# Guoxs/DODT

Hardware: AMD Instinct MI355X
Metric: frame-pairs/sec (whole node) KITTI-shape tau=2 (higher is better)
Workload: dtype f32

## Files before the change

dodt_amd/_lib.py:

```python
import ctypes as C
import os

_HERE = os.path.dirname(os.path.abspath(__file__))
LIB_PATH = os.environ.get('DODT_HIP_LIB') or os.path.join(_HERE, 'lib', 'libdodt_hip.so')

OK, ERR_INVALID, ERR_HIP, ERR_UNSUPPORTED = 0, 1, 2, 3
PTS_VELO_XYZI, PTS_CAM_3XN = 0, 1
EXTRACTOR_VGG_PYR = 0
EXTRACTOR_VGG = 1
EXTRACTOR_SHARED_GPU = 0x100
EXTRACTOR_BF16 = 0x200
EXTRACTOR_SPLIT = 0x400
FC_RELU = 1
FC_BF16 = 2
CONFLICT_RAISE, CONFLICT_NEXT_BEST = 0, 1


class DodtError(RuntimeError):
    pass


class BevParams(C.Structure):
    _fields_ = [
        ('point_format', C.c_int32),
# ... 17 lines not shown


class LayerInfo(C.Structure):
    _fields_ = [('name', C.c_char * 32), ('kernel', C.c_char * 48), ('launches', C.c_int32),
                ('items', C.c_int32), ('flops_direct', C.c_double), ('flops_executed', C.c_double),
                ('bytes', C.c_double), ('ms', C.c_float), ('reserved_', C.c_int32)]


_vp = C.c_void_p
_i = C.c_int
_f = C.c_float
_d = C.c_double
_pi32 = C.c_void_p
_pf = C.c_void_p
_hf = C.c_void_p

SIGNATURES = {
    'dodt_version': (_i, []),
    'dodt_last_error': (C.c_char_p, []),
    'dodt_ctx_create': (_i, [_i, C.POINTER(_vp)]),
    'dodt_mark': (_i, [_vp, _i]),
    'dodt_ctx_wait_mark': (_i, [_vp, _vp, _i]),
    'dodt_mark_elapsed': (_i, [_vp, _i, _vp, _i, C.POINTER(_f)]),
    'dodt_ctx_create_high_priority': (_i, [_i, C.POINTER(_vp)]),
    'dodt_ctx_create_on_stream': (_i, [_i, _vp, C.POINTER(_vp)]),
    'dodt_ctx_destroy': (_i, [_vp]),
    'dodt_ctx_sync': (_i, [_vp]),
    'dodt_ctx_wait_for': (_i, [_vp, _vp]),
    'dodt_malloc': (_i, [_vp, C.c_size_t, C.POINTER(_vp)]),
    'dodt_free': (_i, [_vp, _vp]),
    'dodt_memcpy_h2d': (_i, [_vp, _vp, _vp, C.c_size_t]),
    'dodt_memcpy_d2h': (_i, [_vp, _vp, _vp, C.c_size_t]),
    'dodt_memset': (_i, [_vp, _vp, _i, C.c_size_t]),
    'dodt_pinned_alloc': (_i, [_vp, C.c_size_t, C.POINTER(_vp)]),
    'dodt_pinned_free': (_i, [_vp, _vp]),
    'dodt_memcpy_h2d_async': (_i, [_vp, _vp, _vp, C.c_size_t]),
    'dodt_fetch_i32_begin': (_i, [_vp, _pi32, _i, _i]),
    'dodt_fetch_i32_end': (_i, [_vp, _i, C.POINTER(C.c_int32), _i]),
    'dodt_timer_start': (_i, [_vp]),
    'dodt_timer_stop': (_i, [_vp, C.POINTER(_f)]),
    'dodt_bev_slices': (_i, [_vp, _vp, _i, C.POINTER(BevParams), _pf, _vp]),
    'dodt_bev_status': (_i, [_vp, C.POINTER(_i)]),
    'dodt_bev_support_mask': (_i, [C.POINTER(BevParams), _i, _vp, _i, _i]),
    'dodt_anchor_filter': (_i, [_vp, _vp, _i, _i, _pi32, _i, _i, _pi32, _pi32]),
    'dodt_project_anchors_f64': (_i, [_vp, _vp, _pi32, _i, _pi32,
                                      C.POINTER(_d), C.POINTER(_d), _d, _d,
                                      _pf, _pf, _pf]),
    'dodt_project_anchors_f32': (_i, [_vp, _pf, _i, _pi32, C.POINTER(_f),
                                      C.POINTER(_f), _f, _f, _pf, _pf, _pf]),
    'dodt_img_preprocess': (_i, [_vp, _vp, _i, _i, _i, _i, _i,
                                 C.POINTER(_f), _pf]),
    'dodt_conv_mode': (_i, []),
    'dodt_extractor_create': (_i, [_vp, _i, _i, _i, _i, _i, _i,
                                   C.POINTER(_vp)]),
    'dodt_extractor_destroy': (_i, [_vp]),
    'dodt_extractor_set_layer': (_i, [_vp, C.c_char_p, _vp, _i, _i, _i, _i,
                                      _vp, _vp, _vp]),
    'dodt_extractor_input': (_i, [_vp, C.POINTER(_vp), C.POINTER(C.c_longlong)]),
    'dodt_extractor_forward': (_i, [_vp, _pf, _pf, _pf]),
    'dodt_extractor_forward_padded': (_i, [_vp, _pf, _pf, _pf]),
    'dodt_extractor_set_input': (_i, [_vp, _pf]),
    'dodt_extractor_set_input_support': (_i, [_vp, _vp, _i, _i, C.POINTER(C.c_longlong)]),
    'dodt_extractor_set_frame_tables': (_i, [_vp, _i, C.POINTER(_i)]),
    'dodt_extractor_frame_items': (_i, [_vp, C.POINTER(_i), _i]),
    'dodt_extractor_frame_split': (_i, [_vp, C.POINTER(_i), C.POINTER(_i), _i]),
    'dodt_extractor_store_bytes': (C.c_longlong, [_vp]),
    'dodt_frame_tables_host': (_i, [_vp, _i, _i, _i, _i, _i, _i, _vp, _i, _vp, _vp, C.POINTER(_i)]),
    'dodt_frame_restore_host': (_i, [_vp, _i, _i, _i, _i, _i, _i, _i, _i, _i, _vp, _vp, _vp, _vp]),
    'dodt_frame_lists_host': (_i, [_vp, _i, _i, _i, _i, _i, _i, _vp, _i, _vp, _vp, C.POINTER(_i), _vp, C.POINTER(_i)]),
    'dodt_extractor_read_activation': (_i, [_vp, C.c_char_p, _vp,
                                            C.POINTER(_i), C.POINTER(_i),
                                            C.POINTER(_i)]),
    'dodt_extractor_output_shape': (_i, [_vp, C.POINTER(_i), C.POINTER(_i), C.POINTER(_i)]),
    'dodt_extractor_first_layers_folded': (_i, [_vp]),
    'dodt_extractor_flops': (_d, [_vp]),
    'dodt_extractor_mfma_flops': (_d, [_vp]),
    'dodt_extractor_bytes': (_d, [_vp]),
    'dodt_extractor_layer_count': (_i, [_vp]),
    'dodt_extractor_forward_timed': (_i, [_vp, _pf, _pf, _pf, C.POINTER(LayerInfo), _i]),
    'dodt_crop_and_resize': (_i, [_vp, _pf, _i, _i, _i, _pf, _i, _pi32, _i, _i,
                                  _pf]),
    'dodt_crop_and_resize_strided': (_i, [_vp, _pf, _i, _i, _i, _pf, _i, _pi32, _i, _i, _pf,
                                          C.c_longlong]),
    'dodt_correlation': (_i, [_vp, _pf, _pf, _i, _i, _i, _i, _i, _i, _pf]),
    'dodt_mean_fusion': (_i, [_vp, _pf, _pf, _i, _pi32, _i, _pf]),
    'dodt_fc_create': (_i, [_vp, _i, _i, _hf, _hf, _i, C.POINTER(_vp)]),
    'dodt_fc_create_ex': (_i, [_vp, _i, _i, _hf, _hf, _i, C.POINTER(_vp)]),
    'dodt_fc_destroy': (_i, [_vp]),
    'dodt_fc_forward': (_i, [_vp, _vp, _pf, _pf, _i, _i, _pi32, _pf, _i]),
    'dodt_fc_forward_split': (_i, [_vp, _vp, _pf, _i, _i, _pi32, _i, C.POINTER(_i), C.POINTER(_vp)]),
    'dodt_fc_flops': (_d, [_vp, _i]),
    'dodt_fc_bf16_row_elems': (_i, [_vp]),
    'dodt_fc_forward_bf16': (_i, [_vp, _vp, _vp, _i, _i, _pi32, _vp, _i, _i]),
    'dodt_fc_forward_split_bf16': (_i, [_vp, _vp, _vp, _i, _i, _pi32, _i, C.POINTER(_i), C.POINTER(_vp)]),
    'dodt_rows_to_bf16': (_i, [_vp, _pf, _pf, _i, _pi32, _i, _i, _vp, _i]),
    'dodt_nms': (_i, [_vp, _pf, _pf, _i, _pi32, _i, _f, _pi32, _pi32]),
    'dodt_offset_to_anchor': (_i, [_vp, _pf, _pf, _i, _pi32, _pf]),
    'dodt_softmax_fg': (_i, [_vp, _pf, _i, _pi32, _pf]),
    'dodt_rpn_decode': (_i, [_vp, _pf, _pf, _pf, _i, _pi32, C.POINTER(_f), _pf, _pf, _pf]),
    'dodt_gather_project': (_i, [_vp, _pf, _pi32, _i, _pi32, C.POINTER(_f), C.POINTER(_f), _f, _f, _pf, _pf, _pf]),
    'dodt_final_decode': (_i, [_vp, _pf, _pf, _pf, _pf, _i, _pi32, C.POINTER(_f), C.POINTER(_f),
                               _pf, _pf, _pf, _pf, _pf, _pf]),
    'dodt_gather_rows': (_i, [_vp, _pf, _i, _pi32, _i, _pi32, _pf]),
    'dodt_max_fg_logit': (_i, [_vp, _pf, _i, _i, _pi32, _pf]),
    'dodt_pack_detections': (_i, [_vp, _pf, _pf, _pf, _pf, _pi32, _pi32, _i, _f, _pf, _pi32]),
    'dodt_angle_vector_to_orientation': (_i, [_vp, _pf, _i, _pi32, _pf]),
    'dodt_box_4c_decode': (_i, [_vp, _pf, _pf, _i, _pi32, C.POINTER(_f),
                                C.POINTER(_f), _pf, _pf, _pf]),
    'dodt_comm_unique_id': (_i, [_vp]),
    'dodt_comm_create': (_i, [_vp, _i, _i, _vp, C.POINTER(_vp)]),
    'dodt_comm_destroy': (_i, [_vp]),
    'dodt_comm_attach': (_i, [_vp, _vp]),
    'dodt_comm_rank': (_i, [_vp, C.POINTER(_i), C.POINTER(_i)]),
    'dodt_comm_set_late_peer': (_i, [_vp, _d]),
    'dodt_all_gather_records': (_i, [_vp, _vp, _i, _pf, _pi32, _i, _i, _i, _i, _pf, _pi32]),
    'dodt_comm_join': (_i, [_vp, _i, _vp]),
    'dodt_comm_sync': (_i, [_vp]),
    'dodt_comm_barrier': (_i, [_vp]),
    'dodt_comm_max_f64': (_i, [_vp, C.POINTER(_d)]),
    'dodt_three_d_iou_matrix': (_i, [_vp, _vp, _i, _vp, _i, _vp]),
    'dodt_interpolate_pairs': (_i, [_vp, _vp, _i, _pi32, _i, _i, _i, _d, _i, _vp, C.POINTER(_d), _i, _vp,
                                    _pi32, _pi32]),
    'dodt_track_state_bytes': (_i, [_i, C.POINTER(C.c_size_t)]),
    'dodt_track_reset': (_i, [_vp, _vp, _i]),
    'dodt_track_flush': (_i, [_vp, _vp, _d, _i]),
    'dodt_track_encode': (_i, [_vp, _vp, _i, _pi32, _i, _i, C.POINTER(_d), _d, _d, _d, _pf, _pf, _pi32]),
    'dodt_track_pairs': (_i, [_vp, _vp, _vp, _i, _pi32, _i, _i, C.POINTER(_d), _d, _d, _d, _d, _d, _i]),
    'dodt_track_encoded': (_i, [_vp, _vp, _pf, _pf, _pi32, _i, _i, _d, _d, _i]),
}
COMM_ID_BYTES = 128

_lib = None


def load():
    global _lib
    if _lib is not None:
        return _lib
    if not os.path.exists(LIB_PATH):
        raise DodtError(
            'libdodt_hip.so not found at %s -- build it with '
            '`make -C dodt_amd/csrc` (there is no CPU fallback)' % LIB_PATH)
    lib = C.CDLL(LIB_PATH)
    for name, (res, args) in SIGNATURES.items():
        fn = getattr(lib, name)
        fn.restype = res
        fn.argtypes = args
    _lib = lib
    return lib


def check(rc, what=''):
    if rc == OK:
        return
    msg = load().dodt_last_error().decode('utf-8', 'replace')
    if rc == ERR_INVALID:
        raise ValueError(msg or what)
    raise DodtError('%s: %s (status %d)' % (what, msg, rc))
```

dodt_amd/core/avod_fc_layers/fusion_fc_layers.py:

```python
import os

import numpy as np

from dodt_amd import ops


class EarlyFusionFcLayers(object):

    K_ALIGN = 32

    def __init__(self, ctx, params, outputs=('cls_out', 'off_out', 'ang_out'), dtype='f32'):
        names = sorted(k for k in params if k.startswith('fc'))
        w0 = np.asarray(params[names[0]]['w'], np.float32)
        self.in_k = w0.shape[0]
        self.in_ld = -(-self.in_k // self.K_ALIGN) * self.K_ALIGN
        if self.in_ld != self.in_k:
            w0 = np.concatenate([w0, np.zeros((self.in_ld - self.in_k, w0.shape[1]), np.float32)], 0)
        self.hidden = [ops.FullyConnected(ctx, w0 if k == names[0] else params[k]['w'], params[k]['b'],
                                          True, dtype=dtype) for k in names]
        self._packed_first = None
        self._first_params = (params[names[0]]['w'], params[names[0]]['b'], dtype)
        self.outputs = [ops.FullyConnected(ctx, params[k]['w'], params[k]['b'], False, dtype=dtype)
                        for k in outputs]
        self.fused_out = None
        if len(outputs) > 1:
            w = np.concatenate([np.asarray(params[k]['w'], np.float32) for k in outputs], 1)
            b = np.concatenate([np.asarray(params[k]['b'], np.float32) for k in outputs])
            fused = ops.FullyConnected(ctx, w, b, False, dtype=dtype)
            if fused.can_split():
                self.fused_out = fused
            else:
                fused.close()
        self.width = max(l.N for l in self.hidden)
        self.ctx = ctx
        self.bf16_rows = dtype == 'bf16' and os.environ.get('DODT_FC_BF16_ROWS', '1') != '0' and \
            all(l.bf16_row_elems() > 0 for l in self.hidden) and \
            (self.fused_out.bf16_row_elems() > 0 if self.fused_out is not None
             else all(l.bf16_row_elems() > 0 for l in self.outputs))
        self.in_ld16 = self.hidden[0].bf16_row_elems() if self.bf16_rows else 0

    def make_scratch(self, n_max):
        s = [self.ctx.empty((n_max, self.width), np.float32) for _ in range(2)] + \
            [self.ctx.zeros((n_max, self.in_ld), np.float32)]
        if self.bf16_rows:
            s += [self.ctx.zeros((n_max, self.width), np.uint16) for _ in range(2)] + \
                 [self.ctx.zeros((n_max, self.in_ld16), np.uint16)]
        return s

    def forward(self, ctx, d_rois, d_rois2, n, d_n, d_outs, scratch):
        x, x2 = d_rois, d_rois2
        ldx = self._row_floats(d_rois, n, 'd_rois')
        if x2 is not None and self._row_floats(x2, n, 'd_rois2') != ldx:
            raise ValueError('d_rois and d_rois2 must have the same row layout')
        if self.bf16_rows and len(scratch) > 5:
            ops.rows_to_bf16(ctx, x, x2, n, d_n, self.in_k, ldx, scratch[5], self.in_ld16)
            x16, ld16 = scratch[5], self.in_ld16
            for i, l in enumerate(self.hidden):
                y16 = scratch[3 + (i & 1)]
                l.forward_bf16(x16, n, y16, ldx=ld16, ldy=self.width, d_m=d_n, y_bf16=True, ctx=ctx)
                x16, ld16 = y16, self.width
            if self.fused_out is not None:
                self.fused_out.forward_split_bf16(x16, n, d_outs, [l.N for l in self.outputs], ldx=ld16, d_m=d_n, ctx=ctx)
            else:
                for l, d_y in zip(self.outputs, d_outs):
                    l.forward_bf16(x16, n, d_y, ldx=ld16, d_m=d_n, y_bf16=False, ctx=ctx)
            return
        first = self.hidden[0]
        if ldx != self.in_ld:
            if self._packed_first is None:
                w, b, dtype = self._first_params
                self._packed_first = ops.FullyConnected(self.ctx, w, b, True, dtype=dtype)
            first = self._packed_first
        if x2 is not None and len(scratch) > 2 and ldx == self.in_ld == self.in_k and self.in_k % 4 == 0:
            ops.mean_fusion(ctx, x, x2, n, d_n, self.in_ld, scratch[2])
            x, x2 = scratch[2], None
        for i, l in enumerate([first] + self.hidden[1:]):
            y = scratch[i & 1]
            l.forward(x, n, y, ldx=ldx, ldy=self.width, d_x2=x2, d_m=d_n, ctx=ctx)
            x, x2, ldx = y, None, self.width
        if self.fused_out is not None and ldx % 4 == 0:
            self.fused_out.forward_split(x, n, d_outs, [l.N for l in self.outputs], ldx=ldx, d_m=d_n, ctx=ctx)
            return
        for l, d_y in zip(self.outputs, d_outs):
            l.forward(x, n, d_y, ldx=ldx, d_m=d_n, ctx=ctx)

    def _row_floats(self, d, n, name):
        if d.dtype != np.float32:
            raise ValueError('%s must be float32' % name)
        size = int(np.prod(d.shape, dtype=np.int64))
        rows = d.shape[0] if len(d.shape) > 1 else 0
        if rows < n or rows == 0 or size % rows:
            raise ValueError('%s holds %s, fewer than %d rows' % (name, d.shape, n))
        per_row = size // rows
        if per_row not in (self.in_ld, self.in_k):
            raise ValueError('%s rows hold %d floats; the head takes %d (crop + zero tail) or %d (packed)'
                             % (name, per_row, self.in_ld, self.in_k))
        return per_row

    def flops(self, n):
        return sum(l.flops(n) for l in self.hidden + self.outputs) \
            - 2.0 * n * (self.in_ld - self.in_k) * self.hidden[0].N

    def close(self):
        for l in self.hidden + self.outputs + [self.fused_out, self._packed_first]:
            if l is not None:
                l.close()
```

dodt_amd/core/models/anchor_predictor.py:

```python
import numpy as np

from dodt_amd import ops


class AnchorPredictor(object):
    def __init__(self, ctx, params, dtype='f32'):
        def mat(name):
            w = np.asarray(params[name]['w'], np.float32)
            return w.reshape(-1, w.shape[-1]), np.asarray(params[name]['b'], np.float32)
        wc, bc = mat('cls_fc6')
        wr, br = mat('reg_fc6')
        self.width = wc.shape[1]
        if wr.shape != wc.shape:
            raise ValueError('cls_fc6 and reg_fc6 must have the same size')
        self.fc6 = ops.FullyConnected(ctx, np.concatenate([wc, wr], 1),
                                      np.concatenate([bc, br]), True, dtype=dtype)
        self.cls7 = ops.FullyConnected(ctx, *mat('cls_fc7'), relu=True, dtype=dtype)
        self.reg7 = ops.FullyConnected(ctx, *mat('reg_fc7'), relu=True, dtype=dtype)
        self.cls8 = ops.FullyConnected(ctx, *mat('cls_fc8'), relu=False, dtype=dtype)
        self.reg8 = ops.FullyConnected(ctx, *mat('reg_fc8'), relu=False, dtype=dtype)
        self.layers = [self.fc6, self.cls7, self.reg7, self.cls8, self.reg8]
        (w8c, b8c), (w8r, b8r) = mat('cls_fc8'), mat('reg_fc8')
        w8 = np.zeros((w8c.shape[0] + w8r.shape[0], w8c.shape[1] + w8r.shape[1]), np.float32)
        w8[:w8c.shape[0], :w8c.shape[1]] = w8c
        w8[w8c.shape[0]:, w8c.shape[1]:] = w8r
        self.out8 = ops.FullyConnected(ctx, w8, np.concatenate([b8c, b8r]), False, dtype=dtype)
        if not (self.out8.can_split() and w8c.shape[0] == self.width == w8r.shape[0]):
            self.out8.close()
            self.out8 = None
        self.ctx = ctx

    def make_scratch(self, n_max):
        return [self.ctx.empty((n_max, 2 * self.width), np.float32) for _ in range(2)]

    def forward(self, ctx, d_bev_roi, d_img_roi, n, d_objectness, d_offsets, scratch):
        w = self.width
        h6, h7 = scratch
        self.fc6.forward(d_bev_roi, n, h6, d_x2=d_img_roi, ctx=ctx)
        self.cls7.forward(h6, n, h7, ldx=2 * w, ldy=2 * w, ctx=ctx)
        self.reg7.forward(h6.offset(4 * w, (1,)), n, h7.offset(4 * w, (1,)),
                          ldx=2 * w, ldy=2 * w, ctx=ctx)
        if self.out8 is not None:
            self.out8.forward_split(h7, n, [d_objectness, d_offsets], [self.cls8.N, self.reg8.N], ctx=ctx)
            return
        self.cls8.forward(h7, n, d_objectness, ldx=2 * w, ctx=ctx)
        self.reg8.forward(h7.offset(4 * w, (1,)), n, d_offsets, ldx=2 * w, ctx=ctx)

    def flops(self, n):
        return sum(l.flops(n) for l in self.layers)

    def close(self):
        for l in self.layers + ([self.out8] if self.out8 is not None else []):
            l.close()
```

dodt_amd/csrc/crop.hip:

```cpp
#include "common.h"

namespace {

template <int VEC>
__global__ void __launch_bounds__(256)
crop_kernel(const float* __restrict__ img, int H, int W, int C, const float* __restrict__ boxes,
            int n, const int* __restrict__ d_n, int ch, int cw, float* __restrict__ out,
            long long out_stride) {
    const int groups = C / VEC;
    const long long t = (long long)blockIdx.x * blockDim.x + threadIdx.x;
    const int lim = d_n ? min(*d_n, n) : n;
    const long long total = (long long)lim * ch * cw * groups;
    if (t >= total) return;
    const int g = (int)(t % groups);
    long long r = t / groups;
    const int ix = (int)(r % cw); r /= cw;
    const int iy = (int)(r % ch);
    const int b = (int)(r / ch);
    const float4 bx = reinterpret_cast<const float4*>(boxes)[b];
    const float y1 = bx.x, x1 = bx.y, y2 = bx.z, x2 = bx.w;
    const float hm1 = (float)(H - 1), wm1 = (float)(W - 1);
    const float hs = (ch > 1) ? (y2 - y1) * hm1 / (float)(ch - 1) : 0.0f;
    const float ws = (cw > 1) ? (x2 - x1) * wm1 / (float)(cw - 1) : 0.0f;
    const float in_y = (ch > 1) ? y1 * hm1 + (float)iy * hs : 0.5f * (y1 + y2) * hm1;
    const float in_x = (cw > 1) ? x1 * wm1 + (float)ix * ws : 0.5f * (x1 + x2) * wm1;
    float* o = out + (size_t)b * out_stride + (((size_t)iy * cw + ix) * C + (size_t)g * VEC);
    const bool ok = (in_y >= 0.0f) && (in_y <= hm1) && (in_x >= 0.0f) && (in_x <= wm1);
    if (!ok) {
#pragma unroll
        for (int k = 0; k < VEC; ++k) o[k] = 0.0f;
        return;
    }
    const int ty = (int)floorf(in_y), by = (int)ceilf(in_y);
    const int lx_i = (int)floorf(in_x), rx_i = (int)ceilf(in_x);
    const float ly = in_y - (float)ty, lx = in_x - (float)lx_i;
    const float* ptl = img + ((size_t)ty * W + lx_i) * C + (size_t)g * VEC;
    const float* ptr = img + ((size_t)ty * W + rx_i) * C + (size_t)g * VEC;
    const float* pbl = img + ((size_t)by * W + lx_i) * C + (size_t)g * VEC;
    const float* pbr = img + ((size_t)by * W + rx_i) * C + (size_t)g * VEC;
#pragma unroll
    for (int k = 0; k < VEC; ++k) {
        const float tl = ptl[k], tr = ptr[k], bl = pbl[k], br = pbr[k];
        const float top = tl + (tr - tl) * lx;
        const float bot = bl + (br - bl) * lx;
        o[k] = top + (bot - top) * ly;
    }
}

}

extern "C" int dodt_crop_and_resize(dodt_ctx* ctx, const float* d_image, int H, int W, int C,
                                    const float* d_boxes, int n, const int32_t* d_n, int crop_h,
                                    int crop_w, float* d_out) {
    return dodt_crop_and_resize_strided(ctx, d_image, H, W, C, d_boxes, n, d_n, crop_h, crop_w, d_out,
                                        (long long)crop_h * crop_w * C);
}

extern "C" int dodt_crop_and_resize_strided(dodt_ctx* ctx, const float* d_image, int H, int W, int C,
                                            const float* d_boxes, int n, const int32_t* d_n, int crop_h,
                                            int crop_w, float* d_out, long long out_box_stride) {
    DODT_REQUIRE(ctx && d_image && d_out && (n == 0 || d_boxes),
                 "dodt_crop_and_resize: NULL argument");
    DODT_REQUIRE(H > 0 && W > 0 && C > 0 && crop_h > 0 && crop_w > 0 && n >= 0,
                 "dodt_crop_and_resize: bad sizes");
    DODT_REQUIRE(out_box_stride >= (long long)crop_h * crop_w * C,
                 "dodt_crop_and_resize: output stride %lld shorter than a crop", out_box_stride);
    if (n == 0) return DODT_OK;
    const int vec = (C % 4 == 0 && out_box_stride % 4 == 0) ? 4 : 1;
    const long long total = (long long)n * crop_h * crop_w * (C / vec);
    const int blocks = (int)((total + 255) / 256);
    if (vec == 4)
        hipLaunchKernelGGL(crop_kernel<4>, dim3(blocks), dim3(256), 0, ctx->stream, d_image, H, W,
                           C, d_boxes, n, d_n, crop_h, crop_w, d_out, out_box_stride);
    else
        hipLaunchKernelGGL(crop_kernel<1>, dim3(blocks), dim3(256), 0, ctx->stream, d_image, H, W,
                           C, d_boxes, n, d_n, crop_h, crop_w, d_out, out_box_stride);
    DODT_LAUNCH_CHECK();
    return DODT_OK;
}
```

dodt_amd/csrc/gemm.hip:

```cpp
#include <cmath>
#include <cstdlib>
#include <mutex>
#include <set>
#include <type_traits>
#include <vector>

#include <algorithm>

#include "common.h"
#include "lds_dma.h"

namespace {

typedef float f32x16 __attribute__((ext_vector_type(16)));
typedef float f32x4 __attribute__((ext_vector_type(4)));

constexpr int kKAlign = 64;
constexpr int kSmallK = 16;

struct GemmArgs {
    const float* x;
    const float* x2;
    const float* w;
    const float* bias;
    float* y;
    int M, K, Kp, N, ldx, ldy, relu;
    const int* d_m;
    unsigned long long* clock_probe = nullptr;
};

typedef __bf16 bf16x8 __attribute__((ext_vector_type(8)));
typedef __bf16 bf16x2 __attribute__((ext_vector_type(2)));
typedef float f32x2 __attribute__((ext_vector_type(2)));
__device__ __forceinline__ float pack_bf16(float lo, float hi) {
    return __builtin_bit_cast(float, __builtin_convertvector(f32x2{lo, hi}, bf16x2));
}

__device__ __forceinline__ float bf16_value(float packed, int which) {
    const unsigned u = __builtin_bit_cast(unsigned, packed);
    return __builtin_bit_cast(float, which ? (u & 0xffff0000u) : (u << 16));
}

template <int BM, int BN, int WM, int WN, bool XVEC, int WBN, int kBK, bool FUSE, bool BF16>
__global__ void __launch_bounds__(256)
fc_mfma_kernel(const GemmArgs a) {
    constexpr int MT = BM / 32 / WM, NT = BN / 32 / WN;
    constexpr int KB = BF16 ? 8 : 4;
    constexpr int G = kBK * 4 / KB;
    constexpr int kXS = G + 4;
    constexpr int XITEMS = BM * (G / 4);
    constexpr int WITEMS = G * BN / 4;
    constexpr int NX = (XITEMS + 255) / 256, NW = (WITEMS + 255) / 256;
    constexpr int kBuf = BM * kXS + G * BN;
    extern __shared__ __attribute__((aligned(16))) float smem[];

    const int tid = threadIdx.x, lane = tid & 63, wave = tid >> 6;
    const int wm = wave / WN, wn = wave % WN;
    const int li = lane & 31, lh = lane >> 5;
    const int m0 = blockIdx.x * BM, nt0 = blockIdx.y;
    const int M = a.d_m ? min(*a.d_m, a.M) : a.M;
    if (m0 >= M) return;
    const int nstages = a.Kp / kBK;
    static_assert(WBN % BN == 0, "tile must divide the blocked width");
    const f32x4* wblk = reinterpret_cast<const f32x4*>(a.w) +
                        (size_t)(nt0 * BN / WBN) * (a.Kp / (2 * KB)) * 2 * WBN + (nt0 * BN) % WBN;

    constexpr int XV = KB / 4;
    f32x4 prex[NX][XV];
    f32x4 pre[NX + NW];
    constexpr int NSLOT = NX + NW;
    int g_off[NSLOT];
    int l_off[NSLOT];
    int k_q[NX];
#pragma unroll
    for (int j = 0; j < NSLOT; ++j) {
        if (j < NX) {
            const int t = tid + j * 256;
            const int row = min(t / (G / 4), BM - 1), q = t % (G / 4);
            const int m = min(m0 + row, M - 1);
            g_off[j] = m * a.ldx + q * KB;
            k_q[j < NX ? j : 0] = q * KB;
            l_off[j] = row * kXS + q * 4;
        } else {
            const int t = min(tid + (j - NX) * 256, WITEMS - 1);
            g_off[j] = (t / BN) * WBN + t % BN;
            l_off[j] = BM * kXS + t * 4;
        }
    }
    f32x4 pre2[FUSE ? NX : 1][XV];
    auto load_slot = [&](int j, int st) {
        if (j < NX) {
            const int jx = j < NX ? j : 0;
// ... 99 lines not shown
            } else {
#pragma unroll
                for (int s = 0; s < 2; ++s)
#pragma unroll
                    for (int mt = 0; mt < MT; ++mt)
#pragma unroll
                        for (int nt = 0; nt < NT; ++nt)
                            acc[mt * NT + nt] = __builtin_amdgcn_mfma_f32_32x32x2f32(
                                xf[cb][mt][s], wf[cb][nt][s], acc[mt * NT + nt], 0, 0, 0);
            }
#pragma unroll
            for (int j = q * SPQ; j < (q + 1) * SPQ && j < NSLOT; ++j) {
                store_slot(j, buf ^ 1, min(st + 1, last));
                load_slot(j, st2);
            }
            if constexpr (!BF16) {
#pragma unroll
                for (int s = 2; s < 4; ++s)
#pragma unroll
                    for (int mt = 0; mt < MT; ++mt)
#pragma unroll
                        for (int nt = 0; nt < NT; ++nt)
                            acc[mt * NT + nt] = __builtin_amdgcn_mfma_f32_32x32x2f32(
                                xf[cb][mt][s], wf[cb][nt][s], acc[mt * NT + nt], 0, 0, 0);
            }
            __builtin_amdgcn_sched_barrier(0);
        }
        __syncthreads();
    }
#pragma unroll
    for (int nt = 0; nt < NT; ++nt) {
        const int n = nt0 * BN + (wn * NT + nt) * 32 + li;
        const float b = a.bias[n];
#pragma unroll
        for (int mt = 0; mt < MT; ++mt)
#pragma unroll
            for (int r = 0; r < 16; ++r) {
                const int m = m0 + (wm * MT + mt) * 32 + (r & 3) + 8 * (r >> 2) + 4 * lh;
                if (m < M && n < a.N) {
                    float v = acc[mt * NT + nt][r] + b;
                    if (a.relu) v = fmaxf(v, 0.0f);
                    a.y[(size_t)m * a.ldy + n] = v;
                }
            }
    }
}

template <int BM, int BN, int WM, int WN, int WBN = BN, int kBK = 32, bool BF16 = false>
int launch_fc(hipStream_t s, const GemmArgs& a, int Npad) {
    constexpr int G = BF16 ? kBK / 2 : kBK;
    constexpr size_t lds = 2 * (size_t)(BM * (G + 4) + G * BN) * sizeof(float);
    const bool vec = (a.ldx % 4 == 0) && (a.K % (BF16 ? 8 : 4) == 0);
    dim3 grid(dodt::ceil_div(a.M, BM), Npad / BN);
    auto go = [&](auto kernel) -> hipError_t {
        static std::mutex mu;
        static std::set<const void*> prepared;
        {
            std::lock_guard<std::mutex> lock(mu);
            if (!prepared.count(reinterpret_cast<const void*>(kernel))) {
                hipError_t e = hipFuncSetAttribute(reinterpret_cast<const void*>(kernel),
                                                   hipFuncAttributeMaxDynamicSharedMemorySize,
                                                   (int)lds);
                if (e != hipSuccess) return e;
                prepared.insert(reinterpret_cast<const void*>(kernel));
            }
        }
        hipLaunchKernelGGL(kernel, grid, dim3(256), lds, s, a);
        return hipSuccess;
    };
    hipError_t e;
    if (vec && a.x2) e = go(&fc_mfma_kernel<BM, BN, WM, WN, true, WBN, kBK, true, BF16>);
    else if (vec) e = go(&fc_mfma_kernel<BM, BN, WM, WN, true, WBN, kBK, false, BF16>);
    else if (a.x2) e = go(&fc_mfma_kernel<BM, BN, WM, WN, false, WBN, kBK, true, BF16>);
    else e = go(&fc_mfma_kernel<BM, BN, WM, WN, false, WBN, kBK, false, BF16>);
    DODT_HIP_CHECK(e);
    DODT_LAUNCH_CHECK();
    return DODT_OK;
}

constexpr int kDmaBM = 64, kDmaBK = 32, kDmaStages = 3;
constexpr int kDmaXFloats = kDmaBM * kDmaBK;

template <bool FUSE, int NT>
__global__ void __launch_bounds__(256, 2)
fc_dma_kernel(const GemmArgs a, int tiles_m, int tiles_n) {
    constexpr int kDmaBN = 64 * NT, kDmaWFloats = kDmaBK * kDmaBN;
    using dodt::blds16;
    using dodt::i32x4_t;
    using dodt::kOob;
    using dodt::make_rsrc;
    constexpr int kStage = kDmaXFloats * (FUSE ? 2 : 1) + kDmaWFloats;
    extern __shared__ __attribute__((aligned(16))) float smem[];
    const int tid = threadIdx.x, lane = tid & 63;
    const int wave = __builtin_amdgcn_readfirstlane(tid >> 6);
    const int wm = wave >> 1, wn = wave & 1;
    const int li = lane & 31, lh = lane >> 5;
    const int T = tiles_m * tiles_n;
    int tile = blockIdx.x;
    if (T % 8 == 0) tile = (int)(blockIdx.x % 8) * (T / 8) + (int)(blockIdx.x / 8);
    const int mt = tile / tiles_n, nt0 = tile % tiles_n;
    const int m0 = mt * kDmaBM;
    const int M = a.d_m ? min(*a.d_m, a.M) : a.M;
    if (m0 >= M) return;
    const int nstages = a.K / kDmaBK;

    const int rows = min(M - m0, kDmaBM);
    const i32x4_t x_rsrc = make_rsrc(a.x + (size_t)m0 * a.ldx, (unsigned)(((size_t)(rows - 1) * a.ldx + a.K) * 4));
    i32x4_t x2_rsrc = x_rsrc;
    if (FUSE) x2_rsrc = make_rsrc(a.x2 + (size_t)m0 * a.ldx, (unsigned)(((size_t)(rows - 1) * a.ldx + a.K) * 4));
    const int n0 = nt0 * kDmaBN;
    const float* wblk = a.w + ((size_t)(n0 / 128) * (a.Kp / 8) * 2 * 128 + (n0 % 128)) * 4;
    const i32x4_t w_rsrc = make_rsrc(wblk, (unsigned)(((size_t)(a.Kp / 8) * 2 * 128 - (n0 % 128)) * 16));
    int x_off[2], w_off[2 * NT];
#pragma unroll
    for (int k = 0; k < 2; ++k) {
        const int piece = wave + 4 * k;
        const int row = piece * 8 + (lane >> 3), cq = (lane & 7) ^ ((row >> 1) & 7);
        x_off[k] = row < rows ? (row * a.ldx + cq * 4) * 4 : kOob;
    }
#pragma unroll
    for (int k = 0; k < 2 * NT; ++k) {
        const int piece = wave + 4 * k;
        w_off[k] = ((piece / NT) * 128 + (piece % NT) * 64 + lane) * 16;
    }
    const unsigned lds0 = (unsigned)(size_t)(__attribute__((address_space(3))) void*)smem;
    constexpr int kPerStage = (FUSE ? 4 : 2) + 2 * NT;
    auto issue_one = [&](int st, int buf, int n) {
        const unsigned sX = lds0 + (unsigned)(buf * kStage) * 4;
        constexpr int kX = FUSE ? 4 : 2;
        if (n < kX) {
            const int k = FUSE ? n >> 1 : n;
            const unsigned piece = (unsigned)(wave + 4 * k) * 1024;
            if (FUSE && (n & 1)) dodt::blds16s(x2_rsrc, x_off[k], st * (kDmaBK * 4), sX + kDmaXFloats * 4 + piece);
            else dodt::blds16s(x_rsrc, x_off[k], st * (kDmaBK * 4), sX + piece);
        } else {
            const int k = n - kX;
            dodt::blds16s(w_rsrc, w_off[k], st * (8 * 128 * 16),
                          sX + kDmaXFloats * (FUSE ? 8 : 4) + (unsigned)(wave + 4 * k) * 1024);
        }
    };

    f32x16 acc[NT];
#pragma unroll
    for (int nt = 0; nt < NT; ++nt)
#pragma unroll
        for (int r = 0; r < 16; ++r) acc[nt][r] = 0.0f;
    const int xrow = wm * 32 + li;
    const int xsw = (xrow >> 1) & 7;
    const int x_base = xrow * kDmaBK;
    const int w_base = kDmaXFloats * (FUSE ? 2 : 1) + (lh * kDmaBN + wn * 32 * NT + li) * 4;

    int xo[4];
#pragma unroll
    for (int q = 0; q < 4; ++q) xo[q] = x_base + (((2 * q + lh) ^ xsw) * 4);
    auto stage = [&](auto bufc, int st) {
        constexpr int BUF = decltype(bufc)::value;
        if (st + 1 < nstages) __builtin_amdgcn_s_waitcnt(0x0f70 | kPerStage);
        else __builtin_amdgcn_s_waitcnt(0x0f70);
        __builtin_amdgcn_s_barrier();
        const bool more = st + 2 < nstages;
        const float* sS = smem + BUF * kStage;
        f32x4 xf[4], wf[4][NT], x2[FUSE ? 4 : 1];
        auto read_q = [&](int q) {
            xf[q] = *reinterpret_cast<const f32x4*>(sS + xo[q]);
#pragma unroll
            for (int nt = 0; nt < NT; ++nt)
                wf[q][nt] = *reinterpret_cast<const f32x4*>(sS + w_base + q * (2 * kDmaBN * 4) + nt * 128);
            if (FUSE) x2[q] = *reinterpret_cast<const f32x4*>(sS + kDmaXFloats + xo[q]);
        };
        read_q(0);
        read_q(1);
        __builtin_amdgcn_sched_barrier(0);
        constexpr int kPerQ = (kPerStage + 3) / 4;
#pragma unroll
        for (int q = 0; q < 4; ++q) {
            if (q + 2 < 4) read_q(q + 2);
            if (FUSE) {
#pragma unroll
                for (int e = 0; e < 4; ++e) xf[q][e] = (xf[q][e] + x2[q][e]) / 2.0f;
            }
#pragma unroll
            for (int s2 = 0; s2 < 4; ++s2)
#pragma unroll
                for (int nt = 0; nt < NT; ++nt)
                    acc[nt] = __builtin_amdgcn_mfma_f32_32x32x2f32(xf[q][s2], wf[q][nt][s2], acc[nt], 0, 0, 0);
            if (more) {
#pragma unroll
                for (int n = q * kPerQ; n < (q + 1) * kPerQ && n < kPerStage; ++n) issue_one(st + 2, (BUF + 2) % kDmaStages, n);
            }
            __builtin_amdgcn_sched_barrier(0);
        }
    };
    auto issue = [&](int st, int buf) {
#pragma unroll
        for (int n = 0; n < kPerStage; ++n) issue_one(st, buf, n);
    };
    issue(0, 0);
    if (nstages > 1) issue(1, 1);
    const bool probe = a.clock_probe != nullptr && blockIdx.x == 17 && tid == 0;
    unsigned long long c0 = 0, r0 = 0;
    if (probe) { c0 = __builtin_amdgcn_s_memtime(); r0 = __builtin_amdgcn_s_memrealtime(); }
    for (int st = 0; st < nstages; st += 3) {
        stage(std::integral_constant<int, 0>{}, st);
        if (st + 1 < nstages) stage(std::integral_constant<int, 1>{}, st + 1);
        if (st + 2 < nstages) stage(std::integral_constant<int, 2>{}, st + 2);
    }
    if (probe) {
        a.clock_probe[0] = __builtin_amdgcn_s_memtime() - c0;
        a.clock_probe[1] = __builtin_amdgcn_s_memrealtime() - r0;
    }
#pragma unroll
    for (int nt = 0; nt < NT; ++nt) {
        const int n = n0 + wn * 32 * NT + nt * 32 + li;
        const float b = a.bias[n];
#pragma unroll
        for (int r = 0; r < 16; ++r) {
            const int m = m0 + wm * 32 + (r & 3) + 8 * (r >> 2) + 4 * lh;
            if (m < M && n < a.N) {
                float v = acc[nt][r] + b;
                if (a.relu) v = fmaxf(v, 0.0f);
                a.y[(size_t)m * a.ldy + n] = v;
            }
        }
    }
}

int launch_fc_dma(hipStream_t s, const GemmArgs& a_in, int Npad) {
    GemmArgs a = a_in;
    static const bool want_clock = getenv("DODT_FC_CLOCK") != nullptr;
    static unsigned long long* d_probe = nullptr;
    if (want_clock) {
        if (!d_probe) DODT_HIP_CHECK(hipMalloc(&d_probe, 2 * sizeof(unsigned long long)));
        a.clock_probe = d_probe;
    }
    static const int force_nt = getenv("DODT_FC_NT") ? atoi(getenv("DODT_FC_NT")) : 0;
    const int nt = force_nt ? force_nt
                            : (!a.x2 && (long)dodt::ceil_div(a.M, kDmaBM) * (Npad / 128) >= 2 * 256 ? 2 : 1);
    const int tiles_m = dodt::ceil_div(a.M, kDmaBM), tiles_n = Npad / (64 * nt);
    auto go = [&](auto kernel, size_t lds) -> hipError_t {
        static std::mutex mu;
        static std::set<const void*> prepared;
        {
            std::lock_guard<std::mutex> lock(mu);
            if (!prepared.count(reinterpret_cast<const void*>(kernel))) {
                hipError_t e = hipFuncSetAttribute(reinterpret_cast<const void*>(kernel),
                                                   hipFuncAttributeMaxDynamicSharedMemorySize, (int)lds);
                if (e != hipSuccess) return e;
                prepared.insert(reinterpret_cast<const void*>(kernel));
            }
        }
        hipLaunchKernelGGL(kernel, dim3(tiles_m * tiles_n), dim3(256), lds, s, a, tiles_m, tiles_n);
        return hipSuccess;
    };
    hipError_t e;
    if (a.x2) e = go(&fc_dma_kernel<true, 1>, (size_t)kDmaStages * (2 * kDmaXFloats + kDmaBK * 64) * 4);
    else if (nt == 2) e = go(&fc_dma_kernel<false, 2>, (size_t)kDmaStages * (kDmaXFloats + kDmaBK * 128) * 4);
    else e = go(&fc_dma_kernel<false, 1>, (size_t)kDmaStages * (kDmaXFloats + kDmaBK * 64) * 4);
    DODT_HIP_CHECK(e);
    DODT_LAUNCH_CHECK();
    if (want_clock) {
        unsigned long long h[2] = {0, 0};
        (void)hipStreamSynchronize(s);
        (void)hipMemcpy(h, d_probe, sizeof(h), hipMemcpyDeviceToHost);
        if (h[1])
            fprintf(stderr, "[dodt] fc_dma_kernel M %d K %d N %d: K loop of workgroup 17: %llu shader cycles in %.2f us = %.3f GHz\n",
                    a.M, a.K, a.N, h[0], h[1] / 100.0, (double)h[0] / h[1] * 0.1);
    }
    return DODT_OK;
}

constexpr int kBfBM = 64, kBfBN = 128, kBfStages = 3;
__host__ __device__ constexpr int bf_swz(int r, int S) { return (r / (16 / S)) & (S - 1); }

template <bool YBF16, int BK, int R = kBfStages>
__global__ void __launch_bounds__(256, 2)
fc_bf16_dma_kernel(const GemmArgs a, int tiles_m, int tiles_n) {
    static_assert((R - 2) * ((kBfBM + kBfBN) * BK * 2 / 1024 / 4) <= 63, "vmcnt is six bits");
    using dodt::i32x4_t;
    using dodt::kOob;
    using dodt::make_rsrc;
    constexpr int S = BK / 8;
    constexpr int kXBytes = kBfBM * BK * 2, kWBytes = kBfBN * BK * 2, kStage = kXBytes + kWBytes;
    constexpr int kXPieces = kXBytes / 1024 / 4, kWPieces = kWBytes / 1024 / 4;
    constexpr int kPerStage = kXPieces + kWPieces;
    constexpr int kRowsPerPiece = 1024 / (BK * 2);
    constexpr int NQ = BK / 16;
    extern __shared__ __attribute__((aligned(16))) float smem[];
    const int tid = threadIdx.x, lane = tid & 63;
    const int wave = __builtin_amdgcn_readfirstlane(tid >> 6);
    const int wm = wave >> 1, wn = wave & 1;
    const int li = lane & 31, lh = lane >> 5;
    const int T = tiles_m * tiles_n;
    int tile = blockIdx.x;
    if (T % 8 == 0) tile = (int)(blockIdx.x % 8) * (T / 8) + (int)(blockIdx.x / 8);
    const int mt = tile / tiles_n, nt0 = tile % tiles_n;
    const int m0 = mt * kBfBM;
    const int M = a.d_m ? min(*a.d_m, a.M) : a.M;
    if (m0 >= M) return;
    const int nstages = a.Kp / BK;
    const int rows = min(M - m0, kBfBM);
    const unsigned short* x16 = reinterpret_cast<const unsigned short*>(a.x);
    const i32x4_t x_rsrc = make_rsrc(x16 + (size_t)m0 * a.ldx, (unsigned)(((size_t)(rows - 1) * a.ldx + a.Kp) * 2));
    const char* wblk = reinterpret_cast<const char*>(a.w) + (size_t)nt0 * nstages * kWBytes;
    const i32x4_t w_rsrc = make_rsrc(wblk, (unsigned)((size_t)nstages * kWBytes));
    int x_off[kXPieces];
#pragma unroll
    for (int k = 0; k < kXPieces; ++k) {
        const int row = (wave + 4 * k) * kRowsPerPiece + lane / S, slot = (lane % S) ^ bf_swz(row, S);
        x_off[k] = row < rows ? (row * a.ldx + slot * 8) * 2 : kOob;
    }
    const int w_off = lane * 16;
    const unsigned lds0 = (unsigned)(size_t)(__attribute__((address_space(3))) void*)smem;
    auto issue_one = [&](int st, int buf, int n) {
        const unsigned sX = lds0 + (unsigned)(buf * kStage);
        if (n < kXPieces) dodt::blds16s(x_rsrc, x_off[n < kXPieces ? n : 0], st * (BK * 2), sX + (unsigned)(wave + 4 * n) * 1024);
        else dodt::blds16s(w_rsrc, w_off, st * kWBytes + (wave + 4 * (n - kXPieces)) * 1024,
                           sX + kXBytes + (unsigned)(wave + 4 * (n - kXPieces)) * 1024);
    };
    f32x16 acc[2];
#pragma unroll
    for (int nt = 0; nt < 2; ++nt)
#pragma unroll
        for (int r = 0; r < 16; ++r) acc[nt][r] = 0.0f;
    const int sw = bf_swz(li, S);
    int so[NQ];
#pragma unroll
    for (int q = 0; q < NQ; ++q) so[q] = ((2 * q + lh) ^ sw) * 16;
    const int x_base = (wm * 32 + li) * (BK * 2);
    const int w_base = kXBytes + (wn * 64 + li) * (BK * 2);
    auto stage = [&](auto bufc, int st) {
        constexpr int BUF = decltype(bufc)::value;
        if (st + R - 2 < nstages) asm volatile("s_waitcnt vmcnt(%0)" ::"n"((R - 2) * kPerStage) : "memory");
        else __builtin_amdgcn_s_waitcnt(0x0f70);
        __builtin_amdgcn_s_barrier();
        const bool more = st + R - 1 < nstages;
        const char* sS = reinterpret_cast<const char*>(smem) + BUF * kStage;
        f32x4 xf[NQ], wf[NQ][2];
        auto read_q = [&](int q) {
            xf[q] = *reinterpret_cast<const f32x4*>(sS + x_base + so[q]);
#pragma unroll
            for (int nt = 0; nt < 2; ++nt)
                wf[q][nt] = *reinterpret_cast<const f32x4*>(sS + w_base + nt * 32 * (BK * 2) + so[q]);
        };
        read_q(0);
        read_q(1);
        __builtin_amdgcn_sched_barrier(0);
#pragma unroll
        for (int q = 0; q < NQ; ++q) {
            if (q + 2 < NQ) read_q(q + 2);
#pragma unroll
// ... 153 lines not shown
                wa[u] = ok ? w4[(size_t)jj * 128] : z;
                wb[u] = ok ? w4[(size_t)jj * 128 + 16] : z;
            }
#pragma unroll
            for (int u = 0; u < U; ++u)
#pragma unroll
                for (int s = 0; s < 4; ++s) {
                    acc0 = mfma16x4(xv[u][s], wa[u][s], acc0);
                    acc1 = mfma16x4(xv[u][s], wb[u][s], acc1);
                }
        }
    }
    s_part[wave][0][lane] = acc0;
    s_part[wave][1][lane] = acc1;
    __syncthreads();
    if (tid >= 128) return;
    const int nb = tid >> 6;
    f32x4 sum = s_part[0][nb][lane];
#pragma unroll
    for (int w = 1; w < 8; ++w) sum += s_part[w][nb][lane];
    const int n = nb * 16 + i;
    if (n >= a.N) return;
    const float b = a.bias[n];
    const int p = (n >= so.n_end[0]) + (n >= so.n_end[1]);
    float* y = p == 0 ? so.y[0] : (p == 1 ? so.y[1] : so.y[2]);
    const int ld = p == 0 ? so.ld[0] : (p == 1 ? so.ld[1] : so.ld[2]);
    const int nn = n - (p == 0 ? 0 : (p == 1 ? so.n_end[0] : so.n_end[1]));
#pragma unroll
    for (int r = 0; r < 4; ++r) {
        const int m = m0 + 4 * g + r;
        if (m < M) {
            float v = sum[r] + b;
            if (a.relu) v = fmaxf(v, 0.0f);
            y[(size_t)m * ld + nn] = v;
        }
    }
}

template <bool BF16>
__global__ void __launch_bounds__(256)
fc_smallk_kernel(const GemmArgs a, const float* __restrict__ w_plain) {
    const int M = a.d_m ? min(*a.d_m, a.M) : a.M;
    const int n4 = a.N >> 2;
    const long long t = (long long)blockIdx.x * blockDim.x + threadIdx.x;
    const int m = (int)(t / n4), c = (int)(t - (long long)m * n4) * 4;
    if (m >= M) return;
    const float* x = a.x + (size_t)m * a.ldx;
    const float* x2 = a.x2 ? a.x2 + (size_t)m * a.ldx : nullptr;
    f32x4 acc = {0.f, 0.f, 0.f, 0.f};
    for (int k = 0; k < a.K; ++k) {
        float xv = x[k];
        if (x2) xv = (xv + x2[k]) / 2.0f;
        if constexpr (BF16) xv = bf16_value(pack_bf16(xv, 0.0f), 0);
        const f32x4 wv = *reinterpret_cast<const f32x4*>(w_plain + (size_t)k * a.N + c);
        acc += wv * xv;
    }
    const f32x4 b = *reinterpret_cast<const f32x4*>(a.bias + c);
    acc += b;
    if (a.relu) {
#pragma unroll
        for (int i = 0; i < 4; ++i) acc[i] = fmaxf(acc[i], 0.0f);
    }
    float* y = a.y + (size_t)m * a.ldy + c;
    if ((a.ldy & 3) == 0) *reinterpret_cast<f32x4*>(y) = acc;
    else {
#pragma unroll
        for (int i = 0; i < 4; ++i) y[i] = acc[i];
    }
}

bool skinny_ok(int Npad, int K, const GemmArgs& a) {
    static const bool on = !(getenv("DODT_FC_SKINNY") && atoi(getenv("DODT_FC_SKINNY")) == 0);
    return on && Npad == 32 && K % 16 == 0 && a.ldx % 4 == 0 && (size_t)a.x % 16 == 0 && !a.x2;
}

int launch_fc_skinny(hipStream_t s, const GemmArgs& a, const SplitOut& so, bool bf16, bool x_bf16 = false) {
    if (x_bf16) hipLaunchKernelGGL((fc_skinny_kernel<true, true>), dim3(dodt::ceil_div(a.M, 16)), dim3(512), 0, s, a, so);
    else if (bf16) hipLaunchKernelGGL(fc_skinny_kernel<true>, dim3(dodt::ceil_div(a.M, 16)), dim3(512), 0, s, a, so);
    else hipLaunchKernelGGL(fc_skinny_kernel<false>, dim3(dodt::ceil_div(a.M, 16)), dim3(512), 0, s, a, so);
    DODT_LAUNCH_CHECK();
    return DODT_OK;
}

}

namespace {
__global__ void __launch_bounds__(256)
mean_fusion_kernel(const float4* __restrict__ a, const float4* __restrict__ b, int rows, const int* __restrict__ d_n,
                   int row4, float4* __restrict__ out) {
    const int lim = d_n ? min(*d_n, rows) : rows;
    const long long total = (long long)lim * row4;
    for (long long i = (long long)blockIdx.x * blockDim.x + threadIdx.x; i < total;
         i += (long long)gridDim.x * blockDim.x) {
        const float4 x = a[i], y = b[i];
        out[i] = make_float4((x.x + y.x) / 2.0f, (x.y + y.y) / 2.0f, (x.z + y.z) / 2.0f, (x.w + y.w) / 2.0f);
    }
}
}

extern "C" int dodt_mean_fusion(dodt_ctx* ctx, const float* d_a, const float* d_b, int rows, const int32_t* d_n,
                                int row_floats, float* d_out) {
    DODT_REQUIRE(ctx && d_a && d_b && d_out, "dodt_mean_fusion: NULL argument");
    DODT_REQUIRE(rows >= 0 && row_floats >= 4 && row_floats % 4 == 0,
                 "dodt_mean_fusion: rows of a multiple of four floats, got %d", row_floats);
    DODT_REQUIRE(((size_t)d_a | (size_t)d_b | (size_t)d_out) % 16 == 0, "dodt_mean_fusion: 16-byte aligned blocks");
    if (rows == 0) return DODT_OK;
    const long long total = (long long)rows * (row_floats / 4);
    const int blocks = (int)std::min<long long>((total + 255) / 256, 4096);
    hipLaunchKernelGGL(mean_fusion_kernel, dim3(blocks), dim3(256), 0, ctx->stream,
                       reinterpret_cast<const float4*>(d_a), reinterpret_cast<const float4*>(d_b), rows, d_n,
                       row_floats / 4, reinterpret_cast<float4*>(d_out));
    DODT_LAUNCH_CHECK();
    return DODT_OK;
}

namespace {
__global__ void __launch_bounds__(256)
rows_to_bf16_kernel(const float* __restrict__ a, const float* __restrict__ b, int rows, const int* __restrict__ d_n,
                    int row_floats, int in_ld, unsigned short* __restrict__ out, int out_ld) {
    const int lim = d_n ? min(*d_n, rows) : rows;
    const int q4 = out_ld / 4;
    const long long total = (long long)lim * q4;
    for (long long i = (long long)blockIdx.x * blockDim.x + threadIdx.x; i < total;
         i += (long long)gridDim.x * blockDim.x) {
        const int r = (int)(i / q4), c = (int)(i - (long long)r * q4) * 4;
        float v[4];
#pragma unroll
        for (int e = 0; e < 4; ++e) {
            float t = 0.0f;
            if (c + e < row_floats) {
                t = a[(size_t)r * in_ld + c + e];
                if (b) t = (t + b[(size_t)r * in_ld + c + e]) / 2.0f;
            }
            v[e] = t;
        }
        f32x2 o = {pack_bf16(v[0], v[1]), pack_bf16(v[2], v[3])};
        *reinterpret_cast<f32x2*>(out + (size_t)r * out_ld + c) = o;
    }
}
}

extern "C" int dodt_rows_to_bf16(dodt_ctx* ctx, const float* d_a, const float* d_b, int rows, const int32_t* d_n,
                                 int row_floats, int in_ld, void* d_out_bf16, int out_ld) {
    DODT_REQUIRE(ctx && d_a && d_out_bf16, "dodt_rows_to_bf16: NULL argument");
    DODT_REQUIRE(rows >= 0 && row_floats >= 1 && in_ld >= row_floats && out_ld >= row_floats && out_ld % 4 == 0,
                 "dodt_rows_to_bf16: rows of %d floats, %d apart, into rows of %d bf16 (a multiple of 4)", row_floats,
                 in_ld, out_ld);
    DODT_REQUIRE((size_t)d_out_bf16 % 8 == 0, "dodt_rows_to_bf16: 8-byte aligned output");
    if (rows == 0) return DODT_OK;
    const long long total = (long long)rows * (out_ld / 4);
    const int blocks = (int)std::min<long long>((total + 255) / 256, 4096);
    hipLaunchKernelGGL(rows_to_bf16_kernel, dim3(blocks), dim3(256), 0, ctx->stream, d_a, d_b, rows, d_n, row_floats,
                       in_ld, reinterpret_cast<unsigned short*>(d_out_bf16), out_ld);
    DODT_LAUNCH_CHECK();
    return DODT_OK;
}

struct dodt_fc {
    dodt_ctx* ctx = nullptr;
    int K = 0, Kp = 0, N = 0, Npad = 0, BN = 0, relu = 0;
    bool bf16 = false;
    float* d_w = nullptr;
    float* d_b = nullptr;
    float* d_w_plain = nullptr;
    void* d_w_dma = nullptr;
    int Kd = 0;
// ... 48 lines not shown
    if (bf16 && N % kBfBN == 0 && K >= 128) {
        const int BK = bf16_dma_bk(), S = BK / 8;
        f->Kd = (int)dodt::align_up((size_t)K, (size_t)64);
        f->dma_bk = BK;
        const int ns = f->Kd / BK;
        std::vector<uint16_t> img((size_t)(N / kBfBN) * ns * kBfBN * BK, 0);
        for (int k = 0; k < K; ++k)
            for (int n = 0; n < N; ++n) {
                const int t = n / kBfBN, c = n % kBfBN, st = k / BK, kk = k % BK;
                const int slot = (kk / 8) ^ bf_swz(c, S);
                img[((((size_t)t * ns + st) * kBfBN + c) * S + slot) * 8 + kk % 8] = dodt::float_to_bf16(w[(size_t)k * N + n]);
            }
        if (hipMalloc(&f->d_w_dma, img.size() * sizeof(uint16_t)) != hipSuccess) {
            dodt::set_error("dodt_fc_create: hipMalloc failed");
            dodt_fc_destroy(f);
            return DODT_ERR_HIP;
        }
        DODT_HIP_CHECK(hipMemcpy(f->d_w_dma, img.data(), img.size() * sizeof(uint16_t), hipMemcpyHostToDevice));
    }
    std::vector<float> plain;
    if (K <= kSmallK && N % 4 == 0) {
        plain.assign(w, w + (size_t)K * N);
        if (bf16)
            for (float& v : plain) v = dodt::bf16_to_float(dodt::float_to_bf16(v));
        if (hipMalloc(&f->d_w_plain, plain.size() * sizeof(float)) != hipSuccess) {
            dodt::set_error("dodt_fc_create: hipMalloc failed");
            dodt_fc_destroy(f);
            return DODT_ERR_HIP;
        }
        DODT_HIP_CHECK(hipMemcpyAsync(f->d_w_plain, plain.data(), plain.size() * sizeof(float),
                                      hipMemcpyHostToDevice, ctx->stream));
    }
    DODT_HIP_CHECK(hipStreamSynchronize(ctx->stream));
    *out = f;
    return DODT_OK;
}

int dodt_fc_destroy(dodt_fc* f) {
    if (!f) return DODT_OK;
    if (f->d_w) (void)hipFree(f->d_w);
    if (f->d_b) (void)hipFree(f->d_b);
    if (f->d_w_plain) (void)hipFree(f->d_w_plain);
    if (f->d_w_dma) (void)hipFree(f->d_w_dma);
    delete f;
    return DODT_OK;
}

int dodt_fc_forward(dodt_fc* f, dodt_ctx* ctx, const float* d_x, const float* d_x2, int ldx,
                    int M, const int32_t* d_m, float* d_y, int ldy) {
    DODT_REQUIRE(f && d_x && d_y, "dodt_fc_forward: NULL argument");
    DODT_REQUIRE(M >= 0 && ldx >= f->K && ldy >= f->N, "dodt_fc_forward: bad strides");
    if (M == 0) return DODT_OK;
    GemmArgs a;
    a.x = d_x; a.x2 = d_x2; a.w = f->d_w; a.bias = f->d_b; a.y = d_y;
    a.M = M; a.K = f->K; a.Kp = f->Kp; a.N = f->N; a.ldx = ldx; a.ldy = ldy; a.relu = f->relu;
    a.d_m = d_m;
    hipStream_t s = (ctx ? ctx : f->ctx)->stream;
    static const bool smallk = !(getenv("DODT_FC_SMALLK") && atoi(getenv("DODT_FC_SMALLK")) == 0);
    if (smallk && f->d_w_plain && f->N >= 64 && (size_t)d_y % 16 == 0) {
        const long long threads = (long long)M * (f->N / 4);
        if (f->bf16)
            hipLaunchKernelGGL(fc_smallk_kernel<true>, dim3((unsigned)((threads + 255) / 256)), dim3(256), 0, s, a,
                               f->d_w_plain);
        else
            hipLaunchKernelGGL(fc_smallk_kernel<false>, dim3((unsigned)((threads + 255) / 256)), dim3(256), 0, s, a,
                               f->d_w_plain);
        DODT_LAUNCH_CHECK();
        return DODT_OK;
    }
    if (skinny_ok(f->Npad, f->K, a)) {
        SplitOut so = {{d_y, d_y, d_y}, {f->N, f->N, f->N}, {ldy, ldy, ldy}};
        return launch_fc_skinny(s, a, so, f->bf16);
    }
    if (f->bf16) {
        if (f->BN == 128) {
            static const int bk = getenv("DODT_FC_BF16_BK") ? atoi(getenv("DODT_FC_BF16_BK")) : 32;
            if (bk == 64) return launch_fc<64, 128, 2, 2, 128, 64, true>(s, a, f->Npad);
            if (bk == 32) return launch_fc<64, 128, 2, 2, 128, 32, true>(s, a, f->Npad);
            return launch_fc<64, 128, 2, 2, 128, 128, true>(s, a, f->Npad);
        }
        return launch_fc<128, 32, 4, 1, 32, 64, true>(s, a, f->Npad);
    }
    if (f->BN == 128) {
        static const bool dma = !(getenv("DODT_FC_DMA") && atoi(getenv("DODT_FC_DMA")) == 0);
        if (dma && f->K % kDmaBK == 0 && ldx % 4 == 0 && f->K >= 2 * kDmaBK &&
            ((size_t)d_x % 16 == 0) && (!d_x2 || (size_t)d_x2 % 16 == 0))
            return launch_fc_dma(s, a, f->Npad);
        static const int tile = getenv("DODT_FC_TILE") ? atoi(getenv("DODT_FC_TILE")) : 0;
        if (tile == 256) return launch_fc<128, 128, 2, 2, 128, 32>(s, a, f->Npad);
        if (tile == 64) return launch_fc<64, 64, 2, 2, 128>(s, a, f->Npad);
        if (tile == 32) return launch_fc<64, 128, 2, 2, 128, 32>(s, a, f->Npad);
        return launch_fc<64, 128, 2, 2, 128, 64>(s, a, f->Npad);
    }
    return launch_fc<128, 32, 4, 1>(s, a, f->Npad);
}

int dodt_fc_forward_split(dodt_fc* f, dodt_ctx* ctx, const float* d_x, int ldx, int M, const int32_t* d_m,
                          int parts, const int* widths, float* const* d_ys) {
    DODT_REQUIRE(f && d_x && widths && d_ys, "dodt_fc_forward_split: NULL argument");
    DODT_REQUIRE(parts >= 1 && parts <= 3, "dodt_fc_forward_split: %d parts (1..3)", parts);
    DODT_REQUIRE(M >= 0 && ldx >= f->K, "dodt_fc_forward_split: bad strides");
    GemmArgs a;
    a.x = d_x; a.x2 = nullptr; a.w = f->d_w; a.bias = f->d_b; a.y = nullptr;
    a.M = M; a.K = f->K; a.Kp = f->Kp; a.N = f->N; a.ldx = ldx; a.ldy = 0; a.relu = f->relu;
    a.d_m = d_m;
    SplitOut so;
    int end = 0;
    for (int p = 0; p < 3; ++p) {
        const int q = p < parts ? p : parts - 1;
        DODT_REQUIRE(widths[q] >= 1 && d_ys[q], "dodt_fc_forward_split: part %d is empty", q);
        if (p < parts) end += widths[p];
        so.y[p] = d_ys[q];
        so.n_end[p] = p < parts ? end : f->N + 1;
        so.ld[p] = widths[q];
    }
    DODT_REQUIRE(end == f->N, "dodt_fc_forward_split: the parts have %d columns, the layer %d", end, f->N);
    if (!skinny_ok(f->Npad, f->K, a)) {
        dodt::set_error("dodt_fc_forward_split: layers with N <= 32, K %% 16 == 0 and 16-byte aligned rows only");
        return DODT_ERR_UNSUPPORTED;
    }
    if (M == 0) return DODT_OK;
    return launch_fc_skinny((ctx ? ctx : f->ctx)->stream, a, so, f->bf16);
}

int dodt_fc_bf16_row_elems(const dodt_fc* f) {
    if (!f || !f->bf16) return 0;
    if (f->d_w_dma) return f->Kd;
    return (f->Npad == 32 && f->K % 16 == 0) ? f->K : 0;
}

int dodt_fc_forward_bf16(dodt_fc* f, dodt_ctx* ctx, const void* d_x_bf16, int ldx, int M, const int32_t* d_m,
                         void* d_y, int ldy, int y_bf16) {
    DODT_REQUIRE(f && d_x_bf16 && d_y, "dodt_fc_forward_bf16: NULL argument");
    DODT_REQUIRE(f->bf16, "dodt_fc_forward_bf16: the layer was not created with DODT_FC_BF16");
    DODT_REQUIRE(M >= 0 && ldy >= f->N, "dodt_fc_forward_bf16: bad strides");
    if (M == 0) return DODT_OK;
    GemmArgs a;
    a.x = reinterpret_cast<const float*>(d_x_bf16); a.x2 = nullptr; a.bias = f->d_b; a.y = reinterpret_cast<float*>(d_y);
    a.M = M; a.K = f->K; a.N = f->N; a.ldx = ldx; a.ldy = ldy; a.relu = f->relu; a.d_m = d_m;
    hipStream_t s = (ctx ? ctx : f->ctx)->stream;
    if (f->d_w_dma) {
        DODT_REQUIRE(ldx >= f->Kd && ldx % 8 == 0 && (size_t)d_x_bf16 % 16 == 0,
                     "dodt_fc_forward_bf16: rows of >= %d bf16 (zeros beyond K = %d), 16-byte aligned", f->Kd, f->K);
        DODT_REQUIRE((size_t)M * ldx * 2 < (1ull << 31), "dodt_fc_forward_bf16: x block beyond 2 GB");
        a.w = reinterpret_cast<const float*>(f->d_w_dma);
        a.Kp = f->Kd;
        return launch_fc_bf16_dma(s, a, f->Npad, y_bf16 != 0, f->dma_bk);
    }
    if (f->Npad == 32 && f->K % 16 == 0 && ldx % 4 == 0 && (size_t)d_x_bf16 % 8 == 0 && !y_bf16) {
        DODT_REQUIRE(ldx >= f->K, "dodt_fc_forward_bf16: bad strides");
        a.w = f->d_w; a.Kp = f->Kp;
        float* y = reinterpret_cast<float*>(d_y);
        SplitOut so = {{y, y, y}, {f->N, f->N, f->N}, {ldy, ldy, ldy}};
        return launch_fc_skinny(s, a, so, true, true);
    }
    dodt::set_error("dodt_fc_forward_bf16: layers with N %% 128 == 0 and K >= 128, or N <= 32 and K %% 16 == 0 with "
                    "float32 output, only (K = %d, N = %d)", f->K, f->N);
    return DODT_ERR_UNSUPPORTED;
}

int dodt_fc_forward_split_bf16(dodt_fc* f, dodt_ctx* ctx, const void* d_x_bf16, int ldx, int M, const int32_t* d_m,
                               int parts, const int* widths, float* const* d_ys) {
    DODT_REQUIRE(f && d_x_bf16 && widths && d_ys, "dodt_fc_forward_split_bf16: NULL argument");
    DODT_REQUIRE(f->bf16, "dodt_fc_forward_split_bf16: the layer was not created with DODT_FC_BF16");
    DODT_REQUIRE(parts >= 1 && parts <= 3, "dodt_fc_forward_split_bf16: %d parts (1..3)", parts);
    DODT_REQUIRE(M >= 0 && ldx >= f->K, "dodt_fc_forward_split_bf16: bad strides");
    GemmArgs a;
    a.x = reinterpret_cast<const float*>(d_x_bf16); a.x2 = nullptr; a.w = f->d_w; a.bias = f->d_b; a.y = nullptr;
    a.M = M; a.K = f->K; a.Kp = f->Kp; a.N = f->N; a.ldx = ldx; a.ldy = 0; a.relu = f->relu;
    a.d_m = d_m;
    SplitOut so;
    int end = 0;
    for (int p = 0; p < 3; ++p) {
        const int q = p < parts ? p : parts - 1;
        DODT_REQUIRE(widths[q] >= 1 && d_ys[q], "dodt_fc_forward_split_bf16: part %d is empty", q);
        if (p < parts) end += widths[p];
        so.y[p] = d_ys[q];
// ... 18 lines not shown
```

dodt_amd/csrc/nms.hip:

```cpp
#include "common.h"

namespace {

constexpr int kTile = 8192;
constexpr int kSortThreads = 1024;
constexpr int kChunkRows = 2048;
constexpr int kColGroup = 1;
constexpr int kRankMax = 32768;
constexpr int kRankSeg = 512;

struct NmsState {
    int count;
    int done;
    int n_eff;
    int pad;
};

__device__ __forceinline__ uint32_t ordered_bits(float f) {
    const uint32_t b = __float_as_uint(f);
    return (b & 0x80000000u) ? ~b : (b | 0x80000000u);
}

__global__ void __launch_bounds__(256)
nms_keys_kernel(const float* __restrict__ scores, int n, const int* __restrict__ d_n, int n_pad,
                unsigned long long* __restrict__ keys, NmsState* __restrict__ st,
                unsigned long long* __restrict__ removed, int nb, int* __restrict__ rank) {
    const int i = blockIdx.x * blockDim.x + threadIdx.x;
    const int n_eff = d_n ? min(*d_n, n) : n;
    if (i == 0) { st->count = 0; st->done = (n_eff <= 0); st->n_eff = n_eff; }
    if (i < nb) removed[i] = 0ull;
    if (i >= n_pad) return;
    if (rank) rank[i] = 0;
    unsigned long long k = ~0ull;
    if (i < n_eff) k = ((unsigned long long)(~ordered_bits(scores[i])) << 32) | (uint32_t)i;
    keys[i] = k;
}

__device__ __forceinline__ void cmp_swap(unsigned long long& a, unsigned long long& b, bool up) {
    if ((a > b) == up) { const unsigned long long t = a; a = b; b = t; }
}

__global__ void __launch_bounds__(kSortThreads)
nms_sort_local(unsigned long long* __restrict__ keys, int n_pad) {
    extern __shared__ __attribute__((aligned(16))) unsigned long long s_keys[];
    const int tile = min(kTile, n_pad);
    const size_t base = (size_t)blockIdx.x * tile;
    for (int t = threadIdx.x; t < tile; t += kSortThreads) s_keys[t] = keys[base + t];
    __syncthreads();
    for (int k = 2; k <= tile; k <<= 1) {
        for (int j = k >> 1; j > 0; j >>= 1) {
            for (int t = threadIdx.x; t < tile / 2; t += kSortThreads) {
                const int lo = ((t & ~(j - 1)) << 1) | (t & (j - 1));
                const int hi = lo + j;
                const bool up = (((base + lo) & (size_t)k) == 0);
                unsigned long long a = s_keys[lo], b = s_keys[hi];
                cmp_swap(a, b, up);
                s_keys[lo] = a;
                s_keys[hi] = b;
            }
            __syncthreads();
        }
    }
    for (int t = threadIdx.x; t < tile; t += kSortThreads) keys[base + t] = s_keys[t];
}

__global__ void __launch_bounds__(256)
nms_sort_global_step(unsigned long long* __restrict__ keys, int n_pad, int k, int j) {
    const int t = blockIdx.x * blockDim.x + threadIdx.x;
    if (t >= n_pad / 2) return;
    const int lo = ((t & ~(j - 1)) << 1) | (t & (j - 1));
    const int hi = lo + j;
    unsigned long long a = keys[lo], b = keys[hi];
    const bool up = ((lo & k) == 0);
    if ((a > b) == up) { keys[lo] = b; keys[hi] = a; }
}

__global__ void __launch_bounds__(kSortThreads)
nms_sort_local_merge(unsigned long long* __restrict__ keys, int n_pad, int k) {
    extern __shared__ __attribute__((aligned(16))) unsigned long long s_keys[];
    const size_t base = (size_t)blockIdx.x * kTile;
    for (int t = threadIdx.x; t < kTile; t += kSortThreads) s_keys[t] = keys[base + t];
    __syncthreads();
    for (int j = kTile >> 1; j > 0; j >>= 1) {
        for (int t = threadIdx.x; t < kTile / 2; t += kSortThreads) {
            const int lo = ((t & ~(j - 1)) << 1) | (t & (j - 1));
            const int hi = lo + j;
            const bool up = (((base + lo) & (size_t)k) == 0);
            unsigned long long a = s_keys[lo], b = s_keys[hi];
            cmp_swap(a, b, up);
            s_keys[lo] = a;
            s_keys[hi] = b;
        }
        __syncthreads();
    }
    for (int t = threadIdx.x; t < kTile; t += kSortThreads) keys[base + t] = s_keys[t];
}

__global__ void __launch_bounds__(256)
nms_rank_kernel(const unsigned long long* __restrict__ keys, const NmsState* __restrict__ st, int n_pad,
                int* __restrict__ rank) {
    __shared__ __attribute__((aligned(16))) unsigned long long s_seg[kRankSeg];
    const int n_eff = st->n_eff;
    const int i0 = blockIdx.x * 256, j0 = blockIdx.y * kRankSeg;
    if (i0 >= n_eff || j0 >= n_eff) return;
    for (int t = threadIdx.x; t < kRankSeg; t += 256) s_seg[t] = (j0 + t < n_pad) ? keys[j0 + t] : ~0ull;
    __syncthreads();
    const int i = i0 + threadIdx.x;
    if (i >= n_eff) return;
    const unsigned long long mine = keys[i];
    int cnt = 0;
#pragma unroll 16
    for (int j = 0; j < kRankSeg; ++j) cnt += (s_seg[j] < mine) ? 1 : 0;
    if (cnt) atomicAdd(&rank[i], cnt);
}

__global__ void __launch_bounds__(256)
nms_scatter_kernel(const float* __restrict__ boxes, const int* __restrict__ rank,
                   const NmsState* __restrict__ st, int n_rows, float* __restrict__ sb,
                   int* __restrict__ sorted_idx) {
    const int i = blockIdx.x * blockDim.x + threadIdx.x;
    if (i >= n_rows) return;
    float ymin = 0, xmin = 0, ymax = 0, xmax = 0, area = -1.0f;
    int idx = -1, row = i;
    if (i < st->n_eff) {
        idx = i;
        row = rank[i];
        const float4 b = reinterpret_cast<const float4*>(boxes)[i];
        ymin = fminf(b.x, b.z); ymax = fmaxf(b.x, b.z);
        xmin = fminf(b.y, b.w); xmax = fmaxf(b.y, b.w);
        area = (ymax - ymin) * (xmax - xmin);
    }
    float* o = sb + (size_t)row * 5;
    o[0] = ymin; o[1] = xmin; o[2] = ymax; o[3] = xmax; o[4] = area;
    sorted_idx[row] = idx;
}

struct SBox { float ymin, xmin, ymax, xmax, area; };

__global__ void __launch_bounds__(256)
nms_gather_kernel(const float* __restrict__ boxes, const unsigned long long* __restrict__ keys,
                  const NmsState* __restrict__ st, int n_rows, float* __restrict__ sb,
                  int* __restrict__ sorted_idx) {
    const int i = blockIdx.x * blockDim.x + threadIdx.x;
    if (i >= n_rows) return;
    float ymin = 0, xmin = 0, ymax = 0, xmax = 0, area = -1.0f;
    int idx = -1;
    if (i < st->n_eff) {
        idx = (int)(keys[i] & 0xFFFFFFFFull);
        const float4 b = reinterpret_cast<const float4*>(boxes)[idx];
        ymin = fminf(b.x, b.z); ymax = fmaxf(b.x, b.z);
        xmin = fminf(b.y, b.w); xmax = fmaxf(b.y, b.w);
        area = (ymax - ymin) * (xmax - xmin);
    }
    float* o = sb + (size_t)i * 5;
    o[0] = ymin; o[1] = xmin; o[2] = ymax; o[3] = xmax; o[4] = area;
    sorted_idx[i] = idx;
}

__device__ __forceinline__ bool iou_gt(float ymin_i, float xmin_i, float ymax_i, float xmax_i,
                                       float area_i, float ymin_j, float xmin_j, float ymax_j,
                                       float xmax_j, float area_j, float thr) {
    if (area_i <= 0.0f || area_j <= 0.0f) return false;
    const float iy = fmaxf(fminf(ymax_i, ymax_j) - fmaxf(ymin_i, ymin_j), 0.0f);
    const float ix = fmaxf(fminf(xmax_i, xmax_j) - fmaxf(xmin_i, xmin_j), 0.0f);
    const float inter = iy * ix;
    const float iou = inter / ((area_i + area_j) - inter);
    return iou > thr;
}

__global__ void __launch_bounds__(256)
nms_mask_kernel(const float* __restrict__ sb, const NmsState* __restrict__ st, int row0, int rows,
                int nb, float thr, unsigned long long* __restrict__ mask,
                unsigned long long* __restrict__ diag_cols) {
    if (st->done) return;
    __shared__ float s_rows[4][64][5];
    const int wave = threadIdx.x >> 6, lane = threadIdx.x & 63;
    const int rb = (row0 >> 6) + blockIdx.y * 4 + wave;
    const int n_eff = st->n_eff;
    const int row = rb * 64 + lane;
    {
        const float* p = sb + (size_t)row * 5;
        const bool ok = row < n_eff;
#pragma unroll
        for (int k = 0; k < 5; ++k) s_rows[wave][lane][k] = ok ? p[k] : (k == 4 ? -1.0f : 0.0f);
    }
    __syncthreads();
    if (rb * 64 >= n_eff || rb * 64 >= row0 + rows) return;
    const int cb0 = blockIdx.x * kColGroup;
    unsigned long long words[kColGroup];
#pragma unroll
    for (int g = 0; g < kColGroup; ++g) {
        const int cb = cb0 + g;
        unsigned long long mine = 0ull;
        if (cb >= rb && cb < nb) {
            const int col = cb * 64 + lane;
            float cy0 = 0, cx0 = 0, cy1 = 0, cx1 = 0, ca = -1.0f;
            if (col < n_eff) {
                const float* p = sb + (size_t)col * 5;
                cy0 = p[0]; cx0 = p[1]; cy1 = p[2]; cx1 = p[3]; ca = p[4];
            }
            unsigned long long hits = 0ull;
            for (int r = 0; r < 64; ++r) {
                const float* q = s_rows[wave][r];
                const bool hit = (col > rb * 64 + r) &&
                                 iou_gt(q[0], q[1], q[2], q[3], q[4], cy0, cx0, cy1, cx1, ca, thr);
                const unsigned long long w = __ballot(hit);
                if (lane == r) mine = w;
                hits |= hit ? (1ull << r) : 0ull;
            }
// ... 50 lines not shown
    auto block = [&](auto stage, int b) -> bool {
        constexpr int S = decltype(stage)::value;
        load_block(b + kScanDepth - 1, v[(S + kScanDepth - 1) % kScanDepth]);
        if (tid < 64) {
            const int row = b * 64 + lane;
            const unsigned long long cols = s_cols[(b - b0) * 64 + lane];
            const int valid = min(64, n_eff - b * 64);
            unsigned long long init = ~s_removed[b];
            if (valid < 64) init &= (1ull << valid) - 1ull;
            const bool mine = (init >> lane) & 1ull;
            unsigned long long alive = __ballot(mine);
            for (;;) {
                const unsigned long long na = __ballot(mine && (cols & alive) == 0ull);
                if (na == alive) break;
                alive = na;
            }
            const int cnt0 = __builtin_amdgcn_readfirstlane(s_count);
            const int room = max_out - cnt0;
            const unsigned long long below = (1ull << lane) - 1ull;
            unsigned long long sel = alive;
            if (__popcll(sel) > room)
                sel = __ballot(((sel >> lane) & 1ull) && __popcll(sel & below) < room);
            const int cnt = cnt0 + __popcll(sel);
            if ((sel >> lane) & 1ull) sel_out[cnt0 + __popcll(sel & below)] = sorted_idx[row];
            if (lane == 0) {
                s_sel = sel;
                s_kept[b - b0] = sel;
                s_count = cnt;
                if (cnt >= max_out) s_done = 1;
            }
        }
        __syncthreads();
        const unsigned long long sel = s_sel;
        const bool done = s_done != 0;
        if (!done && sel != 0ull) {
            unsigned long long acc = 0ull;
#pragma unroll
            for (int k = 0; k < 4; ++k)
                if ((sel >> (wave + 16 * k)) & 1ull) acc |= v[S][k];
            if (acc) atomicOr(&s_removed[b + 1 + lane], acc);
        }
        __syncthreads();
        return done;
    };
    bool stop = false;
    for (int b = b0; b < b1 && !stop; b += kScanDepth) {
        stop = block(std::integral_constant<int, 0>{}, b);
        if (!stop && b + 1 < b1) stop = block(std::integral_constant<int, 1>{}, b + 1);
        if (!stop && b + 2 < b1) stop = block(std::integral_constant<int, 2>{}, b + 2);
        if (!stop && b + 3 < b1) stop = block(std::integral_constant<int, 3>{}, b + 3);
    }
    static_assert(kScanDepth == 4, "the loop above is unrolled by hand");

    if (!stop && row0 + rows < n_eff) {
        const int nrows = (b1 - b0) * 64;
        for (int ct = b1; ct < nb; ct += 64) {
            const int c = ct + lane;
            if (c >= nb) continue;
            const unsigned long long* base = mask + (size_t)(b0 * 64 - row0) * nb + c;
            unsigned long long acc = 0ull;
            for (int r0 = wave; r0 < nrows; r0 += 16 * 8) {
                unsigned long long w[8];
#pragma unroll
                for (int k = 0; k < 8; ++k) w[k] = base[(size_t)min(r0 + 16 * k, nrows - 1) * nb];
#pragma unroll
                for (int k = 0; k < 8; ++k) {
                    const int r = r0 + 16 * k;
                    if (r < nrows && ((s_kept[r >> 6] >> (r & 63)) & 1ull)) acc |= w[k];
                }
            }
            if (acc) atomicOr(&s_removed[c], acc);
        }
        __syncthreads();
    }
    for (int c = tid; c < nb; c += 1024) g_removed[c] = s_removed[c];
    if (tid == 0) {
        st->count = s_count;
        const int exhausted = (row0 + rows >= n_eff);
        if (s_done || exhausted) st->done = 1;
        if (last_chunk || s_done || exhausted) *count_out = s_count;
    }
}

int next_pow2(int v) {
    int p = 1;
    while (p < v) p <<= 1;
    return p;
}

}

extern "C" int dodt_nms(dodt_ctx* ctx, const float* d_boxes, const float* d_scores, int n,
                        const int32_t* d_n, int max_out, float iou_threshold, int32_t* d_sel_out,
                        int32_t* d_count_out) {
    DODT_REQUIRE(ctx && d_sel_out && d_count_out && (n == 0 || (d_boxes && d_scores)),
                 "dodt_nms: NULL argument");
    DODT_REQUIRE(n >= 0 && max_out >= 0, "dodt_nms: negative size");
    DODT_REQUIRE(n <= 400000, "dodt_nms: n = %d exceeds 400000", n);
    if (n == 0 || max_out == 0) {
        DODT_HIP_CHECK(hipMemsetAsync(d_count_out, 0, sizeof(int32_t), ctx->stream));
        return DODT_OK;
    }
    const int n_pad = next_pow2(n < 2 ? 2 : n);
    const int nb = dodt::ceil_div(n, 64);
    const int n_rows = nb * 64;
    const bool ranked = n <= kRankMax;
    const int later_rows = nb <= 1024 ? 2 * kChunkRows : kChunkRows;
    int first_rows = (int)dodt::align_up((size_t)max_out + (size_t)max_out / 8, 64) + 64;
    if (first_rows > later_rows) first_rows = later_rows;
    if (first_rows > n_rows || n_rows <= kChunkRows) first_rows = n_rows;
    if (n_rows - first_rows > later_rows && n_rows - later_rows <= later_rows) first_rows = n_rows - later_rows;
    const int chunk_rows = n_rows < later_rows ? n_rows : later_rows;
    size_t off = 0;
    const size_t o_state = off; off += 256;
    const size_t o_keys = off; off += dodt::align_up((size_t)n_pad * 8, 256);
    const size_t o_rank = off; off += dodt::align_up((size_t)n_pad * 4, 256);
    const size_t o_sb = off; off += dodt::align_up((size_t)n_rows * 5 * 4, 256);
    const size_t o_idx = off; off += dodt::align_up((size_t)n_rows * 4, 256);
    const size_t o_removed = off; off += dodt::align_up((size_t)nb * 8, 256);
    const size_t o_diag = off; off += dodt::align_up((size_t)n_rows * 8, 256);
    const size_t o_mask = off; off += (size_t)chunk_rows * nb * 8;
    int rc = ctx->nms_ws.reserve(off);
    if (rc) return rc;
    char* ws = reinterpret_cast<char*>(ctx->nms_ws.ptr);
    NmsState* st = reinterpret_cast<NmsState*>(ws + o_state);
    unsigned long long* keys = reinterpret_cast<unsigned long long*>(ws + o_keys);
    int* rank = reinterpret_cast<int*>(ws + o_rank);
    float* sb = reinterpret_cast<float*>(ws + o_sb);
    int* sorted_idx = reinterpret_cast<int*>(ws + o_idx);
    unsigned long long* removed = reinterpret_cast<unsigned long long*>(ws + o_removed);
    unsigned long long* diag_cols = reinterpret_cast<unsigned long long*>(ws + o_diag);
    unsigned long long* mask = reinterpret_cast<unsigned long long*>(ws + o_mask);
    hipStream_t s = ctx->stream;

    const int init_n = n_pad > nb ? n_pad : nb;
    hipLaunchKernelGGL(nms_keys_kernel, dim3(dodt::ceil_div(init_n, 256)), dim3(256), 0, s,
                       d_scores, n, d_n, n_pad, keys, st, removed, nb, ranked ? rank : (int*)nullptr);
    DODT_LAUNCH_CHECK();
    if (ranked) {
        hipLaunchKernelGGL(nms_rank_kernel, dim3(dodt::ceil_div(n, 256), dodt::ceil_div(n, kRankSeg)),
                           dim3(256), 0, s, keys, st, n_pad, rank);
        DODT_LAUNCH_CHECK();
        hipLaunchKernelGGL(nms_scatter_kernel, dim3(dodt::ceil_div(n_rows, 256)), dim3(256), 0, s,
                           d_boxes, rank, st, n_rows, sb, sorted_idx);
        DODT_LAUNCH_CHECK();
    } else {
        const int tile = n_pad < kTile ? n_pad : kTile;
        hipLaunchKernelGGL(nms_sort_local, dim3(n_pad / tile), dim3(kSortThreads), (size_t)tile * 8, s,
                           keys, n_pad);
        DODT_LAUNCH_CHECK();
        for (int k = 2 * kTile; k <= n_pad; k <<= 1) {
            for (int j = k >> 1; j >= kTile; j >>= 1) {
                hipLaunchKernelGGL(nms_sort_global_step, dim3(dodt::ceil_div(n_pad / 2, 256)),
                                   dim3(256), 0, s, keys, n_pad, k, j);
                DODT_LAUNCH_CHECK();
            }
            hipLaunchKernelGGL(nms_sort_local_merge, dim3(n_pad / kTile), dim3(kSortThreads),
                               (size_t)kTile * 8, s, keys, n_pad, k);
            DODT_LAUNCH_CHECK();
        }
        hipLaunchKernelGGL(nms_gather_kernel, dim3(dodt::ceil_div(n_rows, 256)), dim3(256), 0, s,
                           d_boxes, keys, st, n_rows, sb, sorted_idx);
        DODT_LAUNCH_CHECK();
    }
    const int col_groups = dodt::ceil_div(nb, kColGroup);
    const size_t scan_lds = ((size_t)nb + chunk_rows + chunk_rows / 64) * 8;
    static const hipError_t lds_attr = hipFuncSetAttribute(
        reinterpret_cast<const void*>(nms_scan_kernel), hipFuncAttributeMaxDynamicSharedMemorySize, 128 * 1024);
    DODT_HIP_CHECK(lds_attr);
    for (int row0 = 0; row0 < n_rows;) {
        const int want = row0 == 0 ? first_rows : later_rows;
        const int rows = (n_rows - row0) < want ? (n_rows - row0) : want;
        hipLaunchKernelGGL(nms_mask_kernel, dim3(col_groups, dodt::ceil_div(rows / 64, 4)),
                           dim3(256), 0, s, sb, st, row0, rows, nb, iou_threshold, mask, diag_cols);
        DODT_LAUNCH_CHECK();
        const int last = (row0 + rows >= n_rows);
        hipLaunchKernelGGL(nms_scan_kernel, dim3(1), dim3(1024), scan_lds, s, mask, diag_cols,
                           sorted_idx, st, removed, row0, rows, nb, max_out, d_sel_out,
                           d_count_out, last);
        DODT_LAUNCH_CHECK();
        row0 += rows;
    }
    return DODT_OK;
}
```

dodt_amd/csrc/voxelizer.hip:

```cpp
#include "common.h"

#include <cmath>
#include <vector>

namespace {

constexpr int kMaxSlices = 8;
constexpr int kIdxBits = 25;

struct VoxParams {
    int format, n, S, X, Z;
    int cx_min, cy_min, cz_min;
    int occ_words_per_row;
    int origin_off;
    int has_pre;
    double pre_t[3], pre_r[9];
    double m[12];
    double p2[12];
    double im_w, im_h;
    double a, b, c, d, nrm;
    double ext[6];
    double vs;
    double d_hi[kMaxSlices], d_lo[kMaxSlices];
    double lo[kMaxSlices];
    double per_div;
    double dens_d_hi, dens_d_lo, occ_d_hi, occ_d_lo;
    float quirk[kMaxSlices];
    float dens_table[16];
};

constexpr int kCntList = 0, kCntErr = 1, kCntSlice = 2;

__device__ __forceinline__ bool load_point(const void* pts, const VoxParams& P, int i,
                                           double& x, double& y, double& z, bool warp = true) {
    if (P.format == DODT_PTS_VELO_XYZI) {
        const float4 v = reinterpret_cast<const float4*>(pts)[i];
        double vx = v.x, vy = v.y, vz = v.z;
        if (warp && P.has_pre) {
            const double ax = vx + P.pre_t[0], ay = vy + P.pre_t[1], az = vz + P.pre_t[2];
            vx = (double)(float)fma(az, P.pre_r[6], fma(ay, P.pre_r[3], ax * P.pre_r[0]));
            vy = (double)(float)fma(az, P.pre_r[7], fma(ay, P.pre_r[4], ax * P.pre_r[1]));
            vz = (double)(float)fma(az, P.pre_r[8], fma(ay, P.pre_r[5], ax * P.pre_r[2]));
        }
        x = fma(P.m[2], vz, fma(P.m[1], vy, P.m[0] * vx)) + P.m[3];
        y = fma(P.m[6], vz, fma(P.m[5], vy, P.m[4] * vx)) + P.m[7];
        z = fma(P.m[10], vz, fma(P.m[9], vy, P.m[8] * vx)) + P.m[11];
        if (!(z > 0.0)) return false;
        const double un = fma(P.p2[2], z, fma(P.p2[1], y, P.p2[0] * x)) + P.p2[3];
        const double vn = fma(P.p2[6], z, fma(P.p2[5], y, P.p2[4] * x)) + P.p2[7];
        const double w = fma(P.p2[10], z, fma(P.p2[9], y, P.p2[8] * x)) + P.p2[11];
        const double u = un / w, vv = vn / w;
        return (u > 0.0) && (u < P.im_w) && (vv > 0.0) && (vv < P.im_h);
    } else {
        const double* p = reinterpret_cast<const double*>(pts);
        x = p[i];
        y = p[(size_t)P.n + i];
        z = p[2 * (size_t)P.n + i];
        return true;
    }
}

__device__ __forceinline__ bool in_extents(const VoxParams& P, double x, double y, double z) {
    return x > P.ext[0] && x < P.ext[1] && y > P.ext[2] && y < P.ext[3] && z > P.ext[4] &&
           z < P.ext[5];
}

__global__ void __launch_bounds__(256)
vox_scatter(const void* __restrict__ pts, const VoxParams P, uint32_t* __restrict__ out,
            uint32_t* __restrict__ occ, uint32_t* __restrict__ list,
            uint32_t* __restrict__ counters, uint32_t list_cap) {
    __shared__ uint32_t s_cnt[kMaxSlices];
    __shared__ uint32_t s_n;
    __shared__ uint32_t s_base;
    __shared__ uint32_t s_items[256 * (kMaxSlices + 1)];
    const int tid = threadIdx.x;
    if (tid < kMaxSlices) s_cnt[tid] = 0;
    if (tid == 0) s_n = 0;
    __syncthreads();

    const int i = blockIdx.x * blockDim.x + tid;
    double x, y, z;
    bool ok = i < P.n && load_point(pts, P, i, x, y, z);
    ok = ok && in_extents(P, x, y, z);
    bool occ_ok = ok;
    double occ_dotp = 0.0;
    int occ_xi = 0, occ_zi = 0;
    if (ok) {
        const double dotp = fma(P.c, z, fma(P.b, y, P.a * x));
        const int xi = (int)floor(x / P.vs) - P.cx_min;
        const int yb = (int)floor(y / P.vs) - P.cy_min;
        const int zi = (int)floor(z / P.vs) - P.cz_min;
        if (xi < 0 || xi >= P.X || zi < 0 || zi >= P.Z || yb < 0 || yb > 126) {
            atomicOr(&counters[kCntErr], 1u);
            occ_ok = false;
        } else {
            const int C = P.S + 1;
            const uint32_t base = (uint32_t)(((P.Z - 1 - zi) * P.X + xi) * C);
            const uint32_t key = ~(((uint32_t)yb << kIdxBits) | (uint32_t)i);
            for (int s = 0; s < P.S; ++s) {
                const bool member = ((dotp + P.d_hi[s]) < 0.0) != ((dotp + P.d_lo[s]) < 0.0);
                if (member) {
                    const uint32_t old = atomicMax(&out[base + s], key);
                    if (old == 0u) s_items[atomicAdd(&s_n, 1u)] = base + s;
                    atomicAdd(&s_cnt[s], 1u);
                }
            }
            if (((dotp + P.dens_d_hi) < 0.0) != ((dotp + P.dens_d_lo) < 0.0)) {
                const uint32_t old = atomicAdd(&out[base + P.S], 1u);
                if (old == 0u) s_items[atomicAdd(&s_n, 1u)] = base + P.S;
            }
            occ_dotp = dotp;
            occ_xi = xi;
            occ_zi = zi;
        }
    }
    if (occ != nullptr) {
        if (P.has_pre && P.format == DODT_PTS_VELO_XYZI) {
            double ux, uy, uz;
            occ_ok = i < P.n && load_point(pts, P, i, ux, uy, uz, false) && in_extents(P, ux, uy, uz);
            if (occ_ok) {
                occ_dotp = fma(P.c, uz, fma(P.b, uy, P.a * ux));
                occ_xi = (int)floor(ux / P.vs) - P.cx_min;
                occ_zi = (int)floor(uz / P.vs) - P.cz_min;
                const int yb = (int)floor(uy / P.vs) - P.cy_min;
                if (occ_xi < 0 || occ_xi >= P.X || occ_zi < 0 || occ_zi >= P.Z || yb < 0 || yb > 126) {
                    atomicOr(&counters[kCntErr], 1u);
                    occ_ok = false;
                }
            }
        }
        if (occ_ok && (((occ_dotp + P.occ_d_hi) < 0.0) != ((occ_dotp + P.occ_d_lo) < 0.0)))
            atomicOr(&occ[occ_zi * P.occ_words_per_row + (occ_xi >> 5)], 1u << (occ_xi & 31));
    }
    __syncthreads();
    if (tid < P.S && s_cnt[tid]) atomicAdd(&counters[kCntSlice + tid], s_cnt[tid]);
    if (tid == 0) s_base = s_n ? atomicAdd(&counters[kCntList], s_n) : 0u;
    __syncthreads();
    const uint32_t n = s_n, gbase = s_base;
    for (uint32_t k = tid; k < n; k += 256) {
        if (gbase + k < list_cap) list[gbase + k] = s_items[k];
        else atomicOr(&counters[kCntErr], 2u);
    }
}

__global__ void __launch_bounds__(256)
vox_finalize(const void* __restrict__ pts, const VoxParams P, uint32_t* __restrict__ out,
             const uint32_t* __restrict__ list, const uint32_t* __restrict__ counters,
// ... 30 lines not shown
    outf[off] = (float)(__dsub_rn(h, P.lo[ch]) / P.per_div);
}

}

extern "C" int dodt_bev_slices(dodt_ctx* ctx, const void* d_points, int n_points,
                               const dodt_bev_params* bp, float* d_bev_out,
                               uint32_t* d_occ_bits_out) {
    DODT_REQUIRE(ctx && bp && d_bev_out, "dodt_bev_slices: NULL argument");
    DODT_REQUIRE(n_points >= 0 && (n_points == 0 || d_points),
                 "dodt_bev_slices: bad point buffer");
    DODT_REQUIRE(bp->point_format == DODT_PTS_VELO_XYZI || bp->point_format == DODT_PTS_CAM_3XN,
                 "dodt_bev_slices: unknown point_format %d", bp->point_format);
    DODT_REQUIRE(bp->num_slices >= 1 && bp->num_slices <= kMaxSlices,
                 "dodt_bev_slices: num_slices %d not in [1,%d]", bp->num_slices, kMaxSlices);
    DODT_REQUIRE(n_points < (1 << kIdxBits), "dodt_bev_slices: n_points %d >= 2^25", n_points);
    DODT_REQUIRE(bp->voxel_size > 0, "dodt_bev_slices: voxel_size must be positive");

    VoxParams P;
    P.format = bp->point_format;
    P.n = n_points;
    P.S = bp->num_slices;
    const double vs = bp->voxel_size;
    const double minx = std::floor(bp->extents[0] / vs), maxx = std::ceil(bp->extents[1] / vs - 1);
    const double miny = std::floor(bp->extents[2] / vs), maxy = std::ceil(bp->extents[3] / vs - 1);
    const double minz = std::floor(bp->extents[4] / vs), maxz = std::ceil(bp->extents[5] / vs - 1);
    P.X = (int)(maxx - minx + 1);
    P.Z = (int)(maxz - minz + 1);
    DODT_REQUIRE(P.X > 0 && P.Z > 0, "Extents are the wrong shape");
    DODT_REQUIRE(maxy - miny + 1 <= 127, "dodt_bev_slices: more than 127 y-bins (%g)",
                 maxy - miny + 1);
    DODT_REQUIRE((double)P.X * P.Z * (P.S + 1) < 4.0e9, "dodt_bev_slices: grid too large");
    P.cx_min = (int)minx;
    P.cy_min = (int)miny;
    P.cz_min = (int)minz;
    P.occ_words_per_row = dodt::ceil_div(P.X, 32);
    for (int k = 0; k < 12; ++k) { P.m[k] = bp->velo_to_cam[k]; P.p2[k] = bp->p2[k]; }
    P.has_pre = bp->has_pre_transform != 0;
    DODT_REQUIRE(!P.has_pre || bp->point_format == DODT_PTS_VELO_XYZI,
                 "dodt_bev_slices: the ego-motion pre-transform applies to velodyne points");
    for (int k = 0; k < 3; ++k) P.pre_t[k] = bp->pre_translate[k];
    for (int k = 0; k < 9; ++k) P.pre_r[k] = bp->pre_rotate[k];
    P.im_w = bp->im_w;
    P.im_h = bp->im_h;
    P.a = bp->plane[0]; P.b = bp->plane[1]; P.c = bp->plane[2]; P.d = bp->plane[3];
    P.nrm = std::sqrt(P.a * P.a + P.b * P.b + P.c * P.c);
    DODT_REQUIRE(P.nrm > 0, "dodt_bev_slices: degenerate ground plane");
    for (int k = 0; k < 6; ++k) P.ext[k] = bp->extents[k];
    P.vs = vs;
    const double per_div = (bp->height_hi - bp->height_lo) / P.S;
    P.per_div = per_div;
    const double h0 = P.d / P.nrm;
    for (int s = 0; s < P.S; ++s) {
        const double lo = bp->height_lo + s * per_div;
        const double hi = lo + per_div;
        P.lo[s] = lo;
        P.d_lo[s] = P.d + (-lo);
        P.d_hi[s] = P.d + (-hi);
        P.quirk[s] = (float)((h0 - lo) / per_div);
    }
    P.dens_d_lo = P.d + (-bp->height_lo);
    P.dens_d_hi = P.d + (-bp->height_hi);
    P.occ_d_lo = P.d + (-bp->occ_lo);
    P.occ_d_hi = P.d + (-bp->occ_hi);
    for (int n = 0; n < 16; ++n)
        P.dens_table[n] = (float)std::fmin(1.0, std::log((double)n + 1.0) / std::log(16.0));
    {
        const int ox = 0 - P.cx_min, oz = 0 - P.cz_min;
        P.origin_off = (ox >= 0 && ox < P.X && oz >= 0 && oz < P.Z)
                           ? ((P.Z - 1 - oz) * P.X + ox) * (P.S + 1)
                           : -1;
    }

    const size_t cells = (size_t)P.X * P.Z * (P.S + 1);
    size_t cap = (size_t)3 * n_points;
    if (cap > cells) cap = cells;
    const size_t counters_bytes = 256;
    int rc = ctx->vox_ws.reserve(counters_bytes + (cap + 16) * sizeof(uint32_t));
    if (rc) return rc;
    uint32_t* counters = reinterpret_cast<uint32_t*>(ctx->vox_ws.ptr);
    uint32_t* list = counters + counters_bytes / sizeof(uint32_t);
    uint32_t* out = reinterpret_cast<uint32_t*>(d_bev_out);

    DODT_HIP_CHECK(hipMemsetAsync(out, 0, cells * sizeof(uint32_t), ctx->stream));
    DODT_HIP_CHECK(hipMemsetAsync(counters, 0, counters_bytes, ctx->stream));
    if (d_occ_bits_out)
        DODT_HIP_CHECK(hipMemsetAsync(d_occ_bits_out, 0,
                                      (size_t)P.Z * P.occ_words_per_row * sizeof(uint32_t),
                                      ctx->stream));
    if (n_points > 0) {
        hipLaunchKernelGGL(vox_scatter, dim3(dodt::ceil_div(n_points, 256)), dim3(256), 0,
                           ctx->stream, d_points, P, out, d_occ_bits_out, list, counters,
                           (uint32_t)cap);
        DODT_LAUNCH_CHECK();
    }
    const int fin = (int)cap + P.S;
    hipLaunchKernelGGL(vox_finalize, dim3(dodt::ceil_div(fin, 256)), dim3(256), 0, ctx->stream,
                       d_points, P, out, list, counters, (uint32_t)cap);
    DODT_LAUNCH_CHECK();
    return DODT_OK;
}

extern "C" int dodt_bev_support_mask(const dodt_bev_params* bp, int pad_top, uint8_t* mask, int rows, int cols) {
    DODT_REQUIRE(bp && mask, "dodt_bev_support_mask: NULL argument");
    DODT_REQUIRE(bp->point_format == DODT_PTS_VELO_XYZI,
                 "dodt_bev_support_mask: only velodyne points pass the frustum filter");
    DODT_REQUIRE(bp->voxel_size > 0 && pad_top >= 0, "dodt_bev_support_mask: bad voxel size or padding");
    const double vs = bp->voxel_size;
    const double minx = std::floor(bp->extents[0] / vs), maxx = std::ceil(bp->extents[1] / vs - 1);
    const double minz = std::floor(bp->extents[4] / vs), maxz = std::ceil(bp->extents[5] / vs - 1);
    const int X = (int)(maxx - minx + 1), Z = (int)(maxz - minz + 1);
    DODT_REQUIRE(X > 0 && Z > 0 && rows == pad_top + Z && cols == X,
                 "dodt_bev_support_mask: map is %dx%d, expected %dx%d", rows, cols, pad_top + Z, X);
    const double* p = bp->p2;
    const double ys[2] = {bp->extents[2], bp->extents[3]};
    std::vector<uint8_t> cell((size_t)rows * cols, 0);
    for (int zi = 0; zi < Z; ++zi) {
        const double zs[2] = {(zi + minz) * vs, (zi + minz + 1) * vs};
        for (int xi = 0; xi < X; ++xi) {
            const double xs[2] = {(xi + minx) * vs, (xi + minx + 1) * vs};
            bool maybe = false;
            double umin = INFINITY, umax = -INFINITY;
            for (int k = 0; k < 8; ++k) {
                const double x = xs[k & 1], y = ys[(k >> 1) & 1], z = zs[k >> 2];
                const double w = p[8] * x + p[9] * y + p[10] * z + p[11];
                if (!(w > 0.0)) { maybe = true; break; }
                const double u = (p[0] * x + p[1] * y + p[2] * z + p[3]) / w;
                umin = std::fmin(umin, u);
                umax = std::fmax(umax, u);
            }
            if (maybe || (umax > 0.0 && umin < bp->im_w)) cell[(size_t)(pad_top + Z - 1 - zi) * cols + xi] = 1;
        }
    }
    const int ox = 0 - (int)minx, oz = 0 - (int)minz;
    if (ox >= 0 && ox < X && oz >= 0 && oz < Z) cell[(size_t)(pad_top + Z - 1 - oz) * cols + ox] = 1;
    for (int r = 0; r < rows; ++r)
        for (int c = 0; c < cols; ++c) {
            uint8_t m = 0;
            for (int dr = -1; dr <= 1 && !m && r >= pad_top; ++dr)
                for (int dc = -1; dc <= 1 && !m; ++dc) {
                    const int rr = r + dr, cc = c + dc;
                    m = rr >= 0 && rr < rows && cc >= 0 && cc < cols && cell[(size_t)rr * cols + cc];
                }
            mask[(size_t)r * cols + c] = m;
        }
    return DODT_OK;
}

extern "C" int dodt_bev_status(dodt_ctx* ctx, int* flags) {
    DODT_REQUIRE(ctx && flags, "dodt_bev_status: NULL argument");
    *flags = 0;
    if (!ctx->vox_ws.ptr) return DODT_OK;
    uint32_t host[2] = {0, 0};
    DODT_HIP_CHECK(hipMemcpyAsync(host, ctx->vox_ws.ptr, sizeof(host), hipMemcpyDeviceToHost,
                                  ctx->stream));
    DODT_HIP_CHECK(hipStreamSynchronize(ctx->stream));
    *flags = (int)(host[kCntErr] & 3u);
    return DODT_OK;
}
```

dodt_amd/ops.py:

```python
import ctypes as C
import os

import numpy as np

from dodt_amd import _lib


def _arr(ctype, values):
    values = [float(v) for v in np.asarray(values, dtype=np.float64).reshape(-1)]
    return (ctype * len(values))(*values)


def _p(a):
    return None if a is None else C.c_void_p(a.ptr)


def make_bev_params(cfg, velo_to_cam=None, p2=None, im_wh=None,
                    point_format=_lib.PTS_VELO_XYZI, ground_plane=None,
                    area_extents=None, voxel_size=None):
    bp = _lib.BevParams()
    bp.point_format = point_format
    bp.num_slices = int(cfg['num_slices'])
    m = np.zeros(12) if velo_to_cam is None else \
        np.asarray(velo_to_cam, dtype=np.float64).reshape(-1)[:12]
# ... 53 lines not shown
                                          int(th), int(tw), items.ctypes.data, len(items),
                                          None if prev is None else prev.ctypes.data, run.ctypes.data, C.byref(n)),
               'dodt_frame_tables_host')
    return run[:n.value].copy()


def frame_lists_host(masks, layer, th, tw, items, prev=None, lib=None):
    lib = lib or _lib.load()
    masks = np.ascontiguousarray(masks, dtype=np.uint8)
    items = np.ascontiguousarray(items, dtype=np.int32).reshape(-1, 4)
    prev = None if prev is None else np.ascontiguousarray(prev, dtype=np.uint8)
    run = np.zeros((max(len(items), 1), 4), np.int32)
    restore = np.zeros((max(len(items), 1), 4), np.int32)
    n, nr = C.c_int(), C.c_int()
    _lib.check(lib.dodt_frame_lists_host(masks.ctypes.data, masks.shape[0], masks.shape[1], masks.shape[2], int(layer),
                                         int(th), int(tw), items.ctypes.data, len(items),
                                         None if prev is None else prev.ctypes.data, run.ctypes.data, C.byref(n),
                                         restore.ctypes.data, C.byref(nr)),
               'dodt_frame_lists_host')
    return run[:n.value].copy(), restore[:nr.value].copy()


def frame_restore_host(item, f, th, tw, bn, ch0, dst, src, dst2=None, src2=None, pad_top=-1, lib=None):
    lib = lib or _lib.load()
    for a in (dst, src, dst2, src2):
        assert a is None or (a.dtype == np.float32 and a.flags.c_contiguous)
    item = np.ascontiguousarray(item, dtype=np.int32)
    if pad_top < 0:
        rows, cols, channels = dst.shape[2], dst.shape[3], dst.shape[1] * 8
    else:
        rows, cols, channels = dst.shape[1] + pad_top, dst.shape[2], dst.shape[3]
    _lib.check(lib.dodt_frame_restore_host(item.ctypes.data, int(f), int(th), int(tw), int(bn), int(ch0), rows, cols,
                                           channels, int(pad_top), dst.ctypes.data, src.ctypes.data,
                                           None if dst2 is None else dst2.ctypes.data,
                                           None if src2 is None else src2.ctypes.data), 'dodt_frame_restore_host')


def bev_status(ctx):
    f = C.c_int()
    _lib.check(ctx.lib.dodt_bev_status(ctx.handle, C.byref(f)), 'dodt_bev_status')
    return f.value


def anchor_filter(ctx, d_occ_bits, nx, nz, d_cells, n_anchors, d_keep_idx, d_count,
                  density_threshold=1):
    _lib.check(ctx.lib.dodt_anchor_filter(
        ctx.handle, _p(d_occ_bits), int(nx), int(nz), _p(d_cells), int(n_anchors),
        int(density_threshold), _p(d_keep_idx), _p(d_count)), 'dodt_anchor_filter')


def project_anchors_f64(ctx, d_anchors, d_idx, n, d_n, bev_extents, p2, im_wh,
                        d_bev_norm=None, d_img_norm=None, d_anchors_f32=None):
    _lib.check(ctx.lib.dodt_project_anchors_f64(
        ctx.handle, _p(d_anchors), _p(d_idx), int(n), _p(d_n),
        _arr(C.c_double, bev_extents), _arr(C.c_double, p2),
        float(im_wh[0]), float(im_wh[1]), _p(d_bev_norm), _p(d_img_norm),
        _p(d_anchors_f32)), 'dodt_project_anchors_f64')


def project_anchors_f32(ctx, d_anchors, n, d_n, bev_extents, p2, im_wh,
                        d_bev=None, d_bev_norm_tf=None, d_img_norm_tf=None):
    _lib.check(ctx.lib.dodt_project_anchors_f32(
        ctx.handle, _p(d_anchors), int(n), _p(d_n), _arr(C.c_float, bev_extents),
        _arr(C.c_float, p2), float(im_wh[0]), float(im_wh[1]), _p(d_bev),
        _p(d_bev_norm_tf), _p(d_img_norm_tf)), 'dodt_project_anchors_f32')


def img_preprocess(ctx, d_img_u8, in_hw, out_hw, out_c, mean_rgb, d_out):
    _lib.check(ctx.lib.dodt_img_preprocess(
        ctx.handle, _p(d_img_u8), int(in_hw[0]), int(in_hw[1]), int(out_hw[0]),
        int(out_hw[1]), int(out_c), _arr(C.c_float, mean_rgb), _p(d_out)),
        'dodt_img_preprocess')


def crop_and_resize(ctx, d_image, hwc, d_boxes, n, d_n, crop_hw, d_out, out_box_stride=None):
    if out_box_stride is None:
        out_box_stride = int(crop_hw[0]) * int(crop_hw[1]) * int(hwc[2])
    _lib.check(ctx.lib.dodt_crop_and_resize_strided(
        ctx.handle, _p(d_image), int(hwc[0]), int(hwc[1]), int(hwc[2]), _p(d_boxes),
        int(n), _p(d_n), int(crop_hw[0]), int(crop_hw[1]), _p(d_out), int(out_box_stride)),
        'dodt_crop_and_resize')


def nms(ctx, d_boxes, d_scores, n, d_n, max_out, iou_threshold, d_sel, d_count):
    _lib.check(ctx.lib.dodt_nms(
        ctx.handle, _p(d_boxes), _p(d_scores), int(n), _p(d_n), int(max_out),
        float(iou_threshold), _p(d_sel), _p(d_count)), 'dodt_nms')


def offset_to_anchor(ctx, d_anchors, d_offsets, n, d_n, d_out):
    _lib.check(ctx.lib.dodt_offset_to_anchor(
        ctx.handle, _p(d_anchors), _p(d_offsets), int(n), _p(d_n), _p(d_out)),
        'dodt_offset_to_anchor')


def softmax_fg(ctx, d_logits, n, d_n, d_scores):
    _lib.check(ctx.lib.dodt_softmax_fg(
        ctx.handle, _p(d_logits), int(n), _p(d_n), _p(d_scores)), 'dodt_softmax_fg')


def rpn_decode(ctx, d_anchors, d_offsets, d_logits, n, d_n, bev_extents, d_regressed, d_bev_norm_tf, d_scores):
    _lib.check(ctx.lib.dodt_rpn_decode(
        ctx.handle, _p(d_anchors), _p(d_offsets), _p(d_logits), int(n), _p(d_n), _arr(C.c_float, bev_extents),
        _p(d_regressed), _p(d_bev_norm_tf), _p(d_scores)), 'dodt_rpn_decode')


def gather_project(ctx, d_src, d_idx, n, d_n, bev_extents, p2, im_wh, d_rows, d_bev_norm_tf, d_img_norm_tf):
    _lib.check(ctx.lib.dodt_gather_project(
        ctx.handle, _p(d_src), _p(d_idx), int(n), _p(d_n), _arr(C.c_float, bev_extents), _arr(C.c_float, p2),
        float(im_wh[0]), float(im_wh[1]), _p(d_rows), _p(d_bev_norm_tf), _p(d_img_norm_tf)), 'dodt_gather_project')


def final_decode(ctx, d_top_anchors, d_offsets, d_cls_logits, d_angle_vectors, n, d_n, plane, bev_extents,
                 d_boxes_3d, d_pred_anchors, d_bev_tf, d_nms_scores, d_det_scores, d_orientations):
    _lib.check(ctx.lib.dodt_final_decode(
        ctx.handle, _p(d_top_anchors), _p(d_offsets), _p(d_cls_logits), _p(d_angle_vectors), int(n), _p(d_n),
        _arr(C.c_float, plane), _arr(C.c_float, bev_extents), _p(d_boxes_3d), _p(d_pred_anchors), _p(d_bev_tf),
        _p(d_nms_scores), _p(d_det_scores), _p(d_orientations)), 'dodt_final_decode')


def gather_rows(ctx, d_src, width, d_idx, n, d_n, d_out):
    _lib.check(ctx.lib.dodt_gather_rows(
        ctx.handle, _p(d_src), int(width), _p(d_idx), int(n), _p(d_n), _p(d_out)),
        'dodt_gather_rows')


def box_4c_decode(ctx, d_top_anchors, d_offsets, n, d_n, plane, bev_extents,
                  d_boxes_3d=None, d_pred_anchors=None, d_bev_tf=None):
    _lib.check(ctx.lib.dodt_box_4c_decode(
        ctx.handle, _p(d_top_anchors), _p(d_offsets), int(n), _p(d_n),
        _arr(C.c_float, plane), _arr(C.c_float, bev_extents), _p(d_boxes_3d),
        _p(d_pred_anchors), _p(d_bev_tf)), 'dodt_box_4c_decode')


def max_fg_logit(ctx, d_logits, n_cls, n, d_n, d_scores):
    _lib.check(ctx.lib.dodt_max_fg_logit(
        ctx.handle, _p(d_logits), int(n_cls), int(n), _p(d_n), _p(d_scores)),
        'dodt_max_fg_logit')


def angle_vector_to_orientation(ctx, d_angle_vectors, n, d_n, d_orientations):
    _lib.check(ctx.lib.dodt_angle_vector_to_orientation(
        ctx.handle, _p(d_angle_vectors), int(n), _p(d_n), _p(d_orientations)),
        'dodt_angle_vector_to_orientation')


def pack_detections(ctx, d_boxes_3d, d_scores, d_sel, d_count, max_det, frame_mark,
                    d_rec, d_count_out, d_corr_offsets=None, d_orientations=None):
    _lib.check(ctx.lib.dodt_pack_detections(
        ctx.handle, _p(d_boxes_3d), _p(d_scores), _p(d_orientations), _p(d_corr_offsets),
        _p(d_sel), _p(d_count), int(max_det), float(frame_mark), _p(d_rec), _p(d_count_out)),
        'dodt_pack_detections')


def fetch_i32_begin(ctx, d_src, n, slot):
    _lib.check(ctx.lib.dodt_fetch_i32_begin(ctx.handle, _p(d_src), int(n), int(slot)),
               'dodt_fetch_i32_begin')


def fetch_i32_end(ctx, slot, n):
    buf = (C.c_int32 * n)()
    _lib.check(ctx.lib.dodt_fetch_i32_end(ctx.handle, int(slot), buf, int(n)),
               'dodt_fetch_i32_end')
    return list(buf)


def correlation(ctx, d_a, d_b, hwc, max_displacement, stride_2, pad, d_out):
    _lib.check(ctx.lib.dodt_correlation(
        ctx.handle, _p(d_a), _p(d_b), int(hwc[0]), int(hwc[1]), int(hwc[2]),
        int(max_displacement), int(stride_2), int(pad), _p(d_out)), 'dodt_correlation')


def mean_fusion(ctx, d_a, d_b, rows, d_n, row_floats, d_out):
    _lib.check(ctx.lib.dodt_mean_fusion(ctx.handle, _p(d_a), _p(d_b), int(rows), _p(d_n),
                                        int(row_floats), _p(d_out)), 'dodt_mean_fusion')


def rows_to_bf16(ctx, d_a, d_b, rows, d_n, row_floats, in_ld, d_out, out_ld):
    _lib.check(ctx.lib.dodt_rows_to_bf16(ctx.handle, _p(d_a), _p(d_b), int(rows), _p(d_n), int(row_floats),
                                         int(in_ld), _p(d_out), int(out_ld)), 'dodt_rows_to_bf16')


def bf16_to_float(a):
    return (np.asarray(a, np.uint16).astype(np.uint32) << 16).view(np.float32)


class FullyConnected(object):

    def __init__(self, ctx, w, b, relu, dtype='f32'):
        if dtype not in ('f32', 'bf16'):
            raise ValueError("dtype must be 'f32' or 'bf16'")
        w = np.ascontiguousarray(w, dtype=np.float32)
        b = np.ascontiguousarray(b, dtype=np.float32)
        if w.ndim != 2 or b.shape != (w.shape[1],):
            raise ValueError('weights must be (K,N) and bias (N,)')
        self.ctx, self.K, self.N, self.dtype = ctx, int(w.shape[0]), int(w.shape[1]), dtype
        h = C.c_void_p()
        flags = (_lib.FC_RELU if relu else 0) | (_lib.FC_BF16 if dtype == 'bf16' else 0)
        _lib.check(ctx.lib.dodt_fc_create_ex(ctx.handle, self.K, self.N,
                                             w.ctypes.data_as(C.c_void_p),
                                             b.ctypes.data_as(C.c_void_p), flags, C.byref(h)),
                   'dodt_fc_create_ex')
        self.handle = h

    def forward(self, d_x, M, d_y, ldx=None, ldy=None, d_x2=None, d_m=None, ctx=None):
        c = ctx or self.ctx
        _lib.check(c.lib.dodt_fc_forward(
            self.handle, c.handle, _p(d_x), _p(d_x2), int(self.K if ldx is None else ldx),
            int(M), _p(d_m), _p(d_y), int(self.N if ldy is None else ldy)), 'dodt_fc_forward')

    def can_split(self, ldx=None):
        return self.N <= 32 and self.K % 16 == 0 and \
            (self.K if ldx is None else ldx) % 4 == 0 and os.environ.get('DODT_FC_SKINNY') != '0'

    def forward_split(self, d_x, M, d_ys, widths, ldx=None, d_m=None, ctx=None):
        c = ctx or self.ctx
        w = (C.c_int * len(widths))(*[int(v) for v in widths])
        ys = (C.c_void_p * len(d_ys))(*[_p(y) for y in d_ys])
        _lib.check(c.lib.dodt_fc_forward_split(
            self.handle, c.handle, _p(d_x), int(self.K if ldx is None else ldx), int(M), _p(d_m),
            len(widths), w, ys), 'dodt_fc_forward_split')

    def bf16_row_elems(self):
        return int(self.ctx.lib.dodt_fc_bf16_row_elems(self.handle)) if self.dtype == 'bf16' else 0

    def forward_bf16(self, d_x, M, d_y, ldx, ldy=None, d_m=None, y_bf16=True, ctx=None):
        c = ctx or self.ctx
        _lib.check(c.lib.dodt_fc_forward_bf16(self.handle, c.handle, _p(d_x), int(ldx), int(M), _p(d_m), _p(d_y),
                                              int(self.N if ldy is None else ldy), 1 if y_bf16 else 0),
                   'dodt_fc_forward_bf16')

    def forward_split_bf16(self, d_x, M, d_ys, widths, ldx, d_m=None, ctx=None):
        c = ctx or self.ctx
        w = (C.c_int * len(widths))(*[int(v) for v in widths])
        ys = (C.c_void_p * len(d_ys))(*[_p(y) for y in d_ys])
        _lib.check(c.lib.dodt_fc_forward_split_bf16(
            self.handle, c.handle, _p(d_x), int(ldx), int(M), _p(d_m), len(widths), w, ys), 'dodt_fc_forward_split_bf16')

    def flops(self, M):
        return 2.0 * M * self.K * self.N

    def close(self):
        if self.handle is not None:
            self.ctx.lib.dodt_fc_destroy(self.handle)
            self.handle = None


def three_d_iou_matrix(ctx, d_a, na, d_b, nb, d_iou_out):
    _lib.check(ctx.lib.dodt_three_d_iou_matrix(ctx.handle, _p(d_a), int(na), _p(d_b), int(nb), _p(d_iou_out)),
               'dodt_three_d_iou_matrix')


def temporal_calib(r0_rect, tr_velo_to_cam):
    r0 = np.asarray(r0_rect, np.float64).reshape(3, 3)
    tr = np.asarray(tr_velo_to_cam, np.float64).reshape(3, 4)
    inv = np.zeros_like(tr)
    inv[0:3, 0:3] = np.transpose(tr[0:3, 0:3])
    inv[0:3, 3] = np.dot(-np.transpose(tr[0:3, 0:3]), tr[0:3, 3])
    return np.concatenate([np.linalg.inv(r0).reshape(-1), inv.reshape(-1), tr.reshape(-1), r0.reshape(-1)])


def temporal_ego(ego, n_frames):
    if len(ego) != n_frames - 1:
        raise ValueError('recovery needs one (trans, matrix, delta) per frame 1..n_frames-1')
    out = np.zeros((n_frames, 13))
    for i, (trans, matrix, delta) in enumerate(ego):
        out[i + 1, 0:3] = np.asarray(trans, np.float64).reshape(3)
        out[i + 1, 3:12] = np.linalg.inv(np.asarray(matrix, np.float64).reshape(3, 3)).reshape(-1)
        out[i + 1, 12] = float(delta)
    return out


def interpolate_pairs(ctx, d_records, d_counts, n_pairs, max_det, n_frames, threshold, on_conflict, d_out,
                      d_out_counts, d_status, d_recover=None, calib=None, max_out=None):
    if on_conflict not in ('raise', 'next_best'):
        raise ValueError("on_conflict must be 'raise' or 'next_best'")
    if d_records.dtype not in (np.float32, np.float64):
        raise ValueError('records must be float32 or float64')
    cal = None if calib is None else _arr(C.c_double, calib)
    _lib.check(ctx.lib.dodt_interpolate_pairs(
        ctx.handle, _p(d_records), int(d_records.dtype == np.float64), _p(d_counts), int(n_pairs), int(max_det),
        int(n_frames), float(threshold), _lib.CONFLICT_NEXT_BEST if on_conflict == 'next_best' else _lib.CONFLICT_RAISE,
        _p(d_recover), cal, int(2 * max_det if max_out is None else max_out), _p(d_out), _p(d_out_counts),
        _p(d_status)), 'dodt_interpolate_pairs')


def track_state_bytes(log_capacity):
    n = C.c_size_t()
    _lib.check(_lib.load().dodt_track_state_bytes(int(log_capacity), C.byref(n)), 'dodt_track_state_bytes')
    return int(n.value)


def track_reset(ctx, d_state, log_capacity):
# ... 32 lines not shown
```

dodt_amd/pipeline.py:

```python
import os

import numpy as np

from dodt_amd import config as _config
from dodt_amd import _lib, device, ops, tracking
from dodt_amd.core.anchor_generators import grid_anchor_3d_generator as gen
from dodt_amd.core.avod_fc_layers.fusion_fc_layers import EarlyFusionFcLayers
from dodt_amd.core.feature_extractors.vgg import BevVgg, ImgVgg
from dodt_amd.core.feature_extractors.vgg_pyramid import BevVggPyr, ImgVggPyr
from dodt_amd.core.models.anchor_predictor import AnchorPredictor
from dodt_amd.temporal import unpack_frames

EXTRACTORS = {'vgg_pyr': (BevVggPyr, ImgVggPyr), 'vgg': (BevVgg, ImgVgg)}

MAX_DET = 100
REC_COLS = 17
ROI = 7
CORR_MAX_DISP, CORR_STRIDE2, CORR_PAD = 5, 2, 5
CORR_CH = (2 * (CORR_MAX_DISP // CORR_STRIDE2) + 1) ** 2


class FramePairPipeline(object):

    def __init__(self, ctx, cfg, bev_params, img_params, p2=_config.KITTI_P2,
# ... 411 lines not shown

    def _frame_ids(self, frame_ids):
        if frame_ids is not None:
            ids = [tuple(f) for f in frame_ids]
            return lambda pair, kf: ids[pair][kf]
        tau = self.temporal['n_frames'] - 1 if self.temporal is not None else 1
        return lambda pair, kf: pair * tau + kf * tau

    def tracks_so_far(self, frame_ids=None):
        if self.tracker is None:
            raise ValueError('tracks_so_far: the pipeline has no tracker')
        self.ctx.wait_for(self.img_ctx)
        return tracking.tracks_from_log(self.track_state.read(), self._frame_ids(frame_ids), self.tracker['classes'])

    def end_sequence(self, frame_ids=None):
        if self.tracker is None:
            raise ValueError('end_sequence: the pipeline has no tracker')
        if self.pending is not None:
            raise ValueError('end_sequence: call finish() first (the last step is not tracked yet)')
        self.track_state.flush(ctx=self.img_ctx)
        tracks = self.tracks_so_far(frame_ids)
        self.track_state.reset(ctx=self.img_ctx)
        self.last_sequence_tracks = tracks
        return tracks

    def kitti_tracking_rows(self, tracks=None):
        from dodt_amd.core.dt_evaluator_utils import convert_trajectory_to_kitti_format
        if tracks is None:
            if self.tracker is None or self.last_sequence_tracks is None:
                raise ValueError('kitti_tracking_rows: no sequence has ended')
            tracks = self.last_sequence_tracks
        return convert_trajectory_to_kitti_format(tracks)

    def frames(self):
        if self.temporal is None:
            raise ValueError('frames: the pipeline has no temporal module')
        self.ctx.wait_for(self.img_ctx)
        return unpack_frames(self.d_frames.download(), self.d_frame_counts.download(),
                             self.d_frame_status.download(), self.temporal['on_conflict'])

    CONV_DONE_MARK = 250
    CORR_MAP_MARK = 248

    def _corr_on_img(self):
        return (self.rpn_head is not None and self.fps == 2 and len(self.sides) >= 2
                and not os.environ.get('DODT_PIPE_NO_CORR') and os.environ.get('DODT_PIPE_CORR_ON_F1', '1') != '0'
                and os.environ.get('DODT_PIPE_CORR_MAP', 'img') == 'img')

    def _wait_convs(self, st):
        if self.early_prep:
            for s in self._streams(st['cur'])[0]:
                s.wait_mark(self.ctx, self.CONV_DONE_MARK + st['cur'])
                s.wait_mark(self.img_ctx, self.CONV_DONE_MARK + st['cur'])

    def _tail(self, st):
        cfg, nf = self.cfg, self.nf
        cur = st['cur']
        sides, preps = self._streams(cur)
        ns = len(sides)
        head_scratch = self.head_scratch_sets[cur % len(self.stream_sets)] if self.rpn_head is not None else None
        fr, feat = self.fr2[cur], self.feat[cur]
        heads = st['heads']
        k3 = st['step'] % 3
        counts = [ops.fetch_i32_end(preps[f % ns], 3 * f + k3, 1)[0]
                  for f in range(nf)]
        self.last_anchor_counts = counts
        fr = [dict(b, **p) for b, p in zip(fr, self.prep3[k3])]
        self.fr = fr
        self.d_records, self.d_rec_counts = self.rec2[st['rslot']], self.cnt2[st['rslot']]
        self.d_bev_in = self._views(self.in_bev[cur], (self.bev_h, self.bev_w, self.cfg['bev_depth']), self.bev_pad)
        bev_px = self.bev_fh * self.bev_fw
        img_px = self.img_fh * self.img_fw
        FC = self.feat_c
        bev_hw, img_hw = (self.bev_fh, self.bev_fw), (self.img_fh, self.img_fw)
        plane = cfg['ground_plane']
        if os.environ.get('DODT_PIPE_NO_TAIL'):
            return
        if self.on_records_reuse is not None:
            self.on_records_reuse(st['rslot'], sides)
        computed = heads is None
        split_t = computed and self.fps == 2 and ns >= 2 and not os.environ.get('DODT_PIPE_NO_CORR') \
            and os.environ.get('DODT_PIPE_CORR_ON_F1', '1') != '0'
        corr_img = split_t and self._corr_on_img()
        fused_tail = os.environ.get('DODT_PIPE_FUSED_TAIL', '1') != '0'

        def t_branch_crops(cc, f0, scratch):
            fb0 = feat['bev_feat'].offset(4 * bev_px * FC * f0, bev_hw + (FC,))
            fb1 = feat['bev_feat'].offset(4 * bev_px * FC * (f0 + 1), bev_hw + (FC,))
            ops.correlation(cc, fb0, fb1, bev_hw + (FC,), CORR_MAX_DISP, CORR_STRIDE2, CORR_PAD,
                            scratch['corr_map'])
            ops.crop_and_resize(cc, scratch['corr_map'], bev_hw + (CORR_CH,), fr[f0]['top_bev'], self.P,
                                fr[f0]['top_count'], (ROI, ROI), fr[f0]['corr_rois'],
                                out_box_stride=self.corr_head.in_ld)

        def frame(f):
            c, b, A = sides[f % ns], fr[f], counts[f]
            h = b if computed else heads[f]
            scratch = head_scratch[f % ns] if computed else None
            self._mark(c, st['step'], 'tail%d_start' % f)
            bneck_b = feat['bev_bneck'].offset(4 * bev_px * f, bev_hw + (1,))
            bneck_i = feat['img_bneck'].offset(4 * img_px * f, img_hw + (1,))
            feat_b = feat['bev_feat'].offset(4 * bev_px * FC * f, bev_hw + (FC,))
            feat_i = feat['img_feat'].offset(4 * img_px * FC * f, img_hw + (FC,))
            ops.crop_and_resize(c, bneck_b, bev_hw + (1,), b['bev_norm'], A, None,
                                (3, 3), b['rpn_bev_roi'])
            ops.crop_and_resize(c, bneck_i, img_hw + (1,), b['img_norm'], A, None,
                                (3, 3), b['rpn_img_roi'])
            self._mark(c, st['step'], 'tail%d_crops' % f)
            if computed and not os.environ.get('DODT_PIPE_NO_RPN'):
                self.rpn_head.forward(c, b['rpn_bev_roi'], b['rpn_img_roi'], A, b['rpn_logits'],
                                      b['rpn_offsets'], scratch['rpn'])
            self._mark(c, st['step'], 'tail%d_rpn' % f)
            if fused_tail:
                ops.rpn_decode(c, b['anchors'], h['rpn_offsets'], h['rpn_logits'], A, None, self.bev_extents_flat,
                               b['regressed'], b['prop_bev'], b['scores'])
            else:
                ops.offset_to_anchor(c, b['anchors'], h['rpn_offsets'], A, None, b['regressed'])
                ops.project_anchors_f32(c, b['regressed'], A, None, self.bev_extents_flat, self.p2,
                                        self.image_wh, d_bev_norm_tf=b['prop_bev'])
                ops.softmax_fg(c, h['rpn_logits'], A, None, b['scores'])
            ops.nms(c, b['prop_bev'], b['scores'], A, None, self.P,
                    cfg['rpn_nms_iou_thresh'], b['top_idx'], b['top_count'])
            if fused_tail:
                ops.gather_project(c, b['regressed'], b['top_idx'], self.P, b['top_count'], self.bev_extents_flat,
                                   self.p2, self.image_wh, b['top_anchors'], b['top_bev'], b['top_img'])
                self._mark(c, st['step'], 'tail%d_nms1' % f)
            else:
                ops.gather_rows(c, b['regressed'], 6, b['top_idx'], self.P, b['top_count'],
                                b['top_anchors'])
                self._mark(c, st['step'], 'tail%d_nms1' % f)
                ops.project_anchors_f32(c, b['top_anchors'], self.P, b['top_count'],
                                        self.bev_extents_flat, self.p2, self.image_wh,
                                        d_bev_norm_tf=b['top_bev'], d_img_norm_tf=b['top_img'])
            ops.crop_and_resize(c, feat_b, bev_hw + (FC,), b['top_bev'], self.P,
                                b['top_count'], (ROI, ROI), b['bev_rois'])
            ops.crop_and_resize(c, feat_i, img_hw + (FC,), b['top_img'], self.P,
                                b['top_count'], (ROI, ROI), b['img_rois'])
            yield 'crops'
            pair = self.fps == 2
            corr_offsets = h.get('corr_offsets') if pair and f % 2 == 0 else None
            self._mark(c, st['step'], 'tail%d_crops2' % f)
            if computed:
                self.avod_head.forward(c, b['bev_rois'], b['img_rois'], self.P, b['top_count'],
                                       [b['cls_logits'], b['offsets_4c']]
                                       + ([b['angle_vectors']] if self.box_4ca else []),
                                       scratch['fc'])
                self._mark(c, st['step'], 'tail%d_fc2' % f)
                yield 'head'
                if pair and f % 2 == 0 and not os.environ.get('DODT_PIPE_NO_CORR'):
                    if corr_img:
                        pass
                    else:
                        if split_t:
                            c.wait_mark(sides[(f + 1) % ns], self.CORR_ROIS_MARK)
                        else:
                            t_branch_crops(c, f, scratch)
                        self._mark(c, st['step'], 'tail%d_corrmap' % f)
                        self.corr_head.forward(c, b['corr_rois'], None, self.P, b['top_count'],
                                               [b['corr_offsets']], scratch['fc'])
            self._mark(c, st['step'], 'tail%d_heads' % f)
            if fused_tail:
                ops.final_decode(c, b['top_anchors'], h['offsets_4c'], h['cls_logits'],
                                 h['angle_vectors'] if self.box_4ca else None, self.P, b['top_count'], plane,
                                 self.bev_extents_flat, b['boxes_3d'], b['pred_anchors'], b['nms2_boxes'],
                                 b['nms2_scores'], b['det_scores'], b['orientations'] if self.box_4ca else None)
                ops.nms(c, b['nms2_boxes'], b['nms2_scores'], self.P, b['top_count'], MAX_DET,
                        cfg['avod_nms_iou_thresh'], b['det_idx'], b['det_count'])
            else:
                ops.box_4c_decode(c, b['top_anchors'], h['offsets_4c'], self.P, b['top_count'],
                                  plane, self.bev_extents_flat, b['boxes_3d'], b['pred_anchors'],
                                  b['nms2_boxes'])
                ops.max_fg_logit(c, h['cls_logits'], 2, self.P, b['top_count'], b['nms2_scores'])
                ops.nms(c, b['nms2_boxes'], b['nms2_scores'], self.P, b['top_count'], MAX_DET,
                        cfg['avod_nms_iou_thresh'], b['det_idx'], b['det_count'])
                ops.softmax_fg(c, h['cls_logits'], self.P, b['top_count'], b['det_scores'])
                if self.box_4ca:
                    ops.angle_vector_to_orientation(c, h['angle_vectors'], self.P, b['top_count'],
                                                    b['orientations'])
            yield 'pack'
            ops.pack_detections(
                c, b['boxes_3d'], b['det_scores'], b['det_idx'], b['det_count'], MAX_DET,
                float(f % self.fps),
                self.d_records.offset(4 * MAX_DET * REC_COLS * f, (MAX_DET, REC_COLS)),
                self.d_rec_counts.offset(4 * f, (1,), np.int32), d_corr_offsets=corr_offsets,
                d_orientations=b['orientations'] if self.box_4ca else None)
            self._mark(c, st['step'], 'tail%d_end' % f)

        def drain(g):
            for _ in g:
                pass

        if not split_t:
            for f in range(nf):
                drain(frame(f))
            return
        for f0 in range(0, nf, 2):
            c0, c1 = sides[f0 % ns], sides[(f0 + 1) % ns]
            g0, g1 = frame(f0), frame(f0 + 1)
            while next(g0) != 'crops':
                pass
            c0.mark(self.PROPOSALS_MARK)
            if corr_img:
                while next(g0) != 'pack':
                    pass
                while next(g1) != 'crops':
                    pass
                c1.wait_mark(c0, self.PROPOSALS_MARK)
                c1.wait_mark(self.img_ctx, self.CORR_MAP_MARK + cur)
                ops.crop_and_resize(c1, self.corr_maps[cur][f0 // 2], bev_hw + (CORR_CH,), fr[f0]['top_bev'], self.P,
                                    fr[f0]['top_count'], (ROI, ROI), fr[f0]['corr_rois'],
                                    out_box_stride=self.corr_head.in_ld)
                self.corr_head.forward(c1, fr[f0]['corr_rois'], None, self.P, fr[f0]['top_count'],
                                       [fr[f0]['corr_offsets']], head_scratch[(f0 + 1) % ns]['fc'])
                c1.mark(self.CORR_ROIS_MARK)
                c0.wait_mark(c1, self.CORR_ROIS_MARK)
                drain(g0)
                drain(g1)
                continue
            while next(g0) != 'head':
                pass
            while next(g1) != 'crops':
                pass
            c1.wait_mark(c0, self.PROPOSALS_MARK)
            t_branch_crops(c1, f0, head_scratch[(f0 + 1) % ns])
            c1.mark(self.CORR_ROIS_MARK)
            drain(g1)
            drain(g0)

    PROPOSALS_MARK, CORR_ROIS_MARK = 252, 253
# ... 32 lines not shown
```

include/dodt_hip.h:

```cpp
#ifndef DODT_HIP_H
#define DODT_HIP_H

#include <stddef.h>
#include <stdint.h>

#ifdef __cplusplus
extern "C" {
#endif

#define DODT_OK 0
#define DODT_ERR_INVALID 1
#define DODT_ERR_HIP 2
#define DODT_ERR_UNSUPPORTED 3

typedef struct dodt_ctx dodt_ctx;

int dodt_version(void);
const char* dodt_last_error(void);
int dodt_ctx_create(int device_id, dodt_ctx** out);
int dodt_ctx_create_high_priority(int device_id, dodt_ctx** out);
int dodt_ctx_create_on_stream(int device_id, void* hip_stream, dodt_ctx** out);
int dodt_ctx_destroy(dodt_ctx* ctx);
int dodt_ctx_sync(dodt_ctx* ctx);
int dodt_mark(dodt_ctx* ctx, int slot);
// ... 43 lines not shown

int dodt_anchor_filter(dodt_ctx* ctx, const uint32_t* d_occ_bits, int nx, int nz,
                       const int32_t* d_anchor_cells, int n_anchors,
                       int density_threshold, int32_t* d_keep_idx_out,
                       int32_t* d_count_out);

int dodt_project_anchors_f64(dodt_ctx* ctx, const double* d_anchors,
                             const int32_t* d_idx, int n, const int32_t* d_n,
                             const double bev_extents[4], const double p2[12],
                             double im_w, double im_h, float* d_bev_norm_out,
                             float* d_img_norm_out, float* d_anchors_f32_out);

int dodt_project_anchors_f32(dodt_ctx* ctx, const float* d_anchors, int n,
                             const int32_t* d_n, const float bev_extents[4],
                             const float p2[12], float im_w, float im_h,
                             float* d_bev_out, float* d_bev_norm_tf_out,
                             float* d_img_norm_tf_out);

int dodt_img_preprocess(dodt_ctx* ctx, const uint8_t* d_img_u8, int in_h, int in_w,
                        int out_h, int out_w, int out_c, const float mean_rgb[3],
                        float* d_out);

typedef struct dodt_extractor dodt_extractor;
#define DODT_EXTRACTOR_VGG_PYR 0
#define DODT_EXTRACTOR_VGG 1
#define DODT_EXTRACTOR_SHARED_GPU 0x100
#define DODT_EXTRACTOR_BF16 0x200
#define DODT_EXTRACTOR_SPLIT 0x400
#define DODT_CONV_MODE_DEFAULT 2
int dodt_conv_mode(void);
int dodt_extractor_create(dodt_ctx* ctx, int kind, int in_h, int in_w, int in_c,
                          int pad_top, int batch, dodt_extractor** out);
int dodt_extractor_destroy(dodt_extractor* ex);
int dodt_extractor_set_layer(dodt_extractor* ex, const char* name, const float* w,
                             int kh, int kw, int c_a, int c_b, const float* beta,
                             const float* mean, const float* var);
int dodt_extractor_input(dodt_extractor* ex, float** d_ptr, long long* frame_stride_floats);
int dodt_extractor_forward(dodt_extractor* ex, const float* d_in, float* d_feat_out,
                           float* d_bottleneck_out);
int dodt_extractor_forward_padded(dodt_extractor* ex, const float* d_x0, float* d_feat_out,
                                  float* d_bottleneck_out);
int dodt_extractor_set_input(dodt_extractor* ex, const float* d_x0);
int dodt_extractor_set_input_support(dodt_extractor* ex, const uint8_t* mask, int rows, int cols,
                                     long long* skipped_items);
int dodt_extractor_set_frame_tables(dodt_extractor* ex, int on, int* enabled);
int dodt_extractor_frame_items(dodt_extractor* ex, int* items, int n);
int dodt_extractor_frame_split(dodt_extractor* ex, int* computed, int* restored, int n);
long long dodt_extractor_store_bytes(const dodt_extractor* ex);
int dodt_frame_tables_host(const uint8_t* masks, int frames, int rows, int cols, int layer, int th, int tw,
                           const int* items, int n_items, const uint8_t* prev, int* run, int* n_run);
int dodt_frame_lists_host(const uint8_t* masks, int frames, int rows, int cols, int layer, int th, int tw,
                          const int* items, int n_items, const uint8_t* prev, int* run, int* n_run, int* restore,
                          int* n_restore);
int dodt_frame_restore_host(const int* item, int f, int th, int tw, int bn, int ch0, int rows, int cols, int channels,
                            int pad_top, float* dst, const float* src, float* dst2, const float* src2);
int dodt_extractor_output_shape(const dodt_extractor* ex, int* h, int* w, int* c);
int dodt_extractor_first_layers_folded(const dodt_extractor* ex);
int dodt_extractor_read_activation(dodt_extractor* ex, const char* name, float* dst,
                                   int* h, int* w, int* c);
double dodt_extractor_flops(const dodt_extractor* ex);
double dodt_extractor_mfma_flops(const dodt_extractor* ex);
double dodt_extractor_bytes(const dodt_extractor* ex);
typedef struct dodt_layer_info {
    char name[32];
    char kernel[48];
    int32_t launches;
    int32_t items;
    double flops_direct;
    double flops_executed;
    double bytes;
    float ms;
    int32_t reserved_;
} dodt_layer_info;
int dodt_extractor_layer_count(const dodt_extractor* ex);
int dodt_extractor_forward_timed(dodt_extractor* ex, const float* d_in, float* d_feat_out,
                                 float* d_bottleneck_out, dodt_layer_info* info, int n_info);

int dodt_crop_and_resize(dodt_ctx* ctx, const float* d_image, int H, int W, int C,
                         const float* d_boxes, int n, const int32_t* d_n, int crop_h,
                         int crop_w, float* d_out);
int dodt_crop_and_resize_strided(dodt_ctx* ctx, const float* d_image, int H, int W, int C,
                                 const float* d_boxes, int n, const int32_t* d_n, int crop_h,
                                 int crop_w, float* d_out, long long out_box_stride);

int dodt_correlation(dodt_ctx* ctx, const float* d_a, const float* d_b, int H, int W, int C,
                     int max_displacement, int stride_2, int pad, float* d_out);

int dodt_mean_fusion(dodt_ctx* ctx, const float* d_a, const float* d_b, int rows, const int32_t* d_n,
                     int row_floats, float* d_out);
typedef struct dodt_fc dodt_fc;
int dodt_fc_create(dodt_ctx* ctx, int K, int N, const float* w, const float* bias, int relu,
                   dodt_fc** out);
#define DODT_FC_RELU 1
#define DODT_FC_BF16 2
int dodt_fc_create_ex(dodt_ctx* ctx, int K, int N, const float* w, const float* bias, int flags,
                      dodt_fc** out);
int dodt_fc_destroy(dodt_fc* fc);
int dodt_fc_forward(dodt_fc* fc, dodt_ctx* ctx, const float* d_x, const float* d_x2, int ldx,
                    int M, const int32_t* d_m, float* d_y, int ldy);
int dodt_fc_forward_split(dodt_fc* fc, dodt_ctx* ctx, const float* d_x, int ldx, int M, const int32_t* d_m,
                          int parts, const int* widths, float* const* d_ys);
int dodt_fc_bf16_row_elems(const dodt_fc* fc);
int dodt_fc_forward_bf16(dodt_fc* fc, dodt_ctx* ctx, const void* d_x_bf16, int ldx, int M, const int32_t* d_m,
                         void* d_y, int ldy, int y_bf16);
int dodt_fc_forward_split_bf16(dodt_fc* fc, dodt_ctx* ctx, const void* d_x_bf16, int ldx, int M, const int32_t* d_m,
                               int parts, const int* widths, float* const* d_ys);
int dodt_rows_to_bf16(dodt_ctx* ctx, const float* d_a, const float* d_b, int rows, const int32_t* d_n,
                      int row_floats, int in_ld, void* d_out_bf16, int out_ld);
double dodt_fc_flops(const dodt_fc* fc, int M);

int dodt_nms(dodt_ctx* ctx, const float* d_boxes, const float* d_scores, int n,
             const int32_t* d_n, int max_out, float iou_threshold, int32_t* d_sel_out,
             int32_t* d_count_out);

int dodt_offset_to_anchor(dodt_ctx* ctx, const float* d_anchors, const float* d_offsets,
                          int n, const int32_t* d_n, float* d_out);
int dodt_softmax_fg(dodt_ctx* ctx, const float* d_logits2, int n, const int32_t* d_n,
                    float* d_scores_out);
int dodt_rpn_decode(dodt_ctx* ctx, const float* d_anchors, const float* d_offsets, const float* d_logits2, int n,
                    const int32_t* d_n, const float bev_extents[4], float* d_regressed_out,
                    float* d_bev_norm_tf_out, float* d_scores_out);
int dodt_gather_project(dodt_ctx* ctx, const float* d_src, const int32_t* d_idx, int n, const int32_t* d_n,
                        const float bev_extents[4], const float p2[12], float im_w, float im_h,
                        float* d_rows_out, float* d_bev_norm_tf_out, float* d_img_norm_tf_out);
int dodt_final_decode(dodt_ctx* ctx, const float* d_top_anchors, const float* d_offsets, const float* d_cls_logits2,
                      const float* d_angle_vectors, int n, const int32_t* d_n, const float plane[4],
                      const float bev_extents[4], float* d_boxes_3d_out, float* d_pred_anchors_out,
                      float* d_bev_tf_out, float* d_nms_scores_out, float* d_det_scores_out,
                      float* d_orientations_out);
int dodt_gather_rows(dodt_ctx* ctx, const float* d_src, int width, const int32_t* d_idx,
                     int n, const int32_t* d_n, float* d_out);
int dodt_max_fg_logit(dodt_ctx* ctx, const float* d_logits, int n_cls, int n,
                      const int32_t* d_n, float* d_scores_out);
int dodt_angle_vector_to_orientation(dodt_ctx* ctx, const float* d_angle_vectors, int n,
                                     const int32_t* d_n, float* d_orientations_out);
int dodt_pack_detections(dodt_ctx* ctx, const float* d_boxes_3d, const float* d_scores,
                         const float* d_orientations, const float* d_corr_offsets,
                         const int32_t* d_sel, const int32_t* d_count, int max_det,
                         float frame_mark, float* d_rec_out, int32_t* d_count_out);
int dodt_box_4c_decode(dodt_ctx* ctx, const float* d_top_anchors, const float* d_offsets,
                       int n, const int32_t* d_n, const float plane[4],
                       const float bev_extents[4], float* d_boxes_3d_out,
                       float* d_pred_anchors_out, float* d_bev_tf_out);

int dodt_three_d_iou_matrix(dodt_ctx* ctx, const double* d_a, int na, const double* d_b, int nb,
                            double* d_iou_out);
#define DODT_CONFLICT_RAISE 0
#define DODT_CONFLICT_NEXT_BEST 1
int dodt_interpolate_pairs(dodt_ctx* ctx, const void* d_records, int records_f64, const int32_t* d_counts,
                           int n_pairs, int max_det, int n_frames, double threshold, int on_conflict,
                           const double* d_recover, const double* calib, int max_out, double* d_out,
                           int32_t* d_out_counts, int32_t* d_status);

int dodt_track_state_bytes(int log_capacity, size_t* bytes);
int dodt_track_reset(dodt_ctx* ctx, void* d_state, int log_capacity);
int dodt_track_flush(dodt_ctx* ctx, void* d_state, double high_threshold, int t_min);
int dodt_track_encode(dodt_ctx* ctx, const void* d_records, int records_f64, const int32_t* d_counts,
                      int n_pairs, int max_det, const double* p2, double image_w, double image_h,
                      double score_threshold, float* d_track_out, float* d_ious_out, int32_t* d_counts_out);
int dodt_track_pairs(dodt_ctx* ctx, void* d_state, const void* d_records, int records_f64,
                     const int32_t* d_counts, int n_pairs, int max_det, const double* p2, double image_w,
                     double image_h, double score_threshold, double high_threshold, double iou_threshold,
                     int t_min);
int dodt_track_encoded(dodt_ctx* ctx, void* d_state, const float* d_track, const float* d_ious,
                       const int32_t* d_counts, int n_pairs, int max_rows, double high_threshold,
                       double iou_threshold, int t_min);

typedef struct dodt_comm dodt_comm;
#define DODT_COMM_ID_BYTES 128
int dodt_comm_unique_id(uint8_t* id_out);
int dodt_comm_create(dodt_ctx* ctx, int rank, int world, const uint8_t* id, dodt_comm** out);
int dodt_comm_destroy(dodt_comm* comm);
int dodt_comm_attach(dodt_comm* comm, dodt_ctx* ctx);
int dodt_comm_rank(const dodt_comm* comm, int* rank, int* world);
int dodt_comm_set_late_peer(dodt_comm* comm, double microseconds);
int dodt_all_gather_records(dodt_comm* comm, dodt_ctx* producer, int slot, const float* d_records,
                            const int32_t* d_counts, int pairs, int frames, int max_det, int cols,
                            float* d_all_records, int32_t* d_all_counts);
int dodt_comm_join(dodt_comm* comm, int slot, dodt_ctx* consumer);
int dodt_comm_sync(dodt_comm* comm);
int dodt_comm_barrier(dodt_comm* comm);
int dodt_comm_max_f64(dodt_comm* comm, double* value);
// ... 6 lines not shown
```

Measured before the change: 388.1.

## Fuse RPN crop+fc6, pair cls7/reg7 GEMMs, and fuse ROI crop pair with mean

Adds three fused paths for the per-frame tail. The two 3x3 RPN bottleneck crops, their mean and the K=9 fc6 layer now run in one rpn_front kernel. The cls7 and reg7 layers, which share a shape, run as one paired DMA GEMM launch. The BEV and image ROI crops are done in one kernel that also writes the mean-fused rows, so the FC head skips its separate mean_fusion launch. The aim is fewer kernel launches and less intermediate traffic, in exchange for more code paths and a new default tail mode (2) that enables them.

```diff
diff --git a/dodt_amd/_lib.py b/dodt_amd/_lib.py
--- a/dodt_amd/_lib.py
+++ b/dodt_amd/_lib.py
@@ -123,6 +123,8 @@
                                   _pf]),
     'dodt_crop_and_resize_strided': (_i, [_vp, _pf, _i, _i, _i, _pf, _i, _pi32, _i, _i, _pf,
                                           C.c_longlong]),
+    'dodt_crop_pair': (_i, [_vp, _pf, _i, _i, _pf, _i, _i, _i, _pf, _pf, _i, _pi32, _i, _i, _pf, _pf, C.c_longlong, _pf,
+                            C.c_longlong]),
     'dodt_correlation': (_i, [_vp, _pf, _pf, _i, _i, _i, _i, _i, _i, _pf]),
     'dodt_mean_fusion': (_i, [_vp, _pf, _pf, _i, _pi32, _i, _pf]),
     'dodt_fc_create': (_i, [_vp, _i, _i, _hf, _hf, _i, C.POINTER(_vp)]),
@@ -130,6 +132,8 @@
     'dodt_fc_destroy': (_i, [_vp]),
     'dodt_fc_forward': (_i, [_vp, _vp, _pf, _pf, _i, _i, _pi32, _pf, _i]),
     'dodt_fc_forward_split': (_i, [_vp, _vp, _pf, _i, _i, _pi32, _i, C.POINTER(_i), C.POINTER(_vp)]),
+    'dodt_fc_forward_pair': (_i, [_vp, _vp, _vp, _pf, _pf, _i, _i, _pi32, _pf, _pf, _i]),
+    'dodt_rpn_front': (_i, [_vp, _vp, _pf, _i, _i, _pf, _i, _i, _pf, _pf, _i, _pi32, _pf, _pf, _pf, _i]),
     'dodt_fc_flops': (_d, [_vp, _i]),
     'dodt_fc_bf16_row_elems': (_i, [_vp]),
     'dodt_fc_forward_bf16': (_i, [_vp, _vp, _vp, _i, _i, _pi32, _vp, _i, _i]),
diff --git a/dodt_amd/core/avod_fc_layers/fusion_fc_layers.py b/dodt_amd/core/avod_fc_layers/fusion_fc_layers.py
--- a/dodt_amd/core/avod_fc_layers/fusion_fc_layers.py
+++ b/dodt_amd/core/avod_fc_layers/fusion_fc_layers.py
@@ -47,8 +47,15 @@
                  [self.ctx.zeros((n_max, self.in_ld16), np.uint16)]
         return s
 
-    def forward(self, ctx, d_rois, d_rois2, n, d_n, d_outs, scratch):
+    def mean_rows(self, scratch):
+        if self.bf16_rows and len(scratch) > 5:
+            return None
+        return scratch[2] if len(scratch) > 2 and self.in_ld == self.in_k and self.in_k % 4 == 0 else None
+
+    def forward(self, ctx, d_rois, d_rois2, n, d_n, d_outs, scratch, mean_done=False):
         x, x2 = d_rois, d_rois2
+        if mean_done and (x2 is None or self.mean_rows(scratch) is None):
+            raise ValueError('mean_done: this head takes no precomputed mean rows (mean_rows() is None)')
         ldx = self._row_floats(d_rois, n, 'd_rois')
         if x2 is not None and self._row_floats(x2, n, 'd_rois2') != ldx:
             raise ValueError('d_rois and d_rois2 must have the same row layout')
@@ -72,7 +79,8 @@
                 self._packed_first = ops.FullyConnected(self.ctx, w, b, True, dtype=dtype)
             first = self._packed_first
         if x2 is not None and len(scratch) > 2 and ldx == self.in_ld == self.in_k and self.in_k % 4 == 0:
-            ops.mean_fusion(ctx, x, x2, n, d_n, self.in_ld, scratch[2])
+            if not mean_done:
+                ops.mean_fusion(ctx, x, x2, n, d_n, self.in_ld, scratch[2])
             x, x2 = scratch[2], None
         for i, l in enumerate([first] + self.hidden[1:]):
             y = scratch[i & 1]
diff --git a/dodt_amd/core/models/anchor_predictor.py b/dodt_amd/core/models/anchor_predictor.py
--- a/dodt_amd/core/models/anchor_predictor.py
+++ b/dodt_amd/core/models/anchor_predictor.py
@@ -33,18 +33,29 @@
     def make_scratch(self, n_max):
         return [self.ctx.empty((n_max, 2 * self.width), np.float32) for _ in range(2)]
 
-    def forward(self, ctx, d_bev_roi, d_img_roi, n, d_objectness, d_offsets, scratch):
+    def forward(self, ctx, d_bev_roi, d_img_roi, n, d_objectness, d_offsets, scratch, maps=None, fused=True):
         w = self.width
         h6, h7 = scratch
-        self.fc6.forward(d_bev_roi, n, h6, d_x2=d_img_roi, ctx=ctx)
-        self.cls7.forward(h6, n, h7, ldx=2 * w, ldy=2 * w, ctx=ctx)
-        self.reg7.forward(h6.offset(4 * w, (1,)), n, h7.offset(4 * w, (1,)),
-                          ldx=2 * w, ldy=2 * w, ctx=ctx)
+        if maps is not None:
+            map_b, hw_b, map_i, hw_i, boxes_b, boxes_i = maps
+            self.fc6.rpn_front(map_b, hw_b, map_i, hw_i, boxes_b, boxes_i, n, d_bev_roi, d_img_roi, h6, ctx=ctx)
+        else:
+            self.fc6.forward(d_bev_roi, n, h6, d_x2=d_img_roi, ctx=ctx)
+        if fused and self.cls7.can_pair(self.reg7, ldx=2 * w):
+            self.cls7.forward_pair(self.reg7, h6, h6.offset(4 * w, (1,)), n, h7, h7.offset(4 * w, (1,)),
+                                   ldx=2 * w, ldy=2 * w, ctx=ctx)
+        else:
+            self.cls7.forward(h6, n, h7, ldx=2 * w, ldy=2 * w, ctx=ctx)
+            self.reg7.forward(h6.offset(4 * w, (1,)), n, h7.offset(4 * w, (1,)),
+                              ldx=2 * w, ldy=2 * w, ctx=ctx)
         if self.out8 is not None:
             self.out8.forward_split(h7, n, [d_objectness, d_offsets], [self.cls8.N, self.reg8.N], ctx=ctx)
             return
         self.cls8.forward(h7, n, d_objectness, ldx=2 * w, ctx=ctx)
         self.reg8.forward(h7.offset(4 * w, (1,)), n, d_offsets, ldx=2 * w, ctx=ctx)
+
+    def can_front(self):
+        return self.fc6.can_front()
 
     def flops(self, n):
         return sum(l.flops(n) for l in self.layers)
diff --git a/dodt_amd/csrc/crop.hip b/dodt_amd/csrc/crop.hip
--- a/dodt_amd/csrc/crop.hip
+++ b/dodt_amd/csrc/crop.hip
@@ -1,4 +1,5 @@
 #include "common.h"
+#include "crop_sample.h"
 
 namespace {
 
@@ -47,6 +48,37 @@
     }
 }
 
+template <int VEC>
+__global__ void __launch_bounds__(256)
+crop_pair_kernel(const float* __restrict__ img_a, int Ha, int Wa, const float* __restrict__ img_b, int Hb, int Wb,
+                 int C, const float* __restrict__ boxes_a, const float* __restrict__ boxes_b, int n,
+                 const int* __restrict__ d_n, int ch, int cw, float* __restrict__ out_a, float* __restrict__ out_b,
+                 long long out_stride, float* __restrict__ mean, long long mean_stride) {
+    const int groups = C / VEC;
+    const long long t = (long long)blockIdx.x * blockDim.x + threadIdx.x;
+    const int lim = d_n ? min(*d_n, n) : n;
+    const long long total = (long long)lim * ch * cw * groups;
+    if (t >= total) return;
+    const int g = (int)(t % groups);
+    long long r = t / groups;
+    const int ix = (int)(r % cw); r /= cw;
+    const int iy = (int)(r % ch);
+    const int b = (int)(r / ch);
+    float va[VEC], vb[VEC];
+    dodt::crop_sample<VEC>(img_a, Ha, Wa, C, reinterpret_cast<const float4*>(boxes_a)[b], iy, ix, g, ch, cw, va);
+    dodt::crop_sample<VEC>(img_b, Hb, Wb, C, reinterpret_cast<const float4*>(boxes_b)[b], iy, ix, g, ch, cw, vb);
+    const size_t in_box = ((size_t)iy * cw + ix) * C + (size_t)g * VEC;
+    float* oa = out_a + (size_t)b * out_stride + in_box;
+    float* ob = out_b + (size_t)b * out_stride + in_box;
+#pragma unroll
+    for (int k = 0; k < VEC; ++k) { oa[k] = va[k]; ob[k] = vb[k]; }
+    if (mean) {
+        float* om = mean + (size_t)b * mean_stride + in_box;
+#pragma unroll
+        for (int k = 0; k < VEC; ++k) om[k] = (va[k] + vb[k]) / 2.0f;
+    }
+}
+
 }
 
 extern "C" int dodt_crop_and_resize(dodt_ctx* ctx, const float* d_image, int H, int W, int C,
@@ -78,3 +110,30 @@
     DODT_LAUNCH_CHECK();
     return DODT_OK;
 }
+
+extern "C" int dodt_crop_pair(dodt_ctx* ctx, const float* d_image_a, int Ha, int Wa, const float* d_image_b, int Hb,
+                              int Wb, int C, const float* d_boxes_a, const float* d_boxes_b, int n,
+                              const int32_t* d_n, int crop_h, int crop_w, float* d_out_a, float* d_out_b,
+                              long long out_box_stride, float* d_mean, long long mean_stride) {
+    DODT_REQUIRE(ctx && d_image_a && d_image_b && d_out_a && d_out_b && (n == 0 || (d_boxes_a && d_boxes_b)),
+                 "dodt_crop_pair: NULL argument");
+    DODT_REQUIRE(Ha > 0 && Wa > 0 && Hb > 0 && Wb > 0 && C > 0 && crop_h > 0 && crop_w > 0 && n >= 0,
+                 "dodt_crop_pair: bad sizes");
+    const long long crop = (long long)crop_h * crop_w * C;
+    DODT_REQUIRE(out_box_stride >= crop, "dodt_crop_pair: output stride %lld shorter than a crop", out_box_stride);
+    DODT_REQUIRE(!d_mean || mean_stride >= crop, "dodt_crop_pair: mean stride %lld shorter than a crop", mean_stride);
+    if (n == 0) return DODT_OK;
+    const int vec = (C % 4 == 0 && out_box_stride % 4 == 0 && (!d_mean || mean_stride % 4 == 0)) ? 4 : 1;
+    const long long total = (long long)n * crop_h * crop_w * (C / vec);
+    const int blocks = (int)((total + 255) / 256);
+    if (vec == 4)
+        hipLaunchKernelGGL(crop_pair_kernel<4>, dim3(blocks), dim3(256), 0, ctx->stream, d_image_a, Ha, Wa, d_image_b,
+                           Hb, Wb, C, d_boxes_a, d_boxes_b, n, d_n, crop_h, crop_w, d_out_a, d_out_b, out_box_stride,
+                           d_mean, mean_stride);
+    else
+        hipLaunchKernelGGL(crop_pair_kernel<1>, dim3(blocks), dim3(256), 0, ctx->stream, d_image_a, Ha, Wa, d_image_b,
+                           Hb, Wb, C, d_boxes_a, d_boxes_b, n, d_n, crop_h, crop_w, d_out_a, d_out_b, out_box_stride,
+                           d_mean, mean_stride);
+    DODT_LAUNCH_CHECK();
+    return DODT_OK;
+}
diff --git a/dodt_amd/csrc/crop_sample.h b/dodt_amd/csrc/crop_sample.h
--- /dev/null
+++ b/dodt_amd/csrc/crop_sample.h
@@ -0,0 +1,37 @@
+#pragma once
+#include "common.h"
+
+namespace dodt {
+
+template <int VEC>
+__device__ __forceinline__ void crop_sample(const float* __restrict__ img, int H, int W, int C, const float4 bx,
+                                            int iy, int ix, int g, int ch, int cw, float (&v)[VEC]) {
+    const float y1 = bx.x, x1 = bx.y, y2 = bx.z, x2 = bx.w;
+    const float hm1 = (float)(H - 1), wm1 = (float)(W - 1);
+    const float hs = (ch > 1) ? (y2 - y1) * hm1 / (float)(ch - 1) : 0.0f;
+    const float ws = (cw > 1) ? (x2 - x1) * wm1 / (float)(cw - 1) : 0.0f;
+    const float in_y = (ch > 1) ? y1 * hm1 + (float)iy * hs : 0.5f * (y1 + y2) * hm1;
+    const float in_x = (cw > 1) ? x1 * wm1 + (float)ix * ws : 0.5f * (x1 + x2) * wm1;
+    const bool ok = (in_y >= 0.0f) && (in_y <= hm1) && (in_x >= 0.0f) && (in_x <= wm1);
+    if (!ok) {
+#pragma unroll
+        for (int k = 0; k < VEC; ++k) v[k] = 0.0f;
+        return;
+    }
+    const int ty = (int)floorf(in_y), by = (int)ceilf(in_y);
+    const int lx_i = (int)floorf(in_x), rx_i = (int)ceilf(in_x);
+    const float ly = in_y - (float)ty, lx = in_x - (float)lx_i;
+    const float* ptl = img + ((size_t)ty * W + lx_i) * C + (size_t)g * VEC;
+    const float* ptr = img + ((size_t)ty * W + rx_i) * C + (size_t)g * VEC;
+    const float* pbl = img + ((size_t)by * W + lx_i) * C + (size_t)g * VEC;
+    const float* pbr = img + ((size_t)by * W + rx_i) * C + (size_t)g * VEC;
+#pragma unroll
+    for (int k = 0; k < VEC; ++k) {
+        const float tl = ptl[k], tr = ptr[k], bl = pbl[k], br = pbr[k];
+        const float top = tl + (tr - tl) * lx;
+        const float bot = bl + (br - bl) * lx;
+        v[k] = top + (bot - top) * ly;
+    }
+}
+
+}
diff --git a/dodt_amd/csrc/gemm.hip b/dodt_amd/csrc/gemm.hip
--- a/dodt_amd/csrc/gemm.hip
+++ b/dodt_amd/csrc/gemm.hip
@@ -8,6 +8,7 @@
 #include <algorithm>
 
 #include "common.h"
+#include "crop_sample.h"
 #include "lds_dma.h"
 
 namespace {
@@ -273,8 +274,7 @@
 constexpr int kDmaXFloats = kDmaBM * kDmaBK;
 
 template <bool FUSE, int NT>
-__global__ void __launch_bounds__(256, 2)
-fc_dma_kernel(const GemmArgs a, int tiles_m, int tiles_n) {
+__device__ __forceinline__ void fc_dma_body(const GemmArgs& a, int tiles_m, int tiles_n, const int bid) {
     constexpr int kDmaBN = 64 * NT, kDmaWFloats = kDmaBK * kDmaBN;
     using dodt::blds16;
     using dodt::i32x4_t;
@@ -287,8 +287,8 @@
     const int wm = wave >> 1, wn = wave & 1;
     const int li = lane & 31, lh = lane >> 5;
     const int T = tiles_m * tiles_n;
-    int tile = blockIdx.x;
-    if (T % 8 == 0) tile = (int)(blockIdx.x % 8) * (T / 8) + (int)(blockIdx.x / 8);
+    int tile = bid;
+    if (T % 8 == 0) tile = (int)(bid % 8) * (T / 8) + (int)(bid / 8);
     const int mt = tile / tiles_n, nt0 = tile % tiles_n;
     const int m0 = mt * kDmaBM;
     const int M = a.d_m ? min(*a.d_m, a.M) : a.M;
@@ -388,7 +388,7 @@
     };
     issue(0, 0);
     if (nstages > 1) issue(1, 1);
-    const bool probe = a.clock_probe != nullptr && blockIdx.x == 17 && tid == 0;
+    const bool probe = a.clock_probe != nullptr && bid == 17 && tid == 0;
     unsigned long long c0 = 0, r0 = 0;
     if (probe) { c0 = __builtin_amdgcn_s_memtime(); r0 = __builtin_amdgcn_s_memrealtime(); }
     for (int st = 0; st < nstages; st += 3) {
@@ -414,6 +414,20 @@
             }
         }
     }
+}
+
+template <bool FUSE, int NT>
+__global__ void __launch_bounds__(256, 2)
+fc_dma_kernel(const GemmArgs a, int tiles_m, int tiles_n) {
+    fc_dma_body<FUSE, NT>(a, tiles_m, tiles_n, (int)blockIdx.x);
+}
+
+template <int NT>
+__global__ void __launch_bounds__(256, 2)
+fc_dma_pair_kernel(const GemmArgs a, const GemmArgs b, int tiles_m, int tiles_n) {
+    const int T = tiles_m * tiles_n;
+    const bool second = (int)blockIdx.x >= T;
+    fc_dma_body<false, NT>(second ? b : a, tiles_m, tiles_n, (int)blockIdx.x - (second ? T : 0));
 }
 
 int launch_fc_dma(hipStream_t s, const GemmArgs& a_in, int Npad) {
@@ -457,6 +471,33 @@
             fprintf(stderr, "[dodt] fc_dma_kernel M %d K %d N %d: K loop of workgroup 17: %llu shader cycles in %.2f us = %.3f GHz\n",
                     a.M, a.K, a.N, h[0], h[1] / 100.0, (double)h[0] / h[1] * 0.1);
     }
+    return DODT_OK;
+}
+
+bool fc_dma_ok(int BN, int K, const GemmArgs& a) {
+    static const bool dma = !(getenv("DODT_FC_DMA") && atoi(getenv("DODT_FC_DMA")) == 0);
+    return BN == 128 && dma && K % kDmaBK == 0 && a.ldx % 4 == 0 && K >= 2 * kDmaBK && ((size_t)a.x % 16 == 0) &&
+           (!a.x2 || (size_t)a.x2 % 16 == 0);
+}
+
+int launch_fc_dma_pair(hipStream_t s, const GemmArgs& a, const GemmArgs& b, int Npad) {
+    static const int force_nt = getenv("DODT_FC_NT") ? atoi(getenv("DODT_FC_NT")) : 0;
+    const int nt = force_nt ? force_nt : ((long)dodt::ceil_div(a.M, kDmaBM) * (Npad / 128) >= 2 * 256 ? 2 : 1);
+    const int tiles_m = dodt::ceil_div(a.M, kDmaBM), tiles_n = Npad / (64 * nt);
+    const size_t lds = (size_t)kDmaStages * (kDmaXFloats + kDmaBK * 64 * nt) * 4;
+    static const hipError_t attr1 = hipFuncSetAttribute(reinterpret_cast<const void*>(&fc_dma_pair_kernel<1>),
+                                                        hipFuncAttributeMaxDynamicSharedMemorySize,
+                                                        kDmaStages * (kDmaXFloats + kDmaBK * 64) * 4);
+    static const hipError_t attr2 = hipFuncSetAttribute(reinterpret_cast<const void*>(&fc_dma_pair_kernel<2>),
+                                                        hipFuncAttributeMaxDynamicSharedMemorySize,
+                                                        kDmaStages * (kDmaXFloats + kDmaBK * 128) * 4);
+    DODT_HIP_CHECK(attr1);
+    DODT_HIP_CHECK(attr2);
+    if (nt == 2)
+        hipLaunchKernelGGL(fc_dma_pair_kernel<2>, dim3(2 * tiles_m * tiles_n), dim3(256), lds, s, a, b, tiles_m, tiles_n);
+    else
+        hipLaunchKernelGGL(fc_dma_pair_kernel<1>, dim3(2 * tiles_m * tiles_n), dim3(256), lds, s, a, b, tiles_m, tiles_n);
+    DODT_LAUNCH_CHECK();
     return DODT_OK;
 }
 
@@ -776,6 +817,52 @@
     return DODT_OK;
 }
 
+constexpr int kFrontAnchors = 16, kFrontK = 9;
+
+__global__ void __launch_bounds__(256)
+rpn_front_kernel(const float* __restrict__ map_a, int Ha, int Wa, const float* __restrict__ map_b, int Hb, int Wb,
+                 const float* __restrict__ boxes_a, const float* __restrict__ boxes_b, int n, const int* __restrict__ d_n,
+                 float* __restrict__ roi_a, float* __restrict__ roi_b, const float* __restrict__ w_plain,
+                 const float* __restrict__ bias, int N, int relu, float* __restrict__ y, int ldy) {
+    __shared__ float s_x[kFrontAnchors * kFrontK];
+    const int M = d_n ? min(*d_n, n) : n;
+    const int m0 = blockIdx.x * kFrontAnchors;
+    if (m0 >= M) return;
+    const int tid = threadIdx.x;
+    if (tid < kFrontAnchors * kFrontK) {
+        const int g = tid / kFrontK, k = tid - g * kFrontK, m = m0 + g;
+        if (m < M) {
+            const int iy = k / 3, ix = k - iy * 3;
+            float va[1], vb[1];
+            dodt::crop_sample<1>(map_a, Ha, Wa, 1, reinterpret_cast<const float4*>(boxes_a)[m], iy, ix, 0, 3, 3, va);
+            dodt::crop_sample<1>(map_b, Hb, Wb, 1, reinterpret_cast<const float4*>(boxes_b)[m], iy, ix, 0, 3, 3, vb);
+            roi_a[(size_t)m * kFrontK + k] = va[0];
+            roi_b[(size_t)m * kFrontK + k] = vb[0];
+            s_x[tid] = (va[0] + vb[0]) / 2.0f;
+        }
+    }
+    __syncthreads();
+    const int n4 = N >> 2;
+    const int rows = min(kFrontAnchors, M - m0);
+    for (int it = tid; it < rows * n4; it += 256) {
+        const int g = it / n4, c = (it - g * n4) * 4;
+        f32x4 acc = {0.f, 0.f, 0.f, 0.f};
+#pragma unroll
+        for (int k = 0; k < kFrontK; ++k) {
+            const float xv = s_x[g * kFrontK + k];
+            const f32x4 wv = *reinterpret_cast<const f32x4*>(w_plain + (size_t)k * N + c);
+            acc += wv * xv;
+        }
+        const f32x4 b = *reinterpret_cast<const f32x4*>(bias + c);
+        acc += b;
+        if (relu) {
+#pragma unroll
+            for (int i = 0; i < 4; ++i) acc[i] = fmaxf(acc[i], 0.0f);
+        }
+        *reinterpret_cast<f32x4*>(y + (size_t)(m0 + g) * ldy + c) = acc;
+    }
+}
+
 }
 
 namespace {
@@ -990,10 +1077,7 @@
         return launch_fc<128, 32, 4, 1, 32, 64, true>(s, a, f->Npad);
     }
     if (f->BN == 128) {
-        static const bool dma = !(getenv("DODT_FC_DMA") && atoi(getenv("DODT_FC_DMA")) == 0);
-        if (dma && f->K % kDmaBK == 0 && ldx % 4 == 0 && f->K >= 2 * kDmaBK &&
-            ((size_t)d_x % 16 == 0) && (!d_x2 || (size_t)d_x2 % 16 == 0))
-            return launch_fc_dma(s, a, f->Npad);
+        if (fc_dma_ok(f->BN, f->K, a)) return launch_fc_dma(s, a, f->Npad);
         static const int tile = getenv("DODT_FC_TILE") ? atoi(getenv("DODT_FC_TILE")) : 0;
         if (tile == 256) return launch_fc<128, 128, 2, 2, 128, 32>(s, a, f->Npad);
         if (tile == 64) return launch_fc<64, 64, 2, 2, 128>(s, a, f->Npad);
@@ -1001,6 +1085,44 @@
         return launch_fc<64, 128, 2, 2, 128, 64>(s, a, f->Npad);
     }
     return launch_fc<128, 32, 4, 1>(s, a, f->Npad);
+}
+
+int dodt_rpn_front(dodt_fc* f, dodt_ctx* ctx, const float* d_map_a, int Ha, int Wa, const float* d_map_b, int Hb, int Wb,
+                   const float* d_boxes_a, const float* d_boxes_b, int n, const int32_t* d_n, float* d_roi_a,
+                   float* d_roi_b, float* d_y, int ldy) {
+    DODT_REQUIRE(f && d_map_a && d_map_b && d_roi_a && d_roi_b && d_y && (n == 0 || (d_boxes_a && d_boxes_b)),
+                 "dodt_rpn_front: NULL argument");
+    DODT_REQUIRE(Ha > 0 && Wa > 0 && Hb > 0 && Wb > 0 && n >= 0 && ldy >= f->N, "dodt_rpn_front: bad sizes");
+    if (f->K != kFrontK || f->bf16 || !f->d_w_plain || f->N % 4 != 0 || ldy % 4 != 0 || (size_t)d_y % 16 != 0) {
+        dodt::set_error("dodt_rpn_front: an fp32 layer with K = 9 (3x3x1 crops) and N %% 4 == 0 into 16-byte aligned rows only");
+        return DODT_ERR_UNSUPPORTED;
+    }
+    if (n == 0) return DODT_OK;
+    hipLaunchKernelGGL(rpn_front_kernel, dim3(dodt::ceil_div(n, kFrontAnchors)), dim3(256), 0,
+                       (ctx ? ctx : f->ctx)->stream, d_map_a, Ha, Wa, d_map_b, Hb, Wb, d_boxes_a, d_boxes_b, n, d_n,
+                       d_roi_a, d_roi_b, f->d_w_plain, f->d_b, f->N, f->relu, d_y, ldy);
+    DODT_LAUNCH_CHECK();
+    return DODT_OK;
+}
+
+int dodt_fc_forward_pair(dodt_fc* fa, dodt_fc* fb, dodt_ctx* ctx, const float* d_xa, const float* d_xb, int ldx, int M,
+                         const int32_t* d_m, float* d_ya, float* d_yb, int ldy) {
+    DODT_REQUIRE(fa && fb && d_xa && d_xb && d_ya && d_yb, "dodt_fc_forward_pair: NULL argument");
+    DODT_REQUIRE(M >= 0 && ldx >= fa->K && ldy >= fa->N, "dodt_fc_forward_pair: bad strides");
+    GemmArgs a, b;
+    a.x = d_xa; a.x2 = nullptr; a.w = fa->d_w; a.bias = fa->d_b; a.y = d_ya;
+    a.M = M; a.K = fa->K; a.Kp = fa->Kp; a.N = fa->N; a.ldx = ldx; a.ldy = ldy; a.relu = fa->relu;
+    a.d_m = d_m;
+    b = a;
+    b.x = d_xb; b.w = fb->d_w; b.bias = fb->d_b; b.y = d_yb; b.relu = fb->relu;
+    if (fa->K != fb->K || fa->N != fb->N || fa->bf16 || fb->bf16 || !fc_dma_ok(fa->BN, fa->K, a) ||
+        !fc_dma_ok(fb->BN, fb->K, b)) {
+        dodt::set_error("dodt_fc_forward_pair: two fp32 layers of one size that dodt_fc_forward runs on the LDS-DMA "
+                        "kernel only (N >= 128, K %% 32 == 0, K >= 64, 16-byte aligned rows)");
+        return DODT_ERR_UNSUPPORTED;
+    }
+    if (M == 0) return DODT_OK;
+    return launch_fc_dma_pair((ctx ? ctx : fa->ctx)->stream, a, b, fa->Npad);
 }
 
 int dodt_fc_forward_split(dodt_fc* f, dodt_ctx* ctx, const float* d_x, int ldx, int M, const int32_t* d_m,
diff --git a/dodt_amd/csrc/nms.hip b/dodt_amd/csrc/nms.hip
--- a/dodt_amd/csrc/nms.hip
+++ b/dodt_amd/csrc/nms.hip
@@ -1,4 +1,6 @@
 #include "common.h"
+
+#include <cstdlib>
 
 namespace {
 
@@ -125,6 +127,46 @@
     if (i < st->n_eff) {
         idx = i;
         row = rank[i];
+        const float4 b = reinterpret_cast<const float4*>(boxes)[i];
+        ymin = fminf(b.x, b.z); ymax = fmaxf(b.x, b.z);
+        xmin = fminf(b.y, b.w); xmax = fmaxf(b.y, b.w);
+        area = (ymax - ymin) * (xmax - xmin);
+    }
+    float* o = sb + (size_t)row * 5;
+    o[0] = ymin; o[1] = xmin; o[2] = ymax; o[3] = xmax; o[4] = area;
+    sorted_idx[row] = idx;
+}
+
+__device__ __forceinline__ unsigned long long nms_key(const float* __restrict__ scores, int i, int n_eff) {
+    return i < n_eff ? ((unsigned long long)(~ordered_bits(scores[i])) << 32) | (uint32_t)i : ~0ull;
+}
+
+__global__ void __launch_bounds__(256)
+nms_order_kernel(const float* __restrict__ boxes, const float* __restrict__ scores, int n,
+                 const int* __restrict__ d_n, int n_rows, int nb, NmsState* __restrict__ st,
+                 unsigned long long* __restrict__ removed, float* __restrict__ sb, int* __restrict__ sorted_idx) {
+    __shared__ __attribute__((aligned(16))) unsigned long long s_seg[kRankSeg];
+    const int i = blockIdx.x * 256 + threadIdx.x;
+    const int n_eff = d_n ? min(*d_n, n) : n;
+    if (i == 0) { st->count = 0; st->done = (n_eff <= 0); st->n_eff = n_eff; }
+    if (i < nb) removed[i] = 0ull;
+    int cnt = 0;
+    if (blockIdx.x * 256 < n_eff) {
+        const unsigned long long mine = nms_key(scores, i, n_eff);
+        for (int j0 = 0; j0 < n_eff; j0 += kRankSeg) {
+            __syncthreads();
+            for (int t = threadIdx.x; t < kRankSeg; t += 256) s_seg[t] = nms_key(scores, j0 + t, n_eff);
+            __syncthreads();
+#pragma unroll 16
+            for (int j = 0; j < kRankSeg; ++j) cnt += (s_seg[j] < mine) ? 1 : 0;
+        }
+    }
+    if (i >= n_rows) return;
+    float ymin = 0, xmin = 0, ymax = 0, xmax = 0, area = -1.0f;
+    int idx = -1, row = i;
+    if (i < n_eff) {
+        idx = i;
+        row = cnt;
         const float4 b = reinterpret_cast<const float4*>(boxes)[i];
         ymin = fminf(b.x, b.z); ymax = fmaxf(b.x, b.z);
         xmin = fminf(b.y, b.w); xmax = fmaxf(b.y, b.w);
@@ -341,6 +383,134 @@
     }
 }
 
+constexpr int kOneMax = 2048;
+
+__global__ void __launch_bounds__(1024)
+nms_one_kernel(const float* __restrict__ boxes, const float* __restrict__ scores, int n,
+               const int* __restrict__ d_n, float thr, int max_out, int* __restrict__ sel_out,
+               int* __restrict__ count_out) {
+    __shared__ __attribute__((aligned(16))) float s_raw[kOneMax * 6];
+    __shared__ unsigned long long s_removed[kOneMax / 64], s_cols[64], s_sel;
+    __shared__ int s_count, s_done;
+    const int tid = threadIdx.x, lane = tid & 63, wave = tid >> 6;
+    const int n_eff = d_n ? min(*d_n, n) : n;
+    if (n_eff <= 0) {
+        if (tid == 0) *count_out = 0;
+        return;
+    }
+    int np = 2;
+    while (np < n_eff) np <<= 1;
+    unsigned long long* const s_keys = reinterpret_cast<unsigned long long*>(s_raw);
+    for (int t = tid; t < np; t += 1024) s_keys[t] = nms_key(scores, t, n_eff);
+    __syncthreads();
+    for (int k = 2; k <= np; k <<= 1) {
+        for (int j = k >> 1; j > 0; j >>= 1) {
+            for (int t = tid; t < np / 2; t += 1024) {
+                const int lo = ((t & ~(j - 1)) << 1) | (t & (j - 1));
+                const int hi = lo + j;
+                unsigned long long a = s_keys[lo], b = s_keys[hi];
+                cmp_swap(a, b, (lo & k) == 0);
+                s_keys[lo] = a;
+                s_keys[hi] = b;
+            }
+            __syncthreads();
+        }
+    }
+    const int nbk = (n_eff + 63) >> 6;
+    unsigned long long kk[kOneMax / 1024];
+#pragma unroll
+    for (int q = 0; q < kOneMax / 1024; ++q) kk[q] = (tid + 1024 * q < np) ? s_keys[tid + 1024 * q] : ~0ull;
+    __syncthreads();
+    float* const s_y0 = s_raw;
+    float* const s_x0 = s_raw + kOneMax;
+    float* const s_y1 = s_raw + 2 * kOneMax;
+    float* const s_x1 = s_raw + 3 * kOneMax;
+    float* const s_ar = s_raw + 4 * kOneMax;
+    int* const s_idx = reinterpret_cast<int*>(s_raw + 5 * kOneMax);
+#pragma unroll
+    for (int q = 0; q < kOneMax / 1024; ++q) {
+        const int r = tid + 1024 * q;
+        if (r >= nbk * 64) continue;
+        float ymin = 0, xmin = 0, ymax = 0, xmax = 0, area = -1.0f;
+        int idx = -1;
+        if (r < n_eff) {
+            idx = (int)(kk[q] & 0xFFFFFFFFull);
+            const float4 b = reinterpret_cast<const float4*>(boxes)[idx];
+            ymin = fminf(b.x, b.z); ymax = fmaxf(b.x, b.z);
+            xmin = fminf(b.y, b.w); xmax = fmaxf(b.y, b.w);
+            area = (ymax - ymin) * (xmax - xmin);
+        }
+        s_y0[r] = ymin; s_x0[r] = xmin; s_y1[r] = ymax; s_x1[r] = xmax; s_ar[r] = area;
+        s_idx[r] = idx;
+    }
+    if (tid < kOneMax / 64) s_removed[tid] = 0ull;
+    if (tid == 0) { s_count = 0; s_done = 0; }
+    __syncthreads();
+
+    for (int b = 0; b < nbk; ++b) {
+        if (tid < 64) s_cols[tid] = 0ull;
+        __syncthreads();
+        {
+            const int col = b * 64 + lane;
+            const float cy0 = s_y0[col], cx0 = s_x0[col], cy1 = s_y1[col], cx1 = s_x1[col], ca = s_ar[col];
+            unsigned long long bits = 0ull;
+#pragma unroll
+            for (int q = 0; q < 4; ++q) {
+                const int r = wave * 4 + q, row = b * 64 + r;
+                const bool hit = (col > row) && iou_gt(s_y0[row], s_x0[row], s_y1[row], s_x1[row], s_ar[row],
+                                                       cy0, cx0, cy1, cx1, ca, thr);
+                bits |= hit ? (1ull << r) : 0ull;
+            }
+            if (bits) atomicOr(&s_cols[lane], bits);
+        }
+        __syncthreads();
+        if (tid < 64) {
+            const int row = b * 64 + lane;
+            const unsigned long long cols = s_cols[lane];
+            const int valid = min(64, n_eff - b * 64);
+            unsigned long long init = ~s_removed[b];
+            if (valid < 64) init &= (1ull << valid) - 1ull;
+            const bool mine = (init >> lane) & 1ull;
+            unsigned long long alive = __ballot(mine);
+            for (;;) {
+                const unsigned long long na = __ballot(mine && (cols & alive) == 0ull);
+                if (na == alive) break;
+                alive = na;
+            }
+            const int cnt0 = __builtin_amdgcn_readfirstlane(s_count);
+            const int room = max_out - cnt0;
+            const unsigned long long below = (1ull << lane) - 1ull;
+            unsigned long long sel = alive;
+            if (__popcll(sel) > room)
+                sel = __ballot(((sel >> lane) & 1ull) && __popcll(sel & below) < room);
+            const int cnt = cnt0 + __popcll(sel);
+            if ((sel >> lane) & 1ull) sel_out[cnt0 + __popcll(sel & below)] = s_idx[row];
+            if (lane == 0) {
+                s_sel = sel;
+                s_count = cnt;
+                if (cnt >= max_out) s_done = 1;
+            }
+        }
+        __syncthreads();
+        const unsigned long long sel = s_sel;
+        if (s_done) break;
+        if (sel != 0ull) {
+            for (int c = b + 1 + wave; c < nbk; c += 16) {
+                const int col = c * 64 + lane;
+                const float cy0 = s_y0[col], cx0 = s_x0[col], cy1 = s_y1[col], cx1 = s_x1[col], ca = s_ar[col];
+                bool hit = false;
+                for (unsigned long long m = sel; m != 0ull; m &= m - 1ull) {
+                    const int row = b * 64 + __builtin_ctzll(m);
+                    hit = hit || iou_gt(s_y0[row], s_x0[row], s_y1[row], s_x1[row], s_ar[row], cy0, cx0, cy1, cx1, ca, thr);
+                }
+                const unsigned long long w = __ballot(hit);
+                if (lane == 0 && w) s_removed[c] |= w;
+            }
+        }
+    }
+    if (tid == 0) *count_out = s_count;
+}
+
 int next_pow2(int v) {
     int p = 1;
     while (p < v) p <<= 1;
@@ -363,6 +533,13 @@
     const int n_pad = next_pow2(n < 2 ? 2 : n);
     const int nb = dodt::ceil_div(n, 64);
     const int n_rows = nb * 64;
+    static const bool fused = !(getenv("DODT_NMS_FUSED") && atoi(getenv("DODT_NMS_FUSED")) == 0);
+    if (fused && n_rows <= kOneMax) {
+        hipLaunchKernelGGL(nms_one_kernel, dim3(1), dim3(1024), 0, ctx->stream, d_boxes, d_scores, n, d_n,
+                           iou_threshold, max_out, d_sel_out, d_count_out);
+        DODT_LAUNCH_CHECK();
+        return DODT_OK;
+    }
     const bool ranked = n <= kRankMax;
     const int later_rows = nb <= 1024 ? 2 * kChunkRows : kChunkRows;
     int first_rows = (int)dodt::align_up((size_t)max_out + (size_t)max_out / 8, 64) + 64;
@@ -393,10 +570,17 @@
     hipStream_t s = ctx->stream;
 
     const int init_n = n_pad > nb ? n_pad : nb;
-    hipLaunchKernelGGL(nms_keys_kernel, dim3(dodt::ceil_div(init_n, 256)), dim3(256), 0, s,
-                       d_scores, n, d_n, n_pad, keys, st, removed, nb, ranked ? rank : (int*)nullptr);
-    DODT_LAUNCH_CHECK();
-    if (ranked) {
+    if (ranked && fused) {
+        hipLaunchKernelGGL(nms_order_kernel, dim3(n_rows / 256 + 1), dim3(256), 0, s, d_boxes, d_scores, n, d_n,
+                           n_rows, nb, st, removed, sb, sorted_idx);
+        DODT_LAUNCH_CHECK();
+    } else {
+        hipLaunchKernelGGL(nms_keys_kernel, dim3(dodt::ceil_div(init_n, 256)), dim3(256), 0, s,
+                           d_scores, n, d_n, n_pad, keys, st, removed, nb, ranked ? rank : (int*)nullptr);
+        DODT_LAUNCH_CHECK();
+    }
+    if (ranked && fused) {
+    } else if (ranked) {
         hipLaunchKernelGGL(nms_rank_kernel, dim3(dodt::ceil_div(n, 256), dodt::ceil_div(n, kRankSeg)),
                            dim3(256), 0, s, keys, st, n_pad, rank);
         DODT_LAUNCH_CHECK();
diff --git a/dodt_amd/csrc/voxelizer.hip b/dodt_amd/csrc/voxelizer.hip
--- a/dodt_amd/csrc/voxelizer.hip
+++ b/dodt_amd/csrc/voxelizer.hip
@@ -1,6 +1,8 @@
 #include "common.h"
 
+#include <algorithm>
 #include <cmath>
+#include <cstdlib>
 #include <vector>
 
 namespace {
@@ -63,6 +65,27 @@
 __device__ __forceinline__ bool in_extents(const VoxParams& P, double x, double y, double z) {
     return x > P.ext[0] && x < P.ext[1] && y > P.ext[2] && y < P.ext[3] && z > P.ext[4] &&
            z < P.ext[5];
+}
+
+__device__ __forceinline__ void clear_words(uint32_t* __restrict__ p, size_t n, size_t tid, size_t nthreads) {
+    if (p == nullptr) return;
+    size_t head = ((16 - ((size_t)p & 15)) & 15) / 4;
+    if (head > n) head = n;
+    if (tid < head) p[tid] = 0u;
+    uint4* q = reinterpret_cast<uint4*>(p + head);
+    const size_t n4 = (n - head) / 4;
+    for (size_t i = tid; i < n4; i += nthreads) q[i] = make_uint4(0u, 0u, 0u, 0u);
+    const size_t done = head + 4 * n4;
+    if (tid < n - done) p[done + tid] = 0u;
+}
+
+__global__ void __launch_bounds__(256)
+vox_clear(uint32_t* __restrict__ out, size_t out_words, uint32_t* __restrict__ counters, size_t counter_words,
+          uint32_t* __restrict__ occ, size_t occ_words) {
+    const size_t tid = (size_t)blockIdx.x * blockDim.x + threadIdx.x, nthreads = (size_t)gridDim.x * blockDim.x;
+    clear_words(out, out_words, tid, nthreads);
+    clear_words(counters, counter_words, tid, nthreads);
+    clear_words(occ, occ_words, tid, nthreads);
 }
 
 __global__ void __launch_bounds__(256)
@@ -259,12 +282,20 @@
     uint32_t* list = counters + counters_bytes / sizeof(uint32_t);
     uint32_t* out = reinterpret_cast<uint32_t*>(d_bev_out);
 
-    DODT_HIP_CHECK(hipMemsetAsync(out, 0, cells * sizeof(uint32_t), ctx->stream));
-    DODT_HIP_CHECK(hipMemsetAsync(counters, 0, counters_bytes, ctx->stream));
-    if (d_occ_bits_out)
-        DODT_HIP_CHECK(hipMemsetAsync(d_occ_bits_out, 0,
-                                      (size_t)P.Z * P.occ_words_per_row * sizeof(uint32_t),
-                                      ctx->stream));
+    static const bool one_clear = !(getenv("DODT_VOX_CLEAR") && atoi(getenv("DODT_VOX_CLEAR")) == 0);
+    const size_t occ_words = d_occ_bits_out ? (size_t)P.Z * P.occ_words_per_row : 0;
+    if (one_clear) {
+        const size_t quads = (cells + 3) / 4;
+        const int blocks = (int)std::min<size_t>((quads + 1023) / 1024 + 1, 2048);
+        hipLaunchKernelGGL(vox_clear, dim3(blocks), dim3(256), 0, ctx->stream, out, cells, counters,
+                           counters_bytes / sizeof(uint32_t), d_occ_bits_out, occ_words);
+        DODT_LAUNCH_CHECK();
+    } else {
+        DODT_HIP_CHECK(hipMemsetAsync(out, 0, cells * sizeof(uint32_t), ctx->stream));
+        DODT_HIP_CHECK(hipMemsetAsync(counters, 0, counters_bytes, ctx->stream));
+        if (d_occ_bits_out)
+            DODT_HIP_CHECK(hipMemsetAsync(d_occ_bits_out, 0, occ_words * sizeof(uint32_t), ctx->stream));
+    }
     if (n_points > 0) {
         hipLaunchKernelGGL(vox_scatter, dim3(dodt::ceil_div(n_points, 256)), dim3(256), 0,
                            ctx->stream, d_points, P, out, d_occ_bits_out, list, counters,
diff --git a/dodt_amd/ops.py b/dodt_amd/ops.py
--- a/dodt_amd/ops.py
+++ b/dodt_amd/ops.py
@@ -159,6 +159,16 @@
         'dodt_crop_and_resize')
 
 
+def crop_pair(ctx, d_image_a, hw_a, d_image_b, hw_b, channels, d_boxes_a, d_boxes_b, n, d_n, crop_hw, d_out_a, d_out_b,
+              out_box_stride=None, d_mean=None, mean_stride=None):
+    crop = int(crop_hw[0]) * int(crop_hw[1]) * int(channels)
+    _lib.check(ctx.lib.dodt_crop_pair(
+        ctx.handle, _p(d_image_a), int(hw_a[0]), int(hw_a[1]), _p(d_image_b), int(hw_b[0]), int(hw_b[1]), int(channels),
+        _p(d_boxes_a), _p(d_boxes_b), int(n), _p(d_n), int(crop_hw[0]), int(crop_hw[1]), _p(d_out_a), _p(d_out_b),
+        int(crop if out_box_stride is None else out_box_stride), _p(d_mean),
+        int(crop if mean_stride is None else mean_stride)), 'dodt_crop_pair')
+
+
 def nms(ctx, d_boxes, d_scores, n, d_n, max_out, iou_threshold, d_sel, d_count):
     _lib.check(ctx.lib.dodt_nms(
         ctx.handle, _p(d_boxes), _p(d_scores), int(n), _p(d_n), int(max_out),
@@ -286,6 +296,28 @@
             self.handle, c.handle, _p(d_x), _p(d_x2), int(self.K if ldx is None else ldx),
             int(M), _p(d_m), _p(d_y), int(self.N if ldy is None else ldy)), 'dodt_fc_forward')
 
+    def can_pair(self, other, ldx=None):
+        return self.dtype == other.dtype == 'f32' and (self.K, self.N) == (other.K, other.N) and self.N >= 128 and \
+            self.K % 32 == 0 and self.K >= 64 and (self.K if ldx is None else ldx) % 4 == 0 and \
+            os.environ.get('DODT_FC_DMA') != '0'
+
+    def forward_pair(self, other, d_xa, d_xb, M, d_ya, d_yb, ldx=None, ldy=None, d_m=None, ctx=None):
+        c = ctx or self.ctx
+        _lib.check(c.lib.dodt_fc_forward_pair(
+            self.handle, other.handle, c.handle, _p(d_xa), _p(d_xb), int(self.K if ldx is None else ldx), int(M),
+            _p(d_m), _p(d_ya), _p(d_yb), int(self.N if ldy is None else ldy)), 'dodt_fc_forward_pair')
+
+    def can_front(self):
+        return self.dtype == 'f32' and self.K == 9 and self.N % 4 == 0
+
+    def rpn_front(self, d_map_a, hw_a, d_map_b, hw_b, d_boxes_a, d_boxes_b, n, d_roi_a, d_roi_b, d_y, ldy=None, d_n=None,
+                  ctx=None):
+        c = ctx or self.ctx
+        _lib.check(c.lib.dodt_rpn_front(
+            self.handle, c.handle, _p(d_map_a), int(hw_a[0]), int(hw_a[1]), _p(d_map_b), int(hw_b[0]), int(hw_b[1]),
+            _p(d_boxes_a), _p(d_boxes_b), int(n), _p(d_n), _p(d_roi_a), _p(d_roi_b), _p(d_y),
+            int(self.N if ldy is None else ldy)), 'dodt_rpn_front')
+
     def can_split(self, ldx=None):
         return self.N <= 32 and self.K % 16 == 0 and \
             (self.K if ldx is None else ldx) % 4 == 0 and os.environ.get('DODT_FC_SKINNY') != '0'
diff --git a/dodt_amd/pipeline.py b/dodt_amd/pipeline.py
--- a/dodt_amd/pipeline.py
+++ b/dodt_amd/pipeline.py
@@ -517,7 +517,9 @@
         split_t = computed and self.fps == 2 and ns >= 2 and not os.environ.get('DODT_PIPE_NO_CORR') \
             and os.environ.get('DODT_PIPE_CORR_ON_F1', '1') != '0'
         corr_img = split_t and self._corr_on_img()
-        fused_tail = os.environ.get('DODT_PIPE_FUSED_TAIL', '1') != '0'
+        tail_mode = os.environ.get('DODT_PIPE_FUSED_TAIL', '2')
+        fused_tail = tail_mode != '0'
+        fused_more = tail_mode not in ('0', '1')
 
         def t_branch_crops(cc, f0, scratch):
             fb0 = feat['bev_feat'].offset(4 * bev_px * FC * f0, bev_hw + (FC,))
@@ -537,14 +539,19 @@
             bneck_i = feat['img_bneck'].offset(4 * img_px * f, img_hw + (1,))
             feat_b = feat['bev_feat'].offset(4 * bev_px * FC * f, bev_hw + (FC,))
             feat_i = feat['img_feat'].offset(4 * img_px * FC * f, img_hw + (FC,))
-            ops.crop_and_resize(c, bneck_b, bev_hw + (1,), b['bev_norm'], A, None,
-                                (3, 3), b['rpn_bev_roi'])
-            ops.crop_and_resize(c, bneck_i, img_hw + (1,), b['img_norm'], A, None,
-                                (3, 3), b['rpn_img_roi'])
+            rpn_on = computed and not os.environ.get('DODT_PIPE_NO_RPN')
+            front = fused_more and rpn_on and self.rpn_head.can_front()
+            if not front:
+                ops.crop_and_resize(c, bneck_b, bev_hw + (1,), b['bev_norm'], A, None,
+                                    (3, 3), b['rpn_bev_roi'])
+                ops.crop_and_resize(c, bneck_i, img_hw + (1,), b['img_norm'], A, None,
+                                    (3, 3), b['rpn_img_roi'])
             self._mark(c, st['step'], 'tail%d_crops' % f)
-            if computed and not os.environ.get('DODT_PIPE_NO_RPN'):
+            if rpn_on:
                 self.rpn_head.forward(c, b['rpn_bev_roi'], b['rpn_img_roi'], A, b['rpn_logits'],
-                                      b['rpn_offsets'], scratch['rpn'])
+                                      b['rpn_offsets'], scratch['rpn'], fused=fused_more,
+                                      maps=(bneck_b, bev_hw, bneck_i, img_hw, b['bev_norm'], b['img_norm'])
+                                      if front else None)
             self._mark(c, st['step'], 'tail%d_rpn' % f)
             if fused_tail:
                 ops.rpn_decode(c, b['anchors'], h['rpn_offsets'], h['rpn_logits'], A, None, self.bev_extents_flat,
@@ -567,10 +574,15 @@
                 ops.project_anchors_f32(c, b['top_anchors'], self.P, b['top_count'],
                                         self.bev_extents_flat, self.p2, self.image_wh,
                                         d_bev_norm_tf=b['top_bev'], d_img_norm_tf=b['top_img'])
-            ops.crop_and_resize(c, feat_b, bev_hw + (FC,), b['top_bev'], self.P,
-                                b['top_count'], (ROI, ROI), b['bev_rois'])
-            ops.crop_and_resize(c, feat_i, img_hw + (FC,), b['top_img'], self.P,
-                                b['top_count'], (ROI, ROI), b['img_rois'])
+            mean_rows = self.avod_head.mean_rows(scratch['fc']) if computed and fused_more else None
+            if fused_more:
+                ops.crop_pair(c, feat_b, bev_hw, feat_i, img_hw, FC, b['top_bev'], b['top_img'], self.P, b['top_count'],
+                              (ROI, ROI), b['bev_rois'], b['img_rois'], d_mean=mean_rows)
+            else:
+                ops.crop_and_resize(c, feat_b, bev_hw + (FC,), b['top_bev'], self.P,
+                                    b['top_count'], (ROI, ROI), b['bev_rois'])
+                ops.crop_and_resize(c, feat_i, img_hw + (FC,), b['top_img'], self.P,
+                                    b['top_count'], (ROI, ROI), b['img_rois'])
             yield 'crops'
             pair = self.fps == 2
             corr_offsets = h.get('corr_offsets') if pair and f % 2 == 0 else None
@@ -579,7 +591,7 @@
                 self.avod_head.forward(c, b['bev_rois'], b['img_rois'], self.P, b['top_count'],
                                        [b['cls_logits'], b['offsets_4c']]
                                        + ([b['angle_vectors']] if self.box_4ca else []),
-                                       scratch['fc'])
+                                       scratch['fc'], mean_done=mean_rows is not None)
                 self._mark(c, st['step'], 'tail%d_fc2' % f)
                 yield 'head'
                 if pair and f % 2 == 0 and not os.environ.get('DODT_PIPE_NO_CORR'):
diff --git a/include/dodt_hip.h b/include/dodt_hip.h
--- a/include/dodt_hip.h
+++ b/include/dodt_hip.h
@@ -149,6 +149,10 @@
 int dodt_crop_and_resize_strided(dodt_ctx* ctx, const float* d_image, int H, int W, int C,
                                  const float* d_boxes, int n, const int32_t* d_n, int crop_h,
                                  int crop_w, float* d_out, long long out_box_stride);
+int dodt_crop_pair(dodt_ctx* ctx, const float* d_image_a, int Ha, int Wa, const float* d_image_b, int Hb, int Wb,
+                   int C, const float* d_boxes_a, const float* d_boxes_b, int n, const int32_t* d_n, int crop_h,
+                   int crop_w, float* d_out_a, float* d_out_b, long long out_box_stride, float* d_mean,
+                   long long mean_stride);
 
 int dodt_correlation(dodt_ctx* ctx, const float* d_a, const float* d_b, int H, int W, int C,
                      int max_displacement, int stride_2, int pad, float* d_out);
@@ -165,6 +169,11 @@
 int dodt_fc_destroy(dodt_fc* fc);
 int dodt_fc_forward(dodt_fc* fc, dodt_ctx* ctx, const float* d_x, const float* d_x2, int ldx,
                     int M, const int32_t* d_m, float* d_y, int ldy);
+int dodt_fc_forward_pair(dodt_fc* fc_a, dodt_fc* fc_b, dodt_ctx* ctx, const float* d_xa, const float* d_xb, int ldx,
+                         int M, const int32_t* d_m, float* d_ya, float* d_yb, int ldy);
+int dodt_rpn_front(dodt_fc* fc, dodt_ctx* ctx, const float* d_map_a, int Ha, int Wa, const float* d_map_b, int Hb, int Wb,
+                   const float* d_boxes_a, const float* d_boxes_b, int n, const int32_t* d_n, float* d_roi_a,
+                   float* d_roi_b, float* d_y, int ldy);
 int dodt_fc_forward_split(dodt_fc* fc, dodt_ctx* ctx, const float* d_x, int ldx, int M, const int32_t* d_m,
                           int parts, const int* widths, float* const* d_ys);
 int dodt_fc_bf16_row_elems(const dodt_fc* fc);
```

Result: no change. 389.2 (median of 5 runs) (+0.3%).
